# sara-nl/saraGAN

Hardware: AMD Instinct MI355X
Metric: 3D volumes/sec/node (G+D step) at 128x128x32 (higher is better)
Workload: dtype bf16

## Files before the change

include/saragan_hip.h:

```cpp
#ifndef SARAGAN_HIP_H
#define SARAGAN_HIP_H

#include <stddef.h>
#include <stdint.h>

#ifdef __cplusplus
extern "C" {
#endif

typedef void* sg_stream_t;

typedef enum { SG_F32 = 0, SG_BF16 = 1 } sg_dtype;

enum {
  SG_OK = 0,
  SG_EINVAL = -1,
  SG_EWORKSPACE = -2,
  SG_EALIGN = -3,
  SG_EUNSUPPORTED = -4
};

typedef struct {
  int32_t n, d, h, w;
  int32_t cin, cout;
  int32_t kd, kh, kw;
  int32_t upsample_in;
} sg_conv_shape;

typedef struct {
  uint32_t struct_size;
  const float* bias;
  int32_t act;
  float slope;
  int32_t pixel_norm;
  float eps;
  float* pn_scale;
  const void* mask_bits;
  float mask_slope;
  void* sign_out;
  int32_t out_scale;
  int32_t out_off[3];
  int32_t tap_off[3];
  int32_t pool;
  void* workspace;
  size_t workspace_bytes;
  int32_t x_plane_channels;
  const void* pn_bwd_y;
  const float* pn_bwd_scale;
  const void* in_mask_bits;
  float in_mask_slope;
  float in_gain;
  const float* rgb_w;
  const float* rgb_bias;
  void* rgb_out;
  const void* pw_x;
  const float* pw_wmat;
  void* pw_dx;
  float* pw_dw;
  float* pw_dbias;
  float pw_coef;
} sg_conv_epilogue;

size_t sg_sign_words_bytes(int64_t nvox, int32_t c);
int sg_sign_words(const void* t, void* words, int64_t nvox, int32_t c, sg_dtype dt, sg_stream_t st);

const char* sg_version(void);
const char* sg_error_string(int code);

size_t sg_conv3d_packed_bytes(const sg_conv_shape* s, sg_dtype dt);
int sg_conv3d_pack_weights(const float* w_dhwio, float coef, int transpose_flip, void* wp,
                           const sg_conv_shape* s, sg_dtype dt, sg_stream_t st);
int sg_conv3d_pack_weights_batch(int n, const float* const* w_dhwio, const float* coef, const int* transpose_flip,
                                 void* const* wp, const sg_conv_shape* shapes, sg_dtype dt, sg_stream_t st);
size_t sg_conv3d_fwd_workspace(const sg_conv_shape* s, sg_dtype dt);
size_t sg_conv3d_pw_epilogue_workspace(void);
int sg_conv3d_fwd(const void* x, const void* wp, void* y, const sg_conv_shape* s,
                  const sg_conv_epilogue* ep, sg_dtype dt, sg_stream_t st);
int sg_upconv3d_subpixel_supported(const sg_conv_shape* s, sg_dtype dt);
size_t sg_upconv3d_subpixel_packed_bytes(const sg_conv_shape* s, sg_dtype dt);
int sg_upconv3d_subpixel_pack(const float* w_dhwio, float coef, void* wp, const sg_conv_shape* s, sg_dtype dt, sg_stream_t st);
int sg_upconv3d_subpixel_fwd(const void* x, const void* wp, void* y, const sg_conv_shape* s, const sg_conv_epilogue* ep,
                             sg_dtype dt, sg_stream_t st);
int sg_upconv3d_subpixel_wgrad_supported(const sg_conv_shape* s, sg_dtype dt);
size_t sg_upconv3d_subpixel_wgrad_workspace(const sg_conv_shape* s, sg_dtype dt);
int sg_upconv3d_subpixel_wgrad(const void* x, const void* gy, float* dw_dhwio, float* dbias, float coef, void* workspace,
                               size_t workspace_bytes, const sg_conv_shape* s, sg_dtype dt, sg_stream_t st);
int sg_upconv3d_subpixel_dgrad_supported(const sg_conv_shape* s, sg_dtype dt);
size_t sg_upconv3d_subpixel_dgrad_packed_bytes(const sg_conv_shape* s, sg_dtype dt);
int sg_upconv3d_subpixel_dgrad_pack(const float* w_dhwio, float coef, void* wp, const sg_conv_shape* s, sg_dtype dt, sg_stream_t st);
int sg_upconv3d_subpixel_dgrad(const void* gy, const void* wp, void* gx, const sg_conv_shape* s, sg_dtype dt, sg_stream_t st);
size_t sg_conv3d_wgrad_workspace(const sg_conv_shape* s, sg_dtype dt);
int sg_conv3d_wgrad(const void* x, const void* dy, float* dw_dhwio, float coef, void* workspace,
                    size_t workspace_bytes, const sg_conv_shape* s, sg_dtype dt, sg_stream_t st);
int sg_conv3d_wgrad_bias(const void* x, const void* dy, float* dw_dhwio, float* dbias, float coef, void* workspace,
                         size_t workspace_bytes, const sg_conv_shape* s, sg_dtype dt, sg_stream_t st);
int sg_conv3d_wgrad_bias_up_masked(const void* x, const void* dy_half, const void* mask_bits, float mask_slope, float dy_gain,
                                   float* dw, float* dbias, float coef, void* workspace, size_t workspace_bytes,
                                   const sg_conv_shape* s, sg_dtype dt, sg_stream_t st);
#define SG_WGRAD_ACCUMULATE 1u
#define SG_WGRAD_CLEAN_WORKSPACE 2u
int sg_conv3d_wgrad_bias_ex(const void* x, const void* dy, const void* mask_bits, float mask_slope, float dy_gain,
                            float* dw_dhwio, float* dbias, float coef, unsigned flags, void* workspace, size_t workspace_bytes,
                            const sg_conv_shape* s, sg_dtype dt, sg_stream_t st);
size_t sg_conv3d_wgrad_clean_bytes(const sg_conv_shape* s, sg_dtype dt);

int sg_conv3d_pw_bwd(const void* x, const void* dy, const float* w_mat, float* dw_dhwio, float* dbias, void* dx,
                     float coef, void* workspace, size_t workspace_bytes, const sg_conv_shape* s, sg_dtype dt,
                     sg_stream_t st);

int sg_bias_act_fwd(const void* x, const float* bias, void* y, int64_t nvox, int32_t c, int32_t act,
                    float slope, sg_dtype dt, sg_stream_t st);
size_t sg_bias_act_bwd_workspace(int32_t c);
int sg_bias_act_bwd(const void* dy, const void* y, void* dx, float* dbias, void* workspace, int64_t nvox,
                    int32_t c, float slope, sg_dtype dt, sg_stream_t st);
int sg_bias_act_bwd_bits(const void* dy, const void* y_sign_words, void* dx, float* dbias, void* workspace,
                         int64_t nvox, int32_t c, float slope, sg_dtype dt, sg_stream_t st);
int sg_pixel_norm_fwd(const void* x, void* y, float* scale, int64_t nvox, int32_t c, float eps,
                      sg_dtype dt, sg_stream_t st);
int sg_pixel_norm_bwd(const void* dy, const void* y, const float* scale, void* dx, int64_t nvox,
                      int32_t c, sg_dtype dt, sg_stream_t st);
int sg_pixel_norm_act_bwd(const void* dy, const void* y, const float* scale, const void* y_sign_words, float slope,
                          void* dz, float* dbias, void* workspace, int64_t nvox, int32_t c, sg_dtype dt,
                          sg_stream_t st);
int sg_pixel_norm_act_bwd_pw(const void* g_small, int32_t cs, const float* w_small, const void* y, const float* scale,
                             const void* y_sign_words, float slope, void* dz, float* dbias, void* workspace,
                             int64_t nvox, int32_t c, sg_dtype dt, sg_stream_t st);
size_t sg_pixel_norm_act_bwd_pw_wg_workspace(int32_t c, int32_t cs);
int sg_pixel_norm_act_bwd_pw_wg(const void* g_small, int32_t cs, const float* w_small, const void* y, const float* scale,
                                const void* y_sign_words, float slope, void* dz, float* dbias, float* dw_small, float* db_small,
                                float coef_small, void* workspace, size_t workspace_bytes, int64_t nvox, int32_t c, sg_dtype dt,
                                sg_stream_t st);
int sg_upscale2x(const void* x, void* y, int32_t n, int32_t d, int32_t h, int32_t w, int32_t c,
                 float gain, sg_dtype dt, sg_stream_t st);
int sg_upscale2x_masked(const void* x, void* y, const void* mask_bits, float mask_slope, int32_t n, int32_t d,
                        int32_t h, int32_t w, int32_t c, float gain, sg_dtype dt, sg_stream_t st);
int sg_downscale2x(const void* x, void* y, int32_t n, int32_t d, int32_t h, int32_t w, int32_t c,
                   float gain, sg_dtype dt, sg_stream_t st);
int sg_upscale_nn(const void* x, void* y, const void* mask_bits, float mask_slope, int32_t n, int32_t d, int32_t h,
                  int32_t w, int32_t c, int32_t fd, int32_t fh, int32_t fw, float gain, sg_dtype dt, sg_stream_t st);
int sg_upscale_nn_planes(const void* x, void* y, const void* mask_bits, float mask_slope, int32_t n, int32_t d, int32_t h,
                         int32_t w, int32_t c, int32_t fd, int32_t fh, int32_t fw, float gain, int32_t plane_channels,
                         sg_dtype dt, sg_stream_t st);
int sg_downscale_sum(const void* x, void* y, int32_t n, int32_t d, int32_t h, int32_t w, int32_t c, int32_t fd,
                     int32_t fh, int32_t fw, float gain, sg_dtype dt, sg_stream_t st);
int sg_downscale_sum_masked(const void* x, const void* mask_bits, float mask_slope, void* y, int32_t n, int32_t d, int32_t h,
                            int32_t w, int32_t c, int32_t fd, int32_t fh, int32_t fw, float gain, sg_dtype dt, sg_stream_t st);
int sg_trilinear_up2x(const void* x, void* y, int32_t n, int32_t d, int32_t h, int32_t w, int32_t c, int32_t adjoint,
                      sg_dtype dt, sg_stream_t st);
int sg_axpby(const void* a, const void* b, void* out, float wa, float wb, int64_t numel, sg_dtype dt,
             sg_stream_t st);
int sg_axpby_dev(const void* a, const void* b, void* out, const float* w, int64_t numel, sg_dtype dt, sg_stream_t st);
int sg_lerp_rows(const void* a, const void* b, const float* gamma, void* out, int32_t n, int64_t per_sample, sg_dtype dt,
                 sg_stream_t st);
int sg_add_noise(const void* x, void* out, float stddev, uint64_t seed, uint64_t offset, int64_t numel,
                 sg_dtype dt, sg_stream_t st);
int sg_add_noise_dev(const void* x, void* out, float stddev, uint64_t seed, uint64_t* offset_dev, uint64_t bump,
                     int64_t numel, sg_dtype dt, sg_stream_t st);
int sg_sumsq_ndhwc_keep_w(const void* g, float* out, int32_t n, int32_t d, int32_t h, int32_t w, int32_t c,
                          sg_dtype dt, sg_stream_t st);
int sg_minibatch_stddev_fwd(const void* x, void* y, float* workspace, int32_t n, int64_t vox_per_sample,
                            int32_t c, int32_t group_size, sg_dtype dt, sg_stream_t st);
int sg_minibatch_stddev_bwd(const void* dy, const void* x, void* dx, float* workspace, int32_t n,
                            int64_t vox_per_sample, int32_t c, int32_t group_size, sg_dtype dt, sg_stream_t st);
size_t sg_mbstd_stat_workspace(int32_t n, int64_t vox_per_sample, int32_t c, int32_t group_size, int32_t nseg);
int sg_mbstd_stat_fwd(const void* x, float* stat, float* workspace, size_t workspace_bytes, int32_t n, int64_t vox_per_sample,
                      int32_t c, int32_t group_size, int32_t nseg, sg_dtype dt, sg_stream_t st);
int sg_mbstd_stat_bwd(const float* gstat, const void* x, void* dx, int32_t n, int64_t vox_per_sample, int32_t c,
                      int32_t group_size, int32_t nseg, sg_dtype dt, sg_stream_t st);
int sg_mbstd_stat_bwd2(const void* h, const void* x, const float* gstat, void* gx, float* ggstat, float* workspace,
                       size_t workspace_bytes, int32_t n, int64_t vox_per_sample, int32_t c, int32_t group_size, int32_t nseg,
                       sg_dtype dt, sg_stream_t st);
int sg_mbstd_term_fwd(const void* y, const float* s, const float* B, void* out, int32_t n, int64_t plane, sg_dtype dt,
                      sg_stream_t st);
int sg_mbstd_term_dot(const void* g, const float* B, float* r, int32_t n, int64_t plane, sg_dtype dt, sg_stream_t st);
int sg_mbstd_term_outer(const float* s, const void* g, float* Bg, int32_t n, int64_t plane, sg_dtype dt, sg_stream_t st);
int sg_cond_embed(void* z, const float* c, float* W, void* out, int32_t n, int32_t zdim, int32_t l, int32_t adjoint, sg_dtype dt,
                  sg_stream_t st);
int sg_cond_project(const void* o, const float* c, void* out, int32_t n, int32_t l, int32_t adjoint, sg_dtype dt, sg_stream_t st);
int sg_cast(const void* src, sg_dtype dt_src, void* dst, sg_dtype dt_dst, int64_t numel, sg_stream_t st);

int sg_adam_ema(float* p, const float* g, float* m, float* v, float* ema, int64_t numel, float lr_t,
                float b1, float b2, float eps, float gscale, float ema_decay, sg_stream_t st);
enum { SG_OPT_SGD = 0, SG_OPT_MOMENTUM = 1, SG_OPT_ADADELTA = 2 };
int sg_optim_step(int kind, float* p, const float* g, float* s1, float* s2, float* ema, int64_t numel, float lr,
                  float h, float eps, int nesterov, float gscale, float ema_decay, sg_stream_t st);
int sg_adam_ema_dev(float* p, const float* g, float* m, float* v, float* ema, int64_t numel, const float* lr_t,
                    float b1, float b2, float eps, float gscale, float ema_decay, sg_stream_t st);
int sg_optim_step_dev(int kind, float* p, const float* g, float* s1, float* s2, float* ema, int64_t numel, const float* lr,
                      float h, float eps, int nesterov, float gscale, float ema_decay, sg_stream_t st);
int sg_segment_sumsq(const float* flat, const int64_t* offsets, float* out, int32_t nseg, sg_stream_t st);
int sg_nonfinite_flag(const float* x, int64_t numel, int32_t* flag, int32_t accumulate, sg_stream_t st);
int sg_segment_sumsq_flag(const float* flat, const int64_t* offsets, float* out, int32_t nseg, int32_t* flag,
                          int32_t accumulate, sg_stream_t st);
int sg_guard_step(const int32_t* flag, int64_t* t, int64_t* counters, double lr, const double* lr_dev, float* lr_t,
                  int32_t adam, double b1, double b2, sg_stream_t st);
int sg_adam_ema_guarded(float* p, const float* g, float* m, float* v, float* ema, int64_t numel, const float* lr_t,
                        const int32_t* skip, float b1, float b2, float eps, float gscale, float ema_decay, sg_stream_t st);
int sg_optim_step_guarded(int kind, float* p, const float* g, float* s1, float* s2, float* ema, int64_t numel,
                          const float* lr, const int32_t* skip, float h, float eps, int nesterov, float gscale,
                          float ema_decay, sg_stream_t st);
#define SG_SEG_CHUNK 4096
int sg_adamw_ema(float* p, const float* g, float* m, float* v, float* ema, int64_t total, const int64_t* segs,
                 const int32_t* blocks, int32_t nseg, int32_t nblocks, float lr, const float* lr_dev, const int32_t* skip,
                 float b1, float b2, float eps, float decay, float gscale, float ema_decay, sg_stream_t st);
int sg_lamb_moments(const float* p, const float* g, float* m, float* v, int64_t total, const int64_t* segs,
                    const int32_t* blocks, int32_t nseg, int32_t nblocks, float* partials, const int64_t* t, int32_t advance,
                    const int32_t* skip, double b1, double b2, float eps, float decay, float gscale, sg_stream_t st);
int sg_lamb_ratios(const int64_t* segs, int32_t nseg, int32_t nblocks, const float* partials, float* ratios, int64_t* t,
                   int32_t advance, const int32_t* skip, sg_stream_t st);
int sg_lamb_update(float* p, const float* m, const float* v, float* ema, int64_t total, const int64_t* segs,
                   const int32_t* blocks, int32_t nseg, int32_t nblocks, const float* ratios, const int64_t* t, float lr,
                   const float* lr_dev, const int32_t* skip, double b1, double b2, float eps, float decay, float ema_decay,
                   sg_stream_t st);

#define SG_SPECTRAL_SEG_FIELDS 8
int sg_spectral_refresh(const float* p, float* eff, int64_t total, const int64_t* segs, const int32_t* blocks, int32_t nseg,
                        int32_t nblocks, float* u, int64_t ulen, float* v, int64_t vlen, float* sigma, float* nt,
                        float* partials, float* cols, int64_t collen, int32_t iteration, sg_stream_t st);
int sg_spectral_pullback(float* g, const float* eff, int64_t total, const int64_t* segs, const int32_t* blocks, int32_t nseg,
                         int32_t nblocks, const float* u, int64_t ulen, const float* v, int64_t vlen, const float* sigma,
                         float* partials, sg_stream_t st);

enum { SG_AUG_FLIP_W = 1, SG_AUG_FLIP_H = 2, SG_AUG_FLIP_D = 4, SG_AUG_ROT90 = 8, SG_AUG_TRANSLATE = 16, SG_AUG_ALL = 31 };
int sg_augment_draw(int32_t* params, int32_t n, uint32_t ops, int32_t m_d, int32_t m_h, int32_t m_w, float p,
                    const float* p_dev, uint64_t seed, uint64_t offset, uint64_t* offset_dev, uint64_t bump, sg_stream_t st);
int sg_augment_apply(const void* x, void* y, const int32_t* params, int32_t n, int32_t d, int32_t h, int32_t w, int32_t c,
                     uint32_t ops, float fill, int32_t adjoint, sg_dtype dt, sg_stream_t st);
int sg_ada_update(const float* logits, int32_t n, int64_t* state, float* p, int32_t interval, int64_t target_num,
                  int64_t target_den, float delta, float p_max, sg_stream_t st);

enum { SG_AUGF_SCALE = 32, SG_AUGF_ROTATE = 64, SG_AUGF_SHIFT = 128, SG_AUGF_BRIGHTNESS = 256, SG_AUGF_CONTRAST = 512,
       SG_AUGF_ALL = 992 };
int sg_augment_affine_draw(float* params, int32_t n, uint32_t ops, int32_t d, int32_t h, int32_t w, double max_scale,
                           double max_angle, double max_shift_d, double max_shift_h, double max_shift_w, double max_brightness,
                           double max_contrast, float p, const float* p_dev, uint64_t seed, uint64_t offset, uint64_t* offset_dev,
                           uint64_t bump, sg_stream_t st);
int sg_augment_affine_apply(const void* x, void* y, const float* params, int32_t n, int32_t d, int32_t h, int32_t w, int32_t c,
                            float fill, uint32_t flags, sg_dtype dt, sg_stream_t st);

int sg_filter_axis(const void* x, void* y, const void* add, int64_t outer, int32_t n, int64_t inner, const double* taps,
                   int32_t ntaps, int32_t mode, int32_t border, double alpha, int32_t f64, sg_stream_t st);
int sg_swd_gather(const float* x, float* out, const int32_t* d0, const int32_t* h0, const int32_t* w0, int32_t n_img,
                  int32_t c, int32_t d, int32_t h, int32_t w, int32_t per_image, int32_t rd, int32_t rh, int32_t rw,
// ... 44 lines not shown
```

saragan_amd/_lib.py:

```python
import ctypes as C
import os

_HERE = os.path.dirname(os.path.abspath(__file__))
LIB_PATH = os.environ.get('SARAGAN_LIB') or os.path.join(_HERE, 'libsaragan_hip.so')

SG_F32, SG_BF16 = 0, 1
SG_OPT_SGD, SG_OPT_MOMENTUM, SG_OPT_ADADELTA = 0, 1, 2
SG_SEG_CHUNK = 4096
SG_EUNSUPPORTED = -4
SG_WGRAD_ACCUMULATE, SG_WGRAD_CLEAN_WORKSPACE = 1, 2
SG_AUG_FLIP_W, SG_AUG_FLIP_H, SG_AUG_FLIP_D, SG_AUG_ROT90, SG_AUG_TRANSLATE, SG_AUG_ALL = 1, 2, 4, 8, 16, 31
SG_AUGF_SCALE, SG_AUGF_ROTATE, SG_AUGF_SHIFT, SG_AUGF_BRIGHTNESS, SG_AUGF_CONTRAST, SG_AUGF_ALL = 32, 64, 128, 256, 512, 992
SG_AUGF_ADJOINT, SG_AUGF_LINEAR = 1, 2


class ConvShape(C.Structure):
    _fields_ = [('n', C.c_int32), ('d', C.c_int32), ('h', C.c_int32), ('w', C.c_int32),
                ('cin', C.c_int32), ('cout', C.c_int32),
                ('kd', C.c_int32), ('kh', C.c_int32), ('kw', C.c_int32), ('upsample_in', C.c_int32)]


class ConvEpilogue(C.Structure):
    _fields_ = [('struct_size', C.c_uint32),
                ('bias', C.c_void_p), ('act', C.c_int32), ('slope', C.c_float), ('pixel_norm', C.c_int32),
                ('eps', C.c_float), ('pn_scale', C.c_void_p), ('mask_bits', C.c_void_p), ('mask_slope', C.c_float),
                ('sign_out', C.c_void_p), ('out_scale', C.c_int32), ('out_off', C.c_int32 * 3),
                ('tap_off', C.c_int32 * 3), ('pool', C.c_int32), ('workspace', C.c_void_p),
                ('workspace_bytes', C.c_size_t), ('x_plane_channels', C.c_int32), ('pn_bwd_y', C.c_void_p),
                ('pn_bwd_scale', C.c_void_p), ('in_mask_bits', C.c_void_p), ('in_mask_slope', C.c_float),
                ('in_gain', C.c_float), ('rgb_w', C.c_void_p), ('rgb_bias', C.c_void_p), ('rgb_out', C.c_void_p),
                ('pw_x', C.c_void_p), ('pw_wmat', C.c_void_p), ('pw_dx', C.c_void_p), ('pw_dw', C.c_void_p),
                ('pw_dbias', C.c_void_p), ('pw_coef', C.c_float)]

    def __init__(self, *args, **kw):
        super().__init__(C.sizeof(type(self)), *args, **kw)


class ProfEntry(C.Structure):
    _fields_ = [('kind', C.c_int32), ('shape', ConvShape), ('dtype', C.c_int32), ('launches', C.c_int64),
                ('total_ms', C.c_double), ('flops_per_launch', C.c_double), ('kernel', C.c_char * 64)]


_p, _i32, _i64, _f, _u64, _sz = C.c_void_p, C.c_int32, C.c_int64, C.c_float, C.c_uint64, C.c_size_t
_SHP = C.POINTER(ConvShape)

SIGNATURES = {
    'sg_version': (C.c_char_p, []),
    'sg_error_string': (C.c_char_p, [C.c_int]),
    'sg_conv3d_packed_bytes': (_sz, [_SHP, C.c_int]),
    'sg_conv3d_pack_weights': (C.c_int, [_p, _f, C.c_int, _p, _SHP, C.c_int, _p]),
    'sg_conv3d_pack_weights_batch': (C.c_int, [C.c_int, _p, _p, _p, _p, _p, C.c_int, _p]),
    'sg_conv3d_fwd_workspace': (_sz, [_SHP, C.c_int]),
    'sg_conv3d_pw_epilogue_workspace': (_sz, []),
    'sg_conv3d_fwd': (C.c_int, [_p, _p, _p, _SHP, C.POINTER(ConvEpilogue), C.c_int, _p]),
    'sg_upconv3d_subpixel_supported': (C.c_int, [_SHP, C.c_int]),
    'sg_upconv3d_subpixel_packed_bytes': (_sz, [_SHP, C.c_int]),
    'sg_upconv3d_subpixel_pack': (C.c_int, [_p, _f, _p, _SHP, C.c_int, _p]),
    'sg_upconv3d_subpixel_fwd': (C.c_int, [_p, _p, _p, _SHP, C.POINTER(ConvEpilogue), C.c_int, _p]),
    'sg_upconv3d_subpixel_wgrad_supported': (C.c_int, [_SHP, C.c_int]),
    'sg_upconv3d_subpixel_wgrad_workspace': (_sz, [_SHP, C.c_int]),
    'sg_upconv3d_subpixel_wgrad': (C.c_int, [_p, _p, _p, _p, _f, _p, _sz, _SHP, C.c_int, _p]),
    'sg_upconv3d_subpixel_dgrad_supported': (C.c_int, [_SHP, C.c_int]),
    'sg_upconv3d_subpixel_dgrad_packed_bytes': (_sz, [_SHP, C.c_int]),
    'sg_upconv3d_subpixel_dgrad_pack': (C.c_int, [_p, _f, _p, _SHP, C.c_int, _p]),
    'sg_upconv3d_subpixel_dgrad': (C.c_int, [_p, _p, _p, _SHP, C.c_int, _p]),
    'sg_conv3d_wgrad_workspace': (_sz, [_SHP, C.c_int]),
    'sg_conv3d_wgrad': (C.c_int, [_p, _p, _p, _f, _p, _sz, _SHP, C.c_int, _p]),
    'sg_conv3d_pw_bwd': (C.c_int, [_p, _p, _p, _p, _p, _p, _f, _p, _sz, _SHP, C.c_int, _p]),
    'sg_conv3d_wgrad_bias': (C.c_int, [_p, _p, _p, _p, _f, _p, _sz, _SHP, C.c_int, _p]),
    'sg_conv3d_wgrad_bias_up_masked': (C.c_int, [_p, _p, _p, _f, _f, _p, _p, _f, _p, _sz, _SHP, C.c_int, _p]),
    'sg_conv3d_wgrad_bias_ex': (C.c_int, [_p, _p, _p, _f, _f, _p, _p, _f, C.c_uint, _p, _sz, _SHP, C.c_int, _p]),
    'sg_conv3d_wgrad_clean_bytes': (_sz, [_SHP, C.c_int]),
    'sg_bias_act_fwd': (C.c_int, [_p, _p, _p, _i64, _i32, _i32, _f, C.c_int, _p]),
    'sg_bias_act_bwd_workspace': (_sz, [_i32]),
    'sg_bias_act_bwd': (C.c_int, [_p, _p, _p, _p, _p, _i64, _i32, _f, C.c_int, _p]),
    'sg_bias_act_bwd_bits': (C.c_int, [_p, _p, _p, _p, _p, _i64, _i32, _f, C.c_int, _p]),
    'sg_sign_words_bytes': (_sz, [_i64, _i32]),
    'sg_sign_words': (C.c_int, [_p, _p, _i64, _i32, C.c_int, _p]),
    'sg_pixel_norm_fwd': (C.c_int, [_p, _p, _p, _i64, _i32, _f, C.c_int, _p]),
    'sg_pixel_norm_bwd': (C.c_int, [_p, _p, _p, _p, _i64, _i32, C.c_int, _p]),
    'sg_pixel_norm_act_bwd': (C.c_int, [_p, _p, _p, _p, _f, _p, _p, _p, _i64, _i32, C.c_int, _p]),
    'sg_pixel_norm_act_bwd_pw': (C.c_int, [_p, _i32, _p, _p, _p, _p, _f, _p, _p, _p, _i64, _i32, C.c_int, _p]),
    'sg_pixel_norm_act_bwd_pw_wg': (C.c_int, [_p, _i32, _p, _p, _p, _p, _f, _p, _p, _p, _p, _f, _p, _sz, _i64, _i32, C.c_int, _p]),
    'sg_pixel_norm_act_bwd_pw_wg_workspace': (_sz, [_i32, _i32]),
    'sg_upscale2x': (C.c_int, [_p, _p, _i32, _i32, _i32, _i32, _i32, _f, C.c_int, _p]),
    'sg_upscale2x_masked': (C.c_int, [_p, _p, _p, _f, _i32, _i32, _i32, _i32, _i32, _f, C.c_int, _p]),
    'sg_downscale2x': (C.c_int, [_p, _p, _i32, _i32, _i32, _i32, _i32, _f, C.c_int, _p]),
    'sg_upscale_nn': (C.c_int, [_p, _p, _p, _f, _i32, _i32, _i32, _i32, _i32, _i32, _i32, _i32, _f, C.c_int, _p]),
    'sg_upscale_nn_planes': (C.c_int, [_p, _p, _p, _f, _i32, _i32, _i32, _i32, _i32, _i32, _i32, _i32, _f, _i32, C.c_int, _p]),
    'sg_downscale_sum': (C.c_int, [_p, _p, _i32, _i32, _i32, _i32, _i32, _i32, _i32, _i32, _f, C.c_int, _p]),
    'sg_downscale_sum_masked': (C.c_int, [_p, _p, _f, _p, _i32, _i32, _i32, _i32, _i32, _i32, _i32, _i32, _f, C.c_int, _p]),
    'sg_trilinear_up2x': (C.c_int, [_p, _p, _i32, _i32, _i32, _i32, _i32, _i32, C.c_int, _p]),
    'sg_axpby': (C.c_int, [_p, _p, _p, _f, _f, _i64, C.c_int, _p]),
    'sg_axpby_dev': (C.c_int, [_p, _p, _p, _p, _i64, C.c_int, _p]),
    'sg_lerp_rows': (C.c_int, [_p, _p, _p, _p, _i32, _i64, C.c_int, _p]),
    'sg_add_noise': (C.c_int, [_p, _p, _f, _u64, _u64, _i64, C.c_int, _p]),
    'sg_add_noise_dev': (C.c_int, [_p, _p, _f, _u64, _p, _u64, _i64, C.c_int, _p]),
    'sg_sumsq_ndhwc_keep_w': (C.c_int, [_p, _p, _i32, _i32, _i32, _i32, _i32, C.c_int, _p]),
    'sg_minibatch_stddev_fwd': (C.c_int, [_p, _p, _p, _i32, _i64, _i32, _i32, C.c_int, _p]),
    'sg_minibatch_stddev_bwd': (C.c_int, [_p, _p, _p, _p, _i32, _i64, _i32, _i32, C.c_int, _p]),
    'sg_mbstd_stat_workspace': (_sz, [_i32, _i64, _i32, _i32, _i32]),
    'sg_mbstd_stat_fwd': (C.c_int, [_p, _p, _p, _sz, _i32, _i64, _i32, _i32, _i32, C.c_int, _p]),
    'sg_mbstd_stat_bwd': (C.c_int, [_p, _p, _p, _i32, _i64, _i32, _i32, _i32, C.c_int, _p]),
    'sg_mbstd_stat_bwd2': (C.c_int, [_p, _p, _p, _p, _p, _p, _sz, _i32, _i64, _i32, _i32, _i32, C.c_int, _p]),
    'sg_mbstd_term_fwd': (C.c_int, [_p, _p, _p, _p, _i32, _i64, C.c_int, _p]),
    'sg_mbstd_term_dot': (C.c_int, [_p, _p, _p, _i32, _i64, C.c_int, _p]),
    'sg_mbstd_term_outer': (C.c_int, [_p, _p, _p, _i32, _i64, C.c_int, _p]),
    'sg_cond_embed': (C.c_int, [_p, _p, _p, _p, _i32, _i32, _i32, _i32, C.c_int, _p]),
    'sg_cond_project': (C.c_int, [_p, _p, _p, _i32, _i32, _i32, C.c_int, _p]),
    'sg_cast': (C.c_int, [_p, C.c_int, _p, C.c_int, _i64, _p]),
    'sg_adam_ema': (C.c_int, [_p, _p, _p, _p, _p, _i64, _f, _f, _f, _f, _f, _f, _p]),
    'sg_optim_step': (C.c_int, [C.c_int, _p, _p, _p, _p, _p, _i64, _f, _f, _f, C.c_int, _f, _f, _p]),
    'sg_adam_ema_dev': (C.c_int, [_p, _p, _p, _p, _p, _i64, _p, _f, _f, _f, _f, _f, _p]),
    'sg_optim_step_dev': (C.c_int, [C.c_int, _p, _p, _p, _p, _p, _i64, _p, _f, _f, C.c_int, _f, _f, _p]),
    'sg_segment_sumsq': (C.c_int, [_p, _p, _p, _i32, _p]),
    'sg_nonfinite_flag': (C.c_int, [_p, _i64, _p, _i32, _p]),
    'sg_segment_sumsq_flag': (C.c_int, [_p, _p, _p, _i32, _p, _i32, _p]),
    'sg_guard_step': (C.c_int, [_p, _p, _p, C.c_double, _p, _p, _i32, C.c_double, C.c_double, _p]),
    'sg_adam_ema_guarded': (C.c_int, [_p, _p, _p, _p, _p, _i64, _p, _p, _f, _f, _f, _f, _f, _p]),
    'sg_optim_step_guarded': (C.c_int, [C.c_int, _p, _p, _p, _p, _p, _i64, _p, _p, _f, _f, C.c_int, _f, _f, _p]),
    'sg_adamw_ema': (C.c_int, [_p, _p, _p, _p, _p, _i64, _p, _p, _i32, _i32, _f, _p, _p, _f, _f, _f, _f, _f, _f, _p]),
    'sg_lamb_moments': (C.c_int, [_p, _p, _p, _p, _i64, _p, _p, _i32, _i32, _p, _p, _i32, _p, C.c_double, C.c_double, _f, _f,
                                  _f, _p]),
    'sg_lamb_ratios': (C.c_int, [_p, _i32, _i32, _p, _p, _p, _i32, _p, _p]),
    'sg_lamb_update': (C.c_int, [_p, _p, _p, _p, _i64, _p, _p, _i32, _i32, _p, _p, _f, _p, _p, C.c_double, C.c_double, _f, _f,
                                 _f, _p]),
    'sg_spectral_refresh': (C.c_int, [_p, _p, _i64, _p, _p, _i32, _i32, _p, _i64, _p, _i64, _p, _p, _p, _p, _i64, _i32, _p]),
    'sg_spectral_pullback': (C.c_int, [_p, _p, _i64, _p, _p, _i32, _i32, _p, _i64, _p, _i64, _p, _p, _p]),
    'sg_augment_draw': (C.c_int, [_p, _i32, C.c_uint32, _i32, _i32, _i32, _f, _p, _u64, _u64, _p, _u64, _p]),
    'sg_augment_apply': (C.c_int, [_p, _p, _p, _i32, _i32, _i32, _i32, _i32, C.c_uint32, _f, _i32, C.c_int, _p]),
    'sg_ada_update': (C.c_int, [_p, _i32, _p, _p, _i32, _i64, _i64, _f, _f, _p]),
    'sg_augment_affine_draw': (C.c_int, [_p, _i32, C.c_uint32, _i32, _i32, _i32, C.c_double, C.c_double, C.c_double, C.c_double,
                                         C.c_double, C.c_double, C.c_double, _f, _p, _u64, _u64, _p, _u64, _p]),
    'sg_augment_affine_apply': (C.c_int, [_p, _p, _p, _i32, _i32, _i32, _i32, _i32, _f, C.c_uint32, C.c_int, _p]),
    'sg_filter_axis': (C.c_int, [_p, _p, _p, _i64, _i32, _i64, C.POINTER(C.c_double), _i32, _i32, _i32, C.c_double, _i32, _p]),
    'sg_swd_gather': (C.c_int, [_p, _p, _p, _p, _p, _i32, _i32, _i32, _i32, _i32, _i32, _i32, _i32, _i32, _p]),
    'sg_desc_normalize_workspace': (_sz, [_i32]),
    'sg_desc_normalize': (C.c_int, [_p, _i64, _i32, _i64, _p, _sz, _p]),
    'sg_swd_padded_rows': (_i32, [_i32]),
    'sg_swd_project': (C.c_int, [_p, _p, _p, _i32, _i32, _i32, _i32, _p]),
    'sg_sort_rows': (C.c_int, [_p, _i32, _i32, _p]),
    'sg_swd_distance': (C.c_int, [_p, _p, _p, _i32, _i32, _i32, _p]),
    'sg_metric_workspace': (_sz, []),
    'sg_sqdiff_mean': (C.c_int, [_p, _p, _p, _i64, _p, _sz, _p]),
    'sg_minmax': (C.c_int, [_p, _p, _i64, _p, _sz, _p]),
    'sg_ssim_products': (C.c_int, [_p, _p, _p, _p, _p, _i64, _p]),
    'sg_ssim_mean': (C.c_int, [_p, _p, _p, _p, _p, _p, _i32, _i32, _i32, _i32, _i32, _i32, C.c_double, C.c_double, C.c_double, _p, _sz, _p]),
    'sg_pairwise_sqdist_chunk': (_i32, []),
    'sg_pairwise_sqdist_workspace': (_sz, [_i32, _i32, _i64]),
    'sg_pairwise_sqdist': (C.c_int, [_p, _p, _p, _i32, _i32, _i64, _p, _sz, _p]),
    'sg_prof_enable': (C.c_int, [C.c_int]),
    'sg_prof_enabled': (C.c_int, []),
    'sg_prof_collect': (C.c_int, [C.POINTER(ProfEntry), _i32, C.POINTER(_i32)]),
    'sg_prof_set_filter': (C.c_int, [C.c_int, _SHP]),
    'sg_config_reload': (C.c_int, []),
}

_lib = None


def load():
    global _lib
    if _lib is not None:
        return _lib
    if not os.path.exists(LIB_PATH):
        raise ImportError(
            f'{LIB_PATH} not found: build it with `python -m saragan_amd.build` (hipcc, gfx950). '
            'There is no CPU or PyTorch fallback for the HIP path.')
    import torch
    lib = C.CDLL(LIB_PATH)
    for name, (res, args) in SIGNATURES.items():
        fn = getattr(lib, name)
        fn.restype = res
        fn.argtypes = args
    _lib = lib
    return lib


class SgError(RuntimeError):
    pass


def check(rc, what=''):
    if rc != 0:
        msg = load().sg_error_string(int(rc)).decode()
        raise SgError(f'{what}: {msg} (code {rc})')
```

saragan_amd/csrc/conv3d.hip:

```cpp
#include "common.h"
#include "prof.h"
#include "conv_args.h"

struct PackArgs {
  const float* w;
  void* wp;
  float coef;
  int taps, kd, kh, kw, cin, cout, nchunk, ntile, flip;
};

template <typename T>
__global__ void pack_weights_kernel(PackArgs a) {
  constexpr int CH = sg_traits<T>::CH;
  constexpr int EPL = CH / 2;
  const int64_t total = (int64_t)a.nchunk * a.taps * a.ntile * 64 * EPL;
  T* out = reinterpret_cast<T*>(a.wp);
  for (int64_t i = (int64_t)blockIdx.x * blockDim.x + threadIdx.x; i < total; i += (int64_t)gridDim.x * blockDim.x) {
    int e = (int)(i % EPL);
    int64_t q = i / EPL;
    int lane = (int)(q % 64); q /= 64;
    int nt = (int)(q % a.ntile); q /= a.ntile;
    int tap = (int)(q % a.taps);
    int chunk = (int)(q / a.taps);
    int ci = chunk * CH + (lane >> 5) * EPL + e;
// ... 1856 lines not shown
            float ss = 0.f;
#pragma unroll
            for (int nt = 0; nt < NTB; ++nt)
#pragma unroll
              for (int i = 0; i < 16; ++i) ss += acc[mt][nt][i] * acc[mt][nt][i];
            ss += __shfl_xor(ss, 32);
            const float sc = rsqrtf(ss * inv_c + a.eps);
#pragma unroll
            for (int nt = 0; nt < NTB; ++nt)
#pragma unroll
              for (int i = 0; i < 16; ++i) acc[mt][nt][i] *= sc;
            if (a.pn_scale != nullptr && hh == 0 && ok)
              a.pn_scale[ovox(n, d, h, w)] = sc;
          }
          if (a.sign_out != nullptr) {
#pragma unroll
            for (int nt = 0; nt < NTB; ++nt) {
              const uint32_t sw = sg_sign_word(acc[mt][nt], hh);
              if (hh == 0 && ok && nt < ntb)
                a.sign_out[ovox(n, d, h, w) * a.ntile + nt0 + nt] = sw;
            }
          }
          if (use_mask) {
#pragma unroll
            for (int nt = 0; nt < NTB; ++nt) sg_apply_sign_word(acc[mt][nt], mb[mt][nt], hh, a.mask_slope);
          }
          if (sizeof(T) == 2 && wide_store) {
            bf16_t* yrow = reinterpret_cast<bf16_t*>(y) + ovox(n, d, h, w) * (int64_t)a.cout + nt0 * 32;
#pragma unroll
            for (int nt = 0; nt < NTB; ++nt) sg_store_tile_row_bf16(yrow + nt * 32, acc[mt][nt], hh, ok && nt < ntb);
          } else if (ok) {
            T* yrow = y + ovox(n, d, h, w) * (int64_t)a.cout;
#pragma unroll
            for (int nt = 0; nt < NTB; ++nt)
#pragma unroll
              for (int qd = 0; qd < 4; ++qd) {
                const int co = (nt0 + nt) * 32 + 8 * qd + 4 * hh;
                if (a.vec_out && co + 4 <= a.cout) {
                  T tmp[4];
#pragma unroll
                  for (int e = 0; e < 4; ++e) tmp[e] = sg_traits<T>::from_f(acc[mt][nt][qd * 4 + e]);
                  if (sizeof(T) == 2) *reinterpret_cast<u32x2*>(yrow + co) = *reinterpret_cast<u32x2*>(tmp);
                  else { const u32x4 t16 = *reinterpret_cast<u32x4*>(tmp); *reinterpret_cast<u32x4*>(yrow + co) = t16; SG_STORE16_GUARD(t16); }
                } else {
#pragma unroll
                  for (int e = 0; e < 4; ++e)
                    if (co + e < a.cout) yrow[co + e] = sg_traits<T>::from_f(acc[mt][nt][qd * 4 + e]);
                }
              }
          }
        }
      }
    }
    stamp();
    __syncthreads();
  }
}

template <typename T, int MTW, int NTB, int KD, int KH, int KW, int RS = 1>
static int launch_fwd4(ConvFwdArgs& a, const sg_conv_shape* s, hipStream_t st, bool* used) {
  *used = false;
  constexpr int BM = MTW * 128;
  a.g = sg_make_geom(s, BM, true);
  const sg_tile_geom& g = a.g;
  if (g.TW > 255 || g.TH > 255 || g.TD > 255 || g.TN > 127) return SG_OK;
  const int64_t ntiles = (int64_t)g.nTn * g.nTd * g.nTh * g.nTw;
  const int ny = sg_cdiv(a.ntile, NTB);
  int gx = (256 / ny) / 8 * 8;
  if (gx < 8) gx = 8;
  if (sg_cfg().fwd4_gx > 0) gx = sg_cfg().fwd4_gx;
  if (gx < 8 || (gx & 7)) return SG_EINVAL;
  if (ntiles >= (1 << 24) || ntiles < 2 * gx) return SG_OK;
  if (KD == 1 && ntiles < 4 * gx) return SG_OK;
  if ((int64_t)g.TN * s->d * s->h * s->w * (int64_t)s->cin * (int64_t)sizeof(T) >= (1ll << 31)) return SG_OK;
  const int hv = g.TN * g.HD * g.HH * g.HW;
  a.G = 1;
  a.rs = 32;
  a.xbytes = hv * 32;
  a.lean = ((!s->upsample_in || (g.TD % 2 == 0 && g.TH % 2 == 0 && g.TW % 2 == 0 && g.TN == 1)) &&
            !sg_cfg().fwd4_no_lean) ? 1 : 0;
  a.wbytes = a.taps * NTB * 1024;
  if (sg_cdiv(hv * 2, 64) > (MTW > 2 ? 40 : (RS == 2 ? 24 : 32))) return SG_OK;
  if (MTW * NTB >= 4 && !(RS == 1 ? (g.TW == 32 && g.TH % MTW == 0) : (g.TW == 16 && g.TH % (2 * MTW) == 0))) return SG_OK;
  size_t lds = 2ull * a.xbytes + (size_t)a.nchunk * a.wbytes + NTB * 128;
  a.wres = (lds <= 160 * 1024 && !sg_cfg().fwd4_no_wres) ? 1 : 0;
  if (!a.wres) lds = 2ull * a.xbytes + 2ull * a.wbytes + NTB * 128;
  if (lds > 160 * 1024) return SG_OK;
  a.ntiles = (int)ntiles;
  a.vec_in = 1;
  a.vec_out = (s->cout % 4 == 0) ? 1 : 0;
  auto kern = conv_fwd4_kernel<T, MTW, NTB, KD, KH, KW, RS>;
  SG_ALLOW_160K_LDS(kern);
  SG_KNAME("conv_fwd4<%s,%d,%d,%d,%d,%d>", sg_tname<T>(), MTW, NTB, KD, KH, KW);
  hipLaunchKernelGGL(kern, dim3((unsigned)gx, (unsigned)ny), dim3(512), lds, st, a);
  SG_LAUNCH_CHECK();
  *used = true;
  return SG_OK;
}

template <int RING>
struct sg_unrolled_k5 {
  static constexpr int TAPS = 27, PF = RING - 1, RPS = 4, NA = 36;
  template <int ST>
  static __device__ __forceinline__ void load(u32x4 (&wfr)[RING][2], u32x4 (&xfr)[RING][2], const int (&xaddr)[NA], int wl_off) {
    constexpr int SL = ST % RING;
#pragma unroll
    for (int nt = 0; nt < 2; ++nt)
      asm volatile("ds_read_b128 %0, %1 offset:%2" : "=v"(wfr[SL][nt]) : "v"(wl_off), "n"((ST * 2 + nt) << 10));
#pragma unroll
    for (int mt = 0; mt < 2; ++mt)
      asm volatile("ds_read_b128 %0, %1" : "=v"(xfr[SL][mt]) : "v"(xaddr[sg_xa_index<2, 3, 3, true>(ST, mt)]));
  }
  template <int ST>
  static __device__ __forceinline__ void step(f32x16 (&acc)[2][2], u32x4 (&wfr)[RING][2], u32x4 (&xfr)[RING][2],
                                              const int (&xaddr)[NA], int wl_off) {
    if constexpr (ST < TAPS) {
      if constexpr (ST + PF < TAPS) load<ST + PF>(wfr, xfr, xaddr, wl_off);
      constexpr int younger = (TAPS - 1 - ST < PF ? TAPS - 1 - ST : PF) * RPS;
      asm volatile("s_waitcnt lgkmcnt(%0)" ::"n"(younger));
      __builtin_amdgcn_sched_barrier(0);
#pragma unroll
      for (int mt = 0; mt < 2; ++mt)
#pragma unroll
        for (int nt = 0; nt < 2; ++nt) sg_mfma_bf16_acc(acc[mt][nt], wfr[ST % RING][nt], xfr[ST % RING][mt]);
      __builtin_amdgcn_sched_barrier(0);
      step<ST + 1>(acc, wfr, xfr, xaddr, wl_off);
    }
  }
  template <int ST>
  static __device__ __forceinline__ void prologue(u32x4 (&wfr)[RING][2], u32x4 (&xfr)[RING][2], const int (&xaddr)[NA], int wl_off) {
    if constexpr (ST < PF) {
      load<ST>(wfr, xfr, xaddr, wl_off);
      prologue<ST + 1>(wfr, xfr, xaddr, wl_off);
    }
  }
  static __device__ __forceinline__ void run(f32x16 (&acc)[2][2], const int (&xaddr)[NA], int wl_off) {
    u32x4 wfr[RING][2], xfr[RING][2];
    SG_KLOOP_BEGIN();
    prologue<0>(wfr, xfr, xaddr, wl_off);
    step<0>(acc, wfr, xfr, xaddr, wl_off);
    asm volatile("s_nop 7\n\ts_nop 7\n\ts_nop 3" : "+v"(acc[0][0]), "+v"(acc[0][1]), "+v"(acc[1][0]), "+v"(acc[1][1]));
    SG_KLOOP_END();
  }
};

template <int EPI>
__global__ __launch_bounds__(512) void conv_fwd5_kernel(ConvFwdArgs a) {
  extern __shared__ __attribute__((aligned(16))) char smem[];
  typedef bf16_t T;
  constexpr int TAPS = 27, ES = 2, EPP = 8, NFRAG = TAPS * 2, HF = (NFRAG + 1) / 2;
  constexpr uint32_t DEAD = 0x80000000u;
  constexpr bool SIGN = (EPI & SG_EP_SIGN) != 0, MASK = (EPI & SG_EP_MASK) != 0, PN = (EPI & SG_EP_PN) != 0;
  constexpr bool POOL = (EPI & SG_EP_POOL) != 0;
  const sg_tile_geom& g = a.g;
  const int tid = threadIdx.x, lane = tid & 63;
  const int wave8 = __builtin_amdgcn_readfirstlane(tid >> 6);
  const int grp = wave8 >> 2, wave = wave8 & 3;
  const int r = lane & 31, hh = lane >> 5;
  const int xmine = grp * a.xbytes, wbase = 2 * a.xbytes;
  float* bias_lds = reinterpret_cast<float*>(smem + 2 * a.xbytes + 2 * a.wbytes);
  const int nt0 = blockIdx.y * 2;
  const int ncg = a.nchunk, cout = a.cout, ntile = a.ntile, cin = a.cin;
  const int D = g.D, H = g.H, W = g.W;

  const int xg = blockIdx.x & 7, slot = blockIdx.x >> 3;
  const int per_x = gridDim.x >> 3;
  const int cpx = (a.ntiles + 7) >> 3;
  const int t_begin = xg * cpx;
  const int t_end = min(a.ntiles, t_begin + cpx);
  const int first = t_begin + slot;
  const int K = first < t_end ? (t_end - first + per_x - 1) / per_x : 0;
  const int kmine = (K + 1 - grp) >> 1;
  const int items_mine = kmine * ncg;
  const int items_max = ((K + 1) >> 1) * ncg;

  int xaddr[36];
  int tcoord[2];
#pragma unroll
  for (int mt = 0; mt < 2; ++mt) {
    const int m = (wave * 2 + mt) * 32 + r;
    const int tw = m & 31, q = m >> 5;
    const int th = q % g.TH, td = q / g.TH;
    tcoord[mt] = tw | (th << 8) | (td << 16);
    if (mt > 0) continue;
    const int lrow = (td * g.HH + th) * g.HW + tw;
#pragma unroll
    for (int kd = 0; kd < 3; ++kd)
#pragma unroll
      for (int kh = 0; kh < 4; ++kh)
#pragma unroll
        for (int kw = 0; kw < 3; ++kw) {
          const int row = lrow + (kd * g.HH + kh) * g.HW + kw;
          xaddr[(kd * 4 + kh) * 3 + kw] = xmine + row * 32 + ((hh ^ ((row >> 3) & 1)) << 4);
        }
  }
  const int hv = g.HD * g.HH * g.HW;
  constexpr int MAXIT = 8;
  uint32_t relb[MAXIT];
  int crd[MAXIT];
#pragma unroll
  for (int k = 0; k < MAXIT; ++k) {
    const int it = (wave + 4 * k) * 64 + lane;
    const int row = it >> 1;
    const int sl = (it & 1) ^ ((row >> 3) & 1);
    uint32_t q = sg_div((uint32_t)row, g.fHW);
    const int hw = (int)(row - q * g.HW);
    uint32_t q2 = sg_div(q, g.fHH);
    const int hh_ = (int)(q - q2 * g.HH), hd = (int)q2;
    relb[k] = row < hv ? (uint32_t)((((hd * H + hh_) * W + hw) * cin + sl * EPP) * ES) : 0xC0000000u;
    crd[k] = row < hv ? (hw | (hh_ << 8) | (hd << 16)) : 0x7F7F7F7F;
  }
  const int64_t svox = (int64_t)D * H * W;
  const int64_t xsb = svox * cin * ES, ysb = (POOL ? svox >> 2 : svox) * cout * ES, wsb = svox * ntile * 4, psb = svox * 4;
  auto rsrc_of = [&](const void* base, int64_t sample_bytes, int n0) {
    return __builtin_amdgcn_make_buffer_rsrc(const_cast<char*>(reinterpret_cast<const char*>(base)) + n0 * sample_bytes, 0,
                                             (int)sample_bytes, 0x00020000);
  };
  const __amdgpu_buffer_rsrc_t rw = __builtin_amdgcn_make_buffer_rsrc(const_cast<void*>(a.wp), 0, 0x7FFFFFFF, 0x00020000);

  int kS = 0, cgS = 0;
  __amdgpu_buffer_rsrc_t rxS;
  uint32_t vk[MAXIT];
  auto enter_tile_S = [&]() {
    const sg_tile_origin o = sg_tile_of(g, (uint32_t)(first + (2 * kS + grp) * per_x));
    rxS = rsrc_of(a.x, xsb, o.n0);
    const int tile_off = (((o.d0 - 1) * H + (o.h0 - 1)) * W + (o.w0 - 1)) * cin * ES;
    const int lo_w = max(0, 1 - o.w0), hi_w = min(g.HW, W + 1 - o.w0) - 1;
    const int lo_h = max(0, 1 - o.h0), hi_h = min(g.HH, H + 1 - o.h0) - 1;
    const int lo_d = max(0, 1 - o.d0), hi_d = min(g.HD, D + 1 - o.d0) - 1;
    const uint32_t lo = (uint32_t)(lo_w | (lo_h << 8) | (lo_d << 16));
    const uint32_t hi = (uint32_t)(hi_w | (hi_h << 8) | (hi_d << 16)) | 0x808080u;
#pragma unroll
    for (int k = 0; k < MAXIT; ++k) {
      const uint32_t c_ = (uint32_t)crd[k] & 0xFFFFFFu;
      const uint32_t t1 = (c_ | 0x808080u) - lo, t2 = hi - c_;
      vk[k] = (t1 & t2 & 0x808080u) == 0x808080u ? relb[k] + (uint32_t)tile_off : DEAD;
    }
  };
  auto stage_halo = [&]() {
    const uint32_t soff = (uint32_t)(cgS * 32);
#pragma unroll
    for (int k = 0; k < MAXIT; ++k)
      if ((wave + 4 * k) * 64 < hv * 2 && crd[k] != 0x7F7F7F7F)
        __builtin_amdgcn_raw_ptr_buffer_load_lds(rxS, (lds_ptr_t)(smem + xmine + (wave + 4 * k) * 1024), 16, vk[k], soff, 0, 0);
  };
  auto stage_slab = [&](int j, int f0, int f1, int w, int nw) {
    const int cg = j % ncg;
    char* dst = smem + wbase + (j & 1) * a.wbytes;
    const uint32_t cbase = (uint32_t)(cg * TAPS * ntile + nt0) << 10;
    for (int f = f0 + w; f < f1; f += nw) {
      const int tap = f >> 1, nt = f & 1;
      __builtin_amdgcn_raw_ptr_buffer_load_lds(rw, (lds_ptr_t)(dst + (f << 10)), 16, (uint32_t)(lane * 16),
                                               cbase + ((uint32_t)(tap * ntile + nt) << 10), 0, 0);
    }
  };
  int kE = 0;
  __amdgpu_buffer_rsrc_t ryE, rsE, rmE, rpE;
  uint32_t vox[2];
  uint32_t pvox = DEAD;
  auto enter_tile_E = [&]() {
    const sg_tile_origin o = sg_tile_of(g, (uint32_t)(first + (2 * kE + grp) * per_x));
    ryE = rsrc_of(a.y, ysb, o.n0);
    if (SIGN) rsE = rsrc_of(a.sign_out, wsb, o.n0);
    if (MASK) rmE = rsrc_of(a.mask_bits, wsb, o.n0);
    if (PN) rpE = rsrc_of(a.pn_scale, psb, o.n0);
#pragma unroll
    for (int mt = 0; mt < 2; ++mt) {
      const int tc = tcoord[mt];
      const int d = o.d0 + (tc >> 16), h = o.h0 + ((tc >> 8) & 255), w = o.w0 + (tc & 255);
      vox[mt] = (d < D && h < H && w < W) ? (uint32_t)((d * H + h) * W + w) : DEAD;
      if (POOL && mt == 0)
        pvox = (vox[0] != DEAD && !(r & 1)) ? (uint32_t)((d * (H >> 1) + (h >> 1)) * (W >> 1) + (w >> 1)) : DEAD;
    }
  };
  uint32_t mbn[2][2] = {{0u, 0u}, {0u, 0u}};
  auto request_mask = [&]() {
    if constexpr (MASK) {
#pragma unroll
      for (int mt = 0; mt < 2; ++mt)
#pragma unroll
        for (int nt = 0; nt < 2; ++nt)
          mbn[mt][nt] = __builtin_amdgcn_raw_buffer_load_b32(rmE, (kE < kmine && vox[mt] != DEAD) ? (vox[mt] * (uint32_t)ntile + nt0 + nt) * 4u : DEAD, 0, 0);
    }
  };

  if (tid < 64) {
    const int co = nt0 * 32 + tid;
    bias_lds[tid] = (a.bias != nullptr && co < cout) ? a.bias[co] : 0.f;
  }
  if (items_max > 0) stage_slab(0, 0, NFRAG, wave8, 8);
  if (items_mine > 0) {
    enter_tile_S();
    enter_tile_E();
    request_mask();
    if (grp == 0) stage_halo();
  }
  asm volatile("s_waitcnt vmcnt(0)" ::: "memory");
  __syncthreads();

  const int wl0 = wbase + lane * 16;
  const float inv_c = 1.f / (float)cout;
  const float slope = a.act ? a.slope : 1.f;
  f32x16 acc[2][2];
  auto init_acc = [&]() {
#pragma unroll
    for (int mt = 0; mt < 2; ++mt)
#pragma unroll
      for (int nt = 0; nt < 2; ++nt)
#pragma unroll
        for (int i = 0; i < 16; ++i) acc[mt][nt][i] = bias_lds[nt * 32 + (i & 3) + 8 * (i >> 2) + 4 * hh];
    asm volatile("" : "+v"(acc[0][0]), "+v"(acc[0][1]), "+v"(acc[1][0]), "+v"(acc[1][1]));
  };
  int dbgi = 0;
  auto stamp = [&]() {
    if (a.dbg != nullptr && blockIdx.x == 8 && blockIdx.y == 0 && lane == 0 && wave == 0 && dbgi < 120)
      a.dbg[grp * 128 + dbgi] = __builtin_amdgcn_s_memtime();
    ++dbgi;
  };
  auto mfma_phase = [&](int q) { sg_unrolled_k5<3>::run(acc, xaddr, wl0 + (q & 1) * a.wbytes); };

  auto off_phase = [&](bool closes, int qn, int js, int f0, int f1) {
    if (qn < items_mine) stage_halo();
    if (js < items_max) stage_slab(js, f0, f1, wave, 4);
    __builtin_amdgcn_sched_barrier(0);
    stamp();
    if (closes) {
#pragma unroll
      for (int mt = 0; mt < 2; ++mt) {
        const bool ok = vox[mt] != DEAD;
        if (slope != 1.f) {
#pragma unroll
          for (int nt = 0; nt < 2; ++nt)
#pragma unroll
            for (int i = 0; i < 16; ++i) acc[mt][nt][i] = sg_lrelu(acc[mt][nt][i], slope);
        }
        if (PN) {
          float ss = 0.f;
#pragma unroll
          for (int nt = 0; nt < 2; ++nt)
#pragma unroll
            for (int i = 0; i < 16; ++i) ss += acc[mt][nt][i] * acc[mt][nt][i];
          const auto sw2 = __builtin_amdgcn_permlane32_swap(__float_as_uint(ss), __float_as_uint(ss), false, false);
          ss = __uint_as_float(sw2[0]) + __uint_as_float(sw2[1]);
          const float sc = rsqrtf(ss * inv_c + a.eps);
#pragma unroll
          for (int nt = 0; nt < 2; ++nt)
#pragma unroll
            for (int i = 0; i < 16; ++i) acc[mt][nt][i] *= sc;
          if (a.pn_scale != nullptr)
            __builtin_amdgcn_raw_buffer_store_b32(__float_as_uint(sc), rpE, (ok && hh == 0) ? vox[mt] * 4u : DEAD, 0, 0);
        }
#pragma unroll
        for (int nt = 0; nt < 2; ++nt) {
          if (SIGN) {
            uint32_t b = 0u;
#pragma unroll
            for (int i = 0; i < 16; ++i) b |= (__float_as_uint(acc[mt][nt][i]) >> 31) << ((i & 3) + 8 * (i >> 2));
            b <<= 4 * hh;
            const auto sw2 = __builtin_amdgcn_permlane32_swap(b, b, false, false);
            __builtin_amdgcn_raw_buffer_store_b32(sw2[0] | sw2[1], rsE, (ok && hh == 0) ? (vox[mt] * (uint32_t)ntile + nt0 + nt) * 4u : DEAD, 0, 0);
          }
          if (MASK) sg_apply_sign_word(acc[mt][nt], mbn[mt][nt], hh, a.mask_slope);
          if constexpr (!POOL) {
#pragma unroll
            for (int j = 0; j < 2; ++j) {
              const uint32_t a0 = sg_pack_bf16(acc[mt][nt][8 * j + 0], acc[mt][nt][8 * j + 1]), a1 = sg_pack_bf16(acc[mt][nt][8 * j + 2], acc[mt][nt][8 * j + 3]);
              const uint32_t b0 = sg_pack_bf16(acc[mt][nt][8 * j + 4], acc[mt][nt][8 * j + 5]), b1 = sg_pack_bf16(acc[mt][nt][8 * j + 6], acc[mt][nt][8 * j + 7]);
              const auto s0 = __builtin_amdgcn_permlane32_swap(a0, b0, false, false);
              const auto s1 = __builtin_amdgcn_permlane32_swap(a1, b1, false, false);
              u32x4 out;
              out[0] = s0[0]; out[1] = s1[0]; out[2] = s0[1]; out[3] = s1[1];
              __builtin_amdgcn_raw_buffer_store_b128(out, ryE, ok ? (vox[mt] * (uint32_t)cout + (uint32_t)((nt0 + nt) * 32 + 16 * j + 8 * hh)) * 2u : DEAD, 0, 0);
              SG_STORE16_GUARD(out);
            }
          }
        }
      }
      if constexpr (POOL) {
#pragma unroll
        for (int nt = 0; nt < 2; ++nt) {
          float sp[16];
#pragma unroll
          for (int i = 0; i < 16; ++i) {
            const float t = acc[0][nt][i] + acc[1][nt][i];
            const float u = __uint_as_float((uint32_t)__builtin_amdgcn_update_dpp(0, (int)__float_as_uint(t), 0xB1, 0xF, 0xF, true));
            sp[i] = (t + u) * 0.25f;
          }
#pragma unroll
          for (int j = 0; j < 2; ++j) {
            const uint32_t a0 = sg_pack_bf16(sp[8 * j + 0], sp[8 * j + 1]), a1 = sg_pack_bf16(sp[8 * j + 2], sp[8 * j + 3]);
            const uint32_t b0 = sg_pack_bf16(sp[8 * j + 4], sp[8 * j + 5]), b1 = sg_pack_bf16(sp[8 * j + 6], sp[8 * j + 7]);
            const auto s0 = __builtin_amdgcn_permlane32_swap(a0, b0, false, false);
            const auto s1 = __builtin_amdgcn_permlane32_swap(a1, b1, false, false);
            u32x4 out;
            out[0] = s0[0]; out[1] = s1[0]; out[2] = s0[1]; out[3] = s1[1];
            __builtin_amdgcn_raw_buffer_store_b128(out, ryE, pvox != DEAD ? (pvox * (uint32_t)cout + (uint32_t)((nt0 + nt) * 32 + 16 * j + 8 * hh)) * 2u : DEAD, 0, 0);
            SG_STORE16_GUARD(out);
          }
        }
      }
      ++kE;
      if (kE < kmine) enter_tile_E();
      request_mask();
      init_acc();
    }
    if (qn < items_mine) {
      if (++cgS == ncg) {
        cgS = 0;
        ++kS;
        if (kS < kmine) enter_tile_S();
      }
    }
    asm volatile("s_waitcnt vmcnt(0)" ::: "memory");
  };

  if (grp == 0) {
    init_acc();
    if (items_mine > 0 && ++cgS == ncg) { cgS = 0; ++kS; if (kS < kmine) enter_tile_S(); }
    for (int q = 0; q < items_max; ++q) {
      stamp();
      if (q < items_mine) mfma_phase(q);
      stamp();
      __syncthreads();
      stamp();
      off_phase(q < items_mine && (q % ncg) == ncg - 1, q + 1, q + 1, HF, NFRAG);
      stamp();
      __syncthreads();
    }
  } else {
    init_acc();
    for (int q = 0; q < items_max; ++q) {
      stamp();
      off_phase(q > 0 && q - 1 < items_mine && ((q - 1) % ncg) == ncg - 1, q, q + 1, 0, HF);
      stamp();
      __syncthreads();
      stamp();
      if (q < items_mine) mfma_phase(q);
      stamp();
      __syncthreads();
    }
    if (items_mine > 0 && items_mine == items_max) off_phase(true, items_mine, items_max, 0, 0);
    else if (items_mine > 0) {  }
  }
}

template <int EPI>
static int launch_fwd5_inst(const ConvFwdArgs& a, unsigned gx, unsigned gy, size_t lds, hipStream_t st) {
  auto kern = conv_fwd5_kernel<EPI>;
  SG_ALLOW_160K_LDS(kern);
  hipLaunchKernelGGL(kern, dim3(gx, gy), dim3(512), lds, st, a);
  return SG_OK;
}

static int launch_fwd5(ConvFwdArgs& a, const sg_conv_shape* s, hipStream_t st, bool* used) {
  *used = false;
  if (s->upsample_in || s->kd != 3 || s->kh != 3 || s->kw != 3 || a.os == 2 || a.tap_d || a.tap_h || a.tap_w) return SG_OK;
  if ((s->cin % 16) != 0 || (s->cout % 64) != 0 || a.pool == 1) return SG_OK;
  if (a.pool && ((s->h | s->w) & 1 || a.pixel_norm || a.mask_bits)) return SG_OK;
  if (a.pixel_norm && (a.mask_bits || a.ntile != 2)) return SG_OK;
  if (a.mask_bits && a.sign_out) return SG_OK;
  a.g = sg_make_geom(s, 256, true);
  const sg_tile_geom& g = a.g;
  if (g.TN != 1 || g.TW != 32 || (g.TH & 1) || g.TD * g.TH * g.TW != 256 || g.HD > 127 || g.HH > 127 || g.HW > 127) return SG_OK;
  const int64_t ntiles = (int64_t)g.nTn * g.nTd * g.nTh * g.nTw;
  const int ny = a.ntile / 2;
  int gx = (256 / ny) / 8 * 8;
  if (gx < 8) gx = 8;
  if (ntiles >= (1 << 24) || ntiles < 2 * gx) return SG_OK;
  {
    const int64_t svox = (int64_t)s->d * s->h * s->w;
    if (svox * s->cin * 2 >= (1ll << 31) || svox * s->cout * 2 >= (1ll << 31) || svox * a.ntile * 4 >= (1ll << 31)) return SG_OK;
  }
  const int hv = g.HD * g.HH * g.HW;
  if (sg_cdiv(hv * 2, 64) > 32) return SG_OK;
  a.G = 1;
  a.rs = 32;
  a.xbytes = hv * 32;
  a.wbytes = 27 * 2 * 1024;
  a.wres = 0;
  const size_t lds = 2ull * a.xbytes + 2ull * a.wbytes + 256;
  if (lds > 160 * 1024) return SG_OK;
  a.ntiles = (int)ntiles;
  a.vec_in = 1;
  a.vec_out = 1;
  const int epi = (a.sign_out ? SG_EP_SIGN : 0) | (a.mask_bits ? SG_EP_MASK : 0) | (a.pixel_norm ? SG_EP_PN : 0) |
                  (a.pool ? SG_EP_POOL : 0);
  int rc = SG_OK;
  switch (epi) {
    case 0: rc = launch_fwd5_inst<0>(a, (unsigned)gx, (unsigned)ny, lds, st); break;
    case SG_EP_POOL: rc = launch_fwd5_inst<SG_EP_POOL>(a, (unsigned)gx, (unsigned)ny, lds, st); break;
    case SG_EP_SIGN | SG_EP_POOL: rc = launch_fwd5_inst<SG_EP_SIGN | SG_EP_POOL>(a, (unsigned)gx, (unsigned)ny, lds, st); break;
    case SG_EP_SIGN: rc = launch_fwd5_inst<SG_EP_SIGN>(a, (unsigned)gx, (unsigned)ny, lds, st); break;
    case SG_EP_MASK: rc = launch_fwd5_inst<SG_EP_MASK>(a, (unsigned)gx, (unsigned)ny, lds, st); break;
    case SG_EP_PN: rc = launch_fwd5_inst<SG_EP_PN>(a, (unsigned)gx, (unsigned)ny, lds, st); break;
    case SG_EP_PN | SG_EP_SIGN: rc = launch_fwd5_inst<SG_EP_PN | SG_EP_SIGN>(a, (unsigned)gx, (unsigned)ny, lds, st); break;
    default: return SG_OK;
  }
  if (rc != SG_OK) return rc;
  SG_KNAME("conv_fwd5<bf16,2,2,3,3,3>");
  SG_LAUNCH_CHECK();
  *used = true;
  return SG_OK;
}

template <typename T>
__device__ __forceinline__ float sg_packed_w(const char* wp, int ntile, int cin_j, int cout_c) {
  constexpr int CH = sg_traits<T>::CH, ES = (int)sizeof(T);
  const int chunk = cin_j / CH, hh = (cin_j % CH) / (CH / 2), e = cin_j % (CH / 2);
  const char* frag = wp + ((int64_t)(chunk * ntile + (cout_c >> 5)) << 10);
  return sg_traits<T>::to_f(*reinterpret_cast<const T*>(frag + ((cout_c & 31) + 32 * hh) * 16 + e * ES));
}

template <typename T, int CIN>
__global__ __launch_bounds__(256) void pw_fwd_small_cin_kernel(ConvFwdArgs a, int64_t nvox) {
  constexpr int E = 16 / (int)sizeof(T);
  const int P = a.cout / E;
  const int p = threadIdx.x % P;
  const int c0 = p * E;
  const char* wp = reinterpret_cast<const char*>(a.wp);
  float w[CIN][E], b[E];
#pragma unroll
  for (int j = 0; j < CIN; ++j)
#pragma unroll
    for (int e = 0; e < E; ++e) w[j][e] = sg_packed_w<T>(wp, a.ntile, j, c0 + e);
#pragma unroll
  for (int e = 0; e < E; ++e) b[e] = a.bias ? a.bias[c0 + e] : 0.f;
  const T* x = reinterpret_cast<const T*>(a.x);
  T* y = reinterpret_cast<T*>(a.y);
  const int rows = 256 / P;
  const int tpw = P < 32 / E ? P : 32 / E;
  const int64_t nv_pad = (nvox + rows - 1) / rows * rows;
  const int64_t stride = (int64_t)gridDim.x * rows;
  const float slope = a.act ? a.slope : 1.f;
  const bool masked = a.mask_bits != nullptr, signs = a.sign_out != nullptr;
  const int wsel = c0 >> 5, wsh = c0 & 31, psh = (p % tpw) * E;
  auto fetch = [&](int64_t v, float (&xv)[CIN], uint32_t& mw) {
    const int64_t vc = v < nvox ? v : nvox - 1;
#pragma unroll
    for (int j = 0; j < CIN; ++j) xv[j] = sg_traits<T>::to_f(x[vc * CIN + j]);
    mw = masked ? a.mask_bits[vc * a.ntile + wsel] >> wsh : 0u;
  };
  int64_t v = (int64_t)blockIdx.x * rows + threadIdx.x / P;
  float xn[CIN];
  uint32_t mwn = 0u;
  if (v < nv_pad) fetch(v, xn, mwn);
  for (; v < nv_pad; v += stride) {
    float xv[CIN];
#pragma unroll
    for (int j = 0; j < CIN; ++j) xv[j] = xn[j];
    const uint32_t mw = mwn;
    if (v + stride < nv_pad) fetch(v + stride, xn, mwn);
    const bool live = v < nvox;
    float o[E];
    uint32_t neg = 0u;
#pragma unroll
    for (int e = 0; e < E; ++e) {
      float t = b[e];
#pragma unroll
      for (int j = 0; j < CIN; ++j) t = fmaf(xv[j], w[j][e], t);
      t = fmaxf(t, t * slope);
      neg |= (t < 0.f ? 1u : 0u) << e;
      o[e] = t;
    }
    if (signs) {
      uint32_t wbits = neg << psh;
      if (tpw == 4) {
        wbits |= (uint32_t)__builtin_amdgcn_update_dpp(0, (int)wbits, 0xB1, 0xF, 0xF, true);
        wbits |= (uint32_t)__builtin_amdgcn_update_dpp(0, (int)wbits, 0x4E, 0xF, 0xF, true);
      } else {
        for (int sh = 1; sh < tpw; sh <<= 1) wbits |= (uint32_t)__shfl_xor((int)wbits, sh);
      }
      if (live && p % tpw == 0) a.sign_out[v * a.ntile + wsel] = wbits;
    }
    if (!live) continue;
    if (masked) {
#pragma unroll
      for (int e = 0; e < E; ++e) o[e] = ((mw >> e) & 1u) ? o[e] * a.mask_slope : o[e];
    }
    u32x4 raw;
    T* t = reinterpret_cast<T*>(&raw);
#pragma unroll
    for (int e = 0; e < E; ++e) t[e] = sg_traits<T>::from_f(o[e]);
    __builtin_nontemporal_store(raw, reinterpret_cast<u32x4*>(y + v * a.cout + c0));
    SG_STORE16_GUARD(raw);
  }
}

template <typename T>
__global__ __launch_bounds__(256) void pw_fwd_small_cout_kernel(ConvFwdArgs a, int64_t nvox) {
  constexpr int E = 16 / (int)sizeof(T);
  const int P = a.cin / E;
  const int p = threadIdx.x % P;
  const char* wp = reinterpret_cast<const char*>(a.wp);
  float w[E][4];
#pragma unroll
  for (int e = 0; e < E; ++e)
#pragma unroll
    for (int c = 0; c < 4; ++c) w[e][c] = c < a.cout ? sg_packed_w<T>(wp, a.ntile, p * E + e, c) : 0.f;
  const T* x = reinterpret_cast<const T*>(a.x);
  T* y = reinterpret_cast<T*>(a.y);
  const int rows = 256 / P;
  const int64_t nv_pad = (nvox + rows - 1) / rows * rows;
  constexpr int U = 4;
  const int64_t nv_pad4 = (nvox + U * rows - 1) / (U * rows) * (U * rows);
  for (int64_t vb = (int64_t)blockIdx.x * U * rows + threadIdx.x / P; vb < nv_pad4; vb += (int64_t)gridDim.x * U * rows) {
    u32x4 rawu[U];
    uint32_t mwu[U];
#pragma unroll
    for (int u = 0; u < U; ++u) {
      const int64_t v = vb + u * rows;
      rawu[u] = v < nvox ? *reinterpret_cast<const u32x4*>(x + v * a.cin + p * E) : u32x4{0u, 0u, 0u, 0u};
      mwu[u] = (v < nvox && p == 0 && a.mask_bits) ? a.mask_bits[v] : 0u;
    }
#pragma unroll
    for (int u = 0; u < U; ++u) {
    const int64_t v = vb + u * rows;
    if (v >= nv_pad) break;
    const bool live = v < nvox;
    float s[4] = {0.f, 0.f, 0.f, 0.f};
    {
      const u32x4 raw = rawu[u];
      const T* t = reinterpret_cast<const T*>(&raw);
#pragma unroll
      for (int e = 0; e < E; ++e) {
        const float xv = sg_traits<T>::to_f(t[e]);
#pragma unroll
        for (int c = 0; c < 4; ++c) s[c] = fmaf(xv, w[e][c], s[c]);
      }
    }
    for (int sh = 1; sh < P; sh <<= 1)
#pragma unroll
      for (int c = 0; c < 4; ++c) s[c] += __shfl_xor(s[c], sh);
    if (live && p == 0) {
      uint32_t neg = 0u;
      const uint32_t mw = mwu[u];
#pragma unroll
      for (int c = 0; c < 4; ++c) {
        if (c < a.cout) {
          float t = s[c] + (a.bias ? a.bias[c] : 0.f);
          if (a.act) t = fmaxf(t, t * a.slope);
          neg |= (t < 0.f ? 1u : 0u) << c;
          if ((mw >> c) & 1u) t *= a.mask_slope;
          y[v * a.cout + c] = sg_traits<T>::from_f(t);
        }
      }
      if (a.sign_out != nullptr) a.sign_out[v] = neg;
    }
    }
  }
}

template <typename T>
// ... 30 lines not shown
  if (wave == 0) {
#pragma unroll
    for (int i = 0; i < 16; ++i) {
      float t = 0.f;
#pragma unroll
      for (int w = 0; w < 16; ++w) t += red[w][i][lane];
      const int co = nt0 * 32 + (i & 3) + 8 * (i >> 2) + 4 * hh;
      if (a.bias != nullptr && co < a.cout) t += a.bias[co];
      if (a.act) t = fmaxf(t, t * a.slope);
      acc[i] = t;
    }
    if (a.sign_out != nullptr) {
      const uint32_t sw = sg_sign_word(acc, hh);
      if (hh == 0 && vlive) a.sign_out[(int64_t)vrow * a.ntile + nt0] = sw;
    }
    if (a.mask_bits != nullptr && vlive) sg_apply_sign_word(acc, a.mask_bits[(int64_t)vrow * a.ntile + nt0], hh, a.mask_slope);
    if (vlive) {
      T* yrow = reinterpret_cast<T*>(a.y) + (int64_t)vrow * a.cout;
#pragma unroll
      for (int i = 0; i < 16; ++i) {
        const int co = nt0 * 32 + (i & 3) + 8 * (i >> 2) + 4 * hh;
        if (co < a.cout) yrow[co] = sg_traits<T>::from_f(acc[i]);
      }
    }
  }
}

template <typename T>
static int launch_pw_fwd(ConvFwdArgs& a, const sg_conv_shape* s, hipStream_t st, bool* used) {
  *used = false;
  constexpr int E = 16 / (int)sizeof(T);
  if (a.taps != 1 || s->upsample_in || a.pixel_norm) return SG_OK;
  const int64_t nvox = (int64_t)s->n * s->d * s->h * s->w;
  if (nvox <= 128 && s->cin % sg_traits<T>::CH == 0 && a.nchunk >= 64 && !sg_cfg().fwd_no_dense) {
    SG_KNAME("dense_small_m<%s>", sg_tname<T>());
    hipLaunchKernelGGL(dense_small_m_kernel<T>, dim3((unsigned)a.ntile, (unsigned)((nvox + 31) / 32)), dim3(1024), 0, st, a, (int)nvox);
    SG_LAUNCH_CHECK();
    *used = true;
    return SG_OK;
  }
  if (s->cin <= 4 && s->cout % E == 0 && 256 % (s->cout / E) == 0 && s->cout / E <= 256 &&
      ((s->cout / E) & (s->cout / E - 1)) == 0) {
    const int rows = 256 / (s->cout / E);
    const int64_t full = (nvox + rows - 1) / rows;
    int64_t nb = (full + 7) / 8;
    if (nb < 2048) nb = full < 2048 ? full : 2048;
    SG_KNAME("pw_fwd_small_cin<%s>", sg_tname<T>());
    switch (s->cin) {
      case 1: hipLaunchKernelGGL((pw_fwd_small_cin_kernel<T, 1>), dim3((unsigned)nb), dim3(256), 0, st, a, nvox); break;
      case 2: hipLaunchKernelGGL((pw_fwd_small_cin_kernel<T, 2>), dim3((unsigned)nb), dim3(256), 0, st, a, nvox); break;
      case 3: hipLaunchKernelGGL((pw_fwd_small_cin_kernel<T, 3>), dim3((unsigned)nb), dim3(256), 0, st, a, nvox); break;
      default: hipLaunchKernelGGL((pw_fwd_small_cin_kernel<T, 4>), dim3((unsigned)nb), dim3(256), 0, st, a, nvox); break;
    }
    SG_LAUNCH_CHECK();
    *used = true;
  } else if (s->cout <= 4 && s->cin % E == 0 && (s->cin / E) <= 64 && ((s->cin / E) & (s->cin / E - 1)) == 0) {
    const int rows = 256 / (s->cin / E);
    int64_t nb = (nvox + rows - 1) / rows;
    if (nb > 8192) nb = 8192;
    SG_KNAME("pw_fwd_small_cout<%s>", sg_tname<T>());
    hipLaunchKernelGGL(pw_fwd_small_cout_kernel<T>, dim3((unsigned)nb), dim3(256), 0, st, a, nvox);
    SG_LAUNCH_CHECK();
    *used = true;
  }
  return SG_OK;
}

unsigned long long* g_dbg_ts = nullptr;
extern "C" __attribute__((visibility("default"))) void sg_debug_set_ts_buffer(void* p) { g_dbg_ts = (unsigned long long*)p; }

extern "C" size_t sg_conv3d_pw_epilogue_workspace(void) { return (size_t)SG_PW_PART_ROWS * 64 * sizeof(float); }

extern "C" size_t sg_conv3d_fwd_workspace(const sg_conv_shape* s, sg_dtype dt) {
  if (!conv_shape_ok(s) || dt != SG_BF16) return 0;
  if (!sg_cfg().no_gemm && sg_gemm_conv_eligible(s, dt)) return sg_gemm_conv_workspace(s, dt);
  if (s->kd == 3 && s->kh == 3 && s->kw == 3 && s->cin == 64 && s->cout == 32 && s->w % 32 == 0 && s->d >= 4 &&
      (!s->upsample_in || ((s->d | s->h | s->w) & 1) == 0))
    return (size_t)s->n * s->d * s->h * s->w * (size_t)s->cout * 4;
  return 0;
}

extern "C" int sg_conv3d_fwd(const void* x, const void* wp, void* y, const sg_conv_shape* s,
                             const sg_conv_epilogue* ep, sg_dtype dt, sg_stream_t st) {
  if (!conv_shape_ok(s) || !x || !wp || (!y && !(ep && ep->pw_x))) return SG_EINVAL;
  if (ep && ep->struct_size != (uint32_t)sizeof(sg_conv_epilogue)) return SG_EINVAL;
  if (!sg_aligned16(x) || !sg_aligned16(wp) || !sg_aligned16(y)) return SG_EALIGN;
  ConvFwdArgs a;
  a.x = x; a.wp = wp; a.y = y;
  a.bias = ep ? ep->bias : nullptr;
  a.pn_scale = ep ? ep->pn_scale : nullptr;
  a.mask_bits = ep ? reinterpret_cast<const uint32_t*>(ep->mask_bits) : nullptr;
  a.sign_out = ep ? reinterpret_cast<uint32_t*>(ep->sign_out) : nullptr;
  a.mask_slope = ep ? ep->mask_slope : 0.f;
  a.act = ep ? ep->act : 0;
  a.slope = ep ? ep->slope : 0.f;
  a.pixel_norm = ep ? ep->pixel_norm : 0;
  a.eps = ep ? ep->eps : 0.f;
  a.tap_d = ep ? ep->tap_off[0] : 0; a.tap_h = ep ? ep->tap_off[1] : 0; a.tap_w = ep ? ep->tap_off[2] : 0;
  a.pool = ep ? ep->pool : 0;
  if (a.pool < 0 || a.pool > 3) return SG_EINVAL;
  a.pnb_y = ep ? ep->pn_bwd_y : nullptr;
  a.pnb_scale = ep ? ep->pn_bwd_scale : nullptr;
  if ((a.pnb_y != nullptr) != (a.pnb_scale != nullptr) || (a.pnb_y && !sg_aligned16(a.pnb_y))) return SG_EINVAL;
  a.xcs = s->cin; a.xco = 0; a.addend = nullptr;
  a.in_mask = ep ? reinterpret_cast<const uint32_t*>(ep->in_mask_bits) : nullptr;
  a.in_mask_slope = ep ? ep->in_mask_slope : 0.f;
  a.in_gain = ep ? ep->in_gain : 1.f;
  a.in_mask_nw = (s->cin + 31) >> 5;
  if (a.in_mask && (dt != SG_BF16 || !s->upsample_in || s->kd != 3 || s->kh != 3 || s->kw != 3 || s->cin != 64 || s->cout != 32 ||
                    !sg_aligned16(a.in_mask) || !sg_is_pow2f(a.in_gain)))
    return a.in_mask && !sg_aligned16(a.in_mask) ? SG_EALIGN : SG_EUNSUPPORTED;
  a.rgb_w = ep ? ep->rgb_w : nullptr; a.rgb_bias = ep ? ep->rgb_bias : nullptr; a.rgb_out = ep ? ep->rgb_out : nullptr;
  a.pw_x = ep ? ep->pw_x : nullptr; a.pw_wmat = ep ? ep->pw_wmat : nullptr; a.pw_dx = ep ? ep->pw_dx : nullptr;
  a.pw_part = (ep && ep->pw_x) ? reinterpret_cast<float*>(ep->workspace) : nullptr;
  if (a.rgb_out && (!a.rgb_w || !sg_aligned16(a.rgb_out))) return SG_EINVAL;
  if (a.pw_x && (!a.pw_wmat || !ep->workspace || ep->workspace_bytes < sg_conv3d_pw_epilogue_workspace() || !sg_aligned16(ep->workspace)))
    return SG_EINVAL;
  if ((a.rgb_out || a.pw_x) && (dt != SG_BF16 || s->kd != 3 || s->kh != 3 || s->kw != 3 || s->cin != 32 || s->cout != 32 || s->upsample_in ||
                                !sg_cfg().fwd3s_16 || sg_cfg().fwd_no_v3 || sg_cfg().fwd_no_v3s || sg_cfg().fwd_v1 || ep->x_plane_channels))
    return SG_EUNSUPPORTED;
  a.os = (ep && ep->out_scale == 2) ? 2 : 1;
  a.oa = ep ? ep->out_off[0] : 0; a.ob = ep ? ep->out_off[1] : 0; a.oc = ep ? ep->out_off[2] : 0;
  const bool subpixel = a.os == 2 || a.tap_d || a.tap_h || a.tap_w || s->kd == 2;
  if (subpixel && ((a.tap_d | a.tap_h | a.tap_w | a.oa | a.ob | a.oc) & ~1)) return SG_EINVAL;
  a.dbg = g_dbg_ts;
  a.dbg_flags = sg_cfg().dbg_flags;
  a.cin = s->cin; a.cout = s->cout;
  a.taps = s->kd * s->kh * s->kw; a.kh = s->kh; a.kw = s->kw;
  a.nchunk = conv_nchunk(s, dt);
  a.ntile = conv_ntile(s);
  if (a.pixel_norm && a.ntile > 4) return SG_EINVAL;
  sg_prof_scope prof(0, s, dt, sg_st(st));
  int rc;
  hipStream_t hs = sg_st(st);
  const int es = dt == SG_BF16 ? 2 : 4;
  if (subpixel) {
    const int es_ = dt == SG_BF16 ? 2 : 4;
    bool used = false;
    rc = SG_OK;
    if (s->kd == 2 && s->kh == 2 && s->kw == 2 && (s->cin * es_) % 16 == 0 && (!a.pixel_norm || a.ntile <= 2)) {
      const bool n1 = a.ntile == 1;
      if (dt == SG_BF16) rc = n1 ? launch_fwd4<bf16_t, 2, 1, 2, 2, 2>(a, s, hs, &used) : launch_fwd4<bf16_t, 2, 2, 2, 2, 2>(a, s, hs, &used);
      else rc = n1 ? launch_fwd4<float, 2, 1, 2, 2, 2>(a, s, hs, &used) : launch_fwd4<float, 2, 2, 2, 2, 2>(a, s, hs, &used);
    }
    if (rc == SG_OK && !used) rc = SG_EUNSUPPORTED;
    prof.done(rc);
    return rc;
  }
  if (a.pool && (subpixel || dt != SG_BF16 || sg_cfg().fwd_v1 || (s->cin * 2) % 16 != 0 || a.pixel_norm ||
                 (a.pool == 1 && (sg_cfg().fwd_no_v3 || sg_cfg().fwd_no_v3s)) || (a.pool == 2 && sg_cfg().fwd_no_v5) ||
                 (a.pool == 3 && (s->cin != 32 || s->kd != 3 || s->kh != 3 || s->kw != 3 || s->upsample_in || !sg_cfg().fwd3s_16 ||
                                  sg_cfg().fwd_no_v3 || sg_cfg().fwd_no_v3s || (ep && ep->x_plane_channels)))))
    return SG_EUNSUPPORTED;
  if (a.pnb_y && (subpixel || dt != SG_BF16 || sg_cfg().fwd_v1 || sg_cfg().fwd_no_v3 || sg_cfg().fwd_no_v3s || a.pool ||
                  a.pixel_norm || (s->cin * 2) % 16 != 0 || s->kd != 3 || s->kh != 3 || s->kw != 3 || s->upsample_in ||
                  (ep && ep->x_plane_channels)))
    return SG_EUNSUPPORTED;
  if (sg_small_eligible(s) && !sg_cfg().no_small && !a.pool && !a.pnb_y && !(ep && ep->x_plane_channels)) {
    rc = sg_small_fwd(x, reinterpret_cast<const char*>(wp) + (size_t)a.nchunk * a.taps * a.ntile * 1024, y, s, a.bias, a.act, a.slope,
                      a.pixel_norm, a.eps, a.pn_scale, a.mask_bits, a.mask_slope, a.sign_out, dt, hs);
    prof.done(rc);
    return rc;
  }
  if (dt == SG_BF16 && !sg_cfg().no_gemm && !a.pool && !a.pnb_y && !a.pixel_norm && !(ep && ep->x_plane_channels) &&
      sg_gemm_conv_eligible(s, dt)) {
    bool used = false;
    rc = sg_gemm_conv_fwd(x, wp, y, s, a.bias, a.act, a.slope, a.mask_bits, a.mask_slope, a.sign_out, ep ? ep->workspace : nullptr,
                          ep ? ep->workspace_bytes : 0, hs, &used);
    if (rc != SG_OK || used) { prof.done(rc); return rc; }
  }
  if (a.pool == 2) {
    bool used = false;
    rc = launch_fwd5(a, s, hs, &used);
    if (rc == SG_OK && !used) rc = SG_EUNSUPPORTED;
    prof.done(rc);
    return rc;
  }
  if (!sg_cfg().fwd_no_pw && !a.pool && !a.pnb_y) {
    bool used = false;
    rc = dt == SG_BF16 ? launch_pw_fwd<bf16_t>(a, s, hs, &used) : launch_pw_fwd<float>(a, s, hs, &used);
    if (rc != SG_OK || used) { prof.done(rc); return rc; }
  }
  const bool v2 = ((s->cin * es) % 16 == 0) && !sg_cfg().fwd_v1;
  const int xpl = ep ? ep->x_plane_channels : 0;
  if (xpl != 0 && (xpl != 32 || s->upsample_in || a.pool || !(v2 && !sg_cfg().fwd_no_v3 && (!a.pixel_norm || a.ntile == 1)))) {
    prof.done(xpl != 32 ? SG_EINVAL : SG_EUNSUPPORTED);
    return xpl != 32 ? SG_EINVAL : SG_EUNSUPPORTED;
  }
  if (v2 && !sg_cfg().fwd_no_v3 && (!a.pixel_norm || a.ntile == 1)) {
    bool used = false;
    rc = SG_OK;
    const bool k333 = s->kd == 3 && s->kh == 3 && s->kw == 3, k133 = s->kd == 1 && s->kh == 3 && s->kw == 3;
    if (dt == SG_BF16 && k333 && !sg_cfg().fwd_no_v3s && !sg_cfg().fwd_no_ksplit && a.nchunk == 4 && a.ntile == 1 && s->cin == 64 &&
        !a.pool && !a.pnb_y && !(a.mask_bits && a.sign_out) && !(a.pixel_norm && a.mask_bits) &&
        !(s->upsample_in && a.mask_bits && !a.in_mask) &&
        !(a.in_mask && (!s->upsample_in || a.sign_out || a.pixel_norm || xpl)) &&
        ep && ep->workspace &&
        ep->workspace_bytes >= (size_t)s->n * s->d * s->h * s->w * (size_t)s->cout * 4 && sg_aligned16(ep->workspace)) {
      if (!sg_cfg().fwd_no_3p && !xpl) {
        bool u3 = false;
        rc = sg_launch_fwd3p(a, s, hs, &u3);
        if (rc != SG_OK || u3) { prof.done(rc); return rc; }
      }
      ConvFwdArgs p1 = a, p2 = a;
      sg_conv_shape sh = *s;
      sh.cin = 32;
      p1.cin = p2.cin = 32; p1.nchunk = p2.nchunk = 2; p1.xcs = p2.xcs = 64;
      p1.xco = 0; p1.y = ep->workspace; p1.bias = nullptr; p1.act = 0; p1.mask_bits = nullptr; p1.sign_out = nullptr;
      p1.pixel_norm = 0; p1.pn_scale = nullptr;
      p2.xco = 32; p2.addend = reinterpret_cast<const float*>(ep->workspace);
      if (xpl) {
        p1.xcs = p2.xcs = 32;
        p2.xco = 0;
        p2.x = reinterpret_cast<const char*>(a.x) + (size_t)s->n * s->d * s->h * s->w * 64;
      }
      p2.wp = reinterpret_cast<const char*>(a.wp) + (size_t)2 * a.taps * a.ntile * 1024;
      bool u1 = false, u2 = false;
      rc = launch_fwd3s<2, 1>(p1, &sh, hs, &u1);
      if (rc == SG_OK && u1) {
        rc = launch_fwd3s<2, 2>(p2, &sh, hs, &u2);
        if (rc == SG_OK && !u2) rc = SG_EINVAL;
        SG_KNAME("conv_fwd3s<bf16,2> x2 (K split)");
        prof.done(rc);
        return rc;
      }
      if (rc != SG_OK) { prof.done(rc); return rc; }
    }
    if (xpl || a.in_mask) { prof.done(SG_EUNSUPPORTED); return SG_EUNSUPPORTED; }
    if (dt == SG_BF16 && k333 && !sg_cfg().fwd_no_v3s) {
      if (a.nchunk == 2 && sg_cfg().fwd3s_16) {
        int pw_rows = 0;
        rc = sg_launch_fwd3w(a, s, hs, &used, &pw_rows);
        if (rc == SG_OK && used && a.pw_x)
          rc = sg_pw_wgrad_finalize(a.pw_part, pw_rows, ep->pw_dw, ep->pw_dbias, ep->pw_coef, hs);
        if (rc != SG_OK || used) { prof.done(rc); return rc; }
      }
      if (a.rgb_out || a.pw_x || a.pool == 3) { prof.done(SG_EUNSUPPORTED); return SG_EUNSUPPORTED; }
      if (a.nchunk == 2) rc = launch_fwd3s<2>(a, s, hs, &used);
      else if (a.nchunk == 1) rc = launch_fwd3s<1>(a, s, hs, &used);
      if (rc != SG_OK || used) { prof.done(rc); return rc; }
    }
    if (a.pool || a.pnb_y) { prof.done(SG_EUNSUPPORTED); return SG_EUNSUPPORTED; }
    if (dt == SG_BF16) {
      if (k333 && a.nchunk == 2) rc = launch_fwd3r<bf16_t, 2, 2, 3, 3, 3>(a, s, hs, &used);
      else if (k333 && a.nchunk == 1) rc = launch_fwd3r<bf16_t, 2, 1, 3, 3, 3>(a, s, hs, &used);
      else if (k133 && a.nchunk == 2) rc = launch_fwd3r<bf16_t, 2, 2, 1, 3, 3>(a, s, hs, &used);
      else if (k133 && a.nchunk == 1) rc = launch_fwd3r<bf16_t, 2, 1, 1, 3, 3>(a, s, hs, &used);
    } else {
      if (k333 && a.nchunk == 2) rc = launch_fwd3r<float, 2, 2, 3, 3, 3>(a, s, hs, &used);
      else if (k333 && a.nchunk == 1) rc = launch_fwd3r<float, 2, 1, 3, 3, 3>(a, s, hs, &used);
      else if (k133 && a.nchunk == 2) rc = launch_fwd3r<float, 2, 2, 1, 3, 3>(a, s, hs, &used);
      else if (k133 && a.nchunk == 1) rc = launch_fwd3r<float, 2, 1, 1, 3, 3>(a, s, hs, &used);
    }
    if (rc != SG_OK || used) { prof.done(rc); return rc; }
  }
  if (a.in_mask) { prof.done(SG_EUNSUPPORTED); return SG_EUNSUPPORTED; }
  if (v2 && dt == SG_BF16 && !sg_cfg().fwd_no_v5) {
    bool used = false;
    rc = launch_fwd5(a, s, hs, &used);
    if (rc != SG_OK || used) { prof.done(rc); return rc; }
  }
  if (v2 && !sg_cfg().fwd_no_v4 && (!a.pixel_norm || a.ntile <= 2)) {
    bool used = false;
    rc = SG_OK;
    const bool k333 = s->kd == 3 && s->kh == 3 && s->kw == 3, k133 = s->kd == 1 && s->kh == 3 && s->kw == 3;
    const sg_tile_geom g4 = sg_make_geom(s, 256, true);
    const bool n1 = a.ntile == 1 || (!(g4.TW == 32 && (g4.TH & 1) == 0) && !a.pixel_norm);
    if (dt == SG_BF16 && k333 && a.ntile >= 2 && g4.TW == 16 && (g4.TH & 3) == 0 && !a.pixel_norm && !sg_cfg().fwd4_no_lean) {
      rc = launch_fwd4<bf16_t, 2, 2, 3, 3, 3, 2>(a, s, hs, &used);
      if (rc != SG_OK || used) { prof.done(rc); return rc; }
    }
    if (dt == SG_BF16) {
      if (k333) rc = n1 ? launch_fwd4<bf16_t, 2, 1, 3, 3, 3>(a, s, hs, &used) : launch_fwd4<bf16_t, 2, 2, 3, 3, 3>(a, s, hs, &used);
      else if (k133) rc = n1 ? launch_fwd4<bf16_t, 2, 1, 1, 3, 3>(a, s, hs, &used) : launch_fwd4<bf16_t, 2, 2, 1, 3, 3>(a, s, hs, &used);
    } else {
      if (k333) rc = n1 ? launch_fwd4<float, 2, 1, 3, 3, 3>(a, s, hs, &used) : launch_fwd4<float, 2, 2, 3, 3, 3>(a, s, hs, &used);
      else if (k133) rc = n1 ? launch_fwd4<float, 2, 1, 1, 3, 3>(a, s, hs, &used) : launch_fwd4<float, 2, 2, 1, 3, 3>(a, s, hs, &used);
    }
    if (rc != SG_OK || used) { prof.done(rc); return rc; }
  }
  {
    const int cand[5][2] = {{2, 4}, {2, 2}, {2, 1}, {1, 2}, {1, 1}};
    int best = -1;
    int64_t best_blocks = -1;
    for (int i = 0; i < 5; ++i) {
      const int mtw = cand[i][0], ntb = cand[i][1];
      if (ntb > 1 && ntb / 2 >= a.ntile) continue;
      if (a.pixel_norm && ntb < a.ntile) continue;
      if (!v2 && mtw == 1) continue;
      sg_tile_geom gg = sg_make_geom(s, mtw * 128, v2);
      const int64_t blocks = (int64_t)gg.nTn * gg.nTd * gg.nTh * gg.nTw * sg_cdiv(a.ntile, ntb);
      if (blocks >= 384) { best = i; break; }
      if (blocks > best_blocks) { best_blocks = blocks; best = i; }
    }
    if (best < 0) best = 0;
    const int mtw = cand[best][0], ntb = cand[best][1];
    const int gc = !v2 ? 0 : (a.nchunk >= 4 && a.taps <= 9 && !(mtw == 2 && ntb == 4) ? 4 : (a.nchunk >= 2 ? 2 : 1));
#define SG_FWD2(T, M, N)                                                                                   \
  (gc == 4 ? launch_fwd2<T, M, (M == 2 && N == 4 ? 2 : N), 4>(a, s, hs)                                     \
           : gc == 2 ? launch_fwd2<T, M, N, 2>(a, s, hs) : launch_fwd2<T, M, N, 1>(a, s, hs))
#define SG_FWD_PICK(T)                                                                                     \
  do {                                                                                                     \
    if (!v2) {                                                                                             \
      rc = ntb == 4 ? launch_fwd<T, 2, 4>(a, s, hs) : ntb == 2 ? launch_fwd<T, 2, 2>(a, s, hs)              \
                                                              : launch_fwd<T, 2, 1>(a, s, hs);              \
    } else if (mtw == 2) {                                                                                 \
      rc = ntb == 4 ? SG_FWD2(T, 2, 4) : ntb == 2 ? SG_FWD2(T, 2, 2) : SG_FWD2(T, 2, 1);                    \
    } else {                                                                                               \
      rc = ntb == 2 ? SG_FWD2(T, 1, 2) : SG_FWD2(T, 1, 1);                                                  \
    }                                                                                                      \
  } while (0)
    if (dt == SG_BF16) SG_FWD_PICK(bf16_t);
    else if (dt == SG_F32) SG_FWD_PICK(float);
    else rc = SG_EINVAL;
#undef SG_FWD_PICK
#undef SG_FWD2
  }
  prof.done(rc);
  return rc;
}
```

saragan_amd/csrc/subpix.hip:

```cpp
#include "common.h"
#include "prof.h"
#include <type_traits>

struct SubpixArgs {
  const bf16_t* x;
  const char* wp;
  bf16_t* y;
  const float* bias;
  float* pn_scale;
  uint32_t* sign_out;
  float slope, eps;
  int act, pixel_norm;
  int N, d, h, w, cin, cout, nchunk, ntile;
  int TD, TH, TW;
  int nTd, nTh, nTw;
  int HH, HW, hv;
  int64_t class_stride;
};

namespace {
constexpr int kWHalf = 4 * 8 * 1024;
constexpr int kXMax = 4 * 6 * 34 * 32;

template <int A, int AO>
// ... 450 lines not shown
          if (hh == 0) a.sign_out[ov * 2 + t2] = sw_;
        }
        sg_store_tile_row_bf16(a.y + ov * 64 + t2 * 32, acc[t2 * 4 + cl], hh, true);
      }
    }
  };
  parity(std::integral_constant<int, 0>{});
  parity(std::integral_constant<int, 1>{});
}

struct SubpixPackArgs {
  const float* w;
  char* wp;
  float coef;
  int cin, cout, nchunk, ntile;
  int64_t class_stride;
};

__global__ void upconv_subpixel_pack_kernel(SubpixPackArgs a) {
  const int64_t per_class = (int64_t)a.nchunk * 8 * a.ntile * 64 * 8;
  const int64_t total = per_class * 8;
  for (int64_t i = (int64_t)blockIdx.x * blockDim.x + threadIdx.x; i < total; i += (int64_t)gridDim.x * blockDim.x) {
    const int cls = (int)(i / per_class);
    int64_t q = i % per_class;
    const int e = (int)(q % 8); q /= 8;
    const int lane = (int)(q % 64); q /= 64;
    const int nt = (int)(q % a.ntile); q /= a.ntile;
    const int tap = (int)(q % 8);
    const int chunk = (int)(q / 8);
    const int ci = chunk * 16 + (lane >> 5) * 8 + e, co = nt * 32 + (lane & 31);
    float v = 0.f;
    if (ci < a.cin && co < a.cout) {
      const int par[3] = {cls >> 2, (cls >> 1) & 1, cls & 1};
      const int tp[3] = {tap >> 2, (tap >> 1) & 1, tap & 1};
      int lo[3], hi[3];
#pragma unroll
      for (int k = 0; k < 3; ++k) {
        if (par[k] == 0) { lo[k] = tp[k] == 0 ? 0 : 1; hi[k] = tp[k] == 0 ? 0 : 2; }
        else { lo[k] = tp[k] == 0 ? 0 : 2; hi[k] = tp[k] == 0 ? 1 : 2; }
      }
      for (int kd = lo[0]; kd <= hi[0]; ++kd)
        for (int kh = lo[1]; kh <= hi[1]; ++kh)
          for (int kw = lo[2]; kw <= hi[2]; ++kw)
            v += a.w[((((int64_t)kd * 3 + kh) * 3 + kw) * a.cin + ci) * a.cout + co];
      v *= a.coef;
    }
    reinterpret_cast<bf16_t*>(a.wp + (int64_t)cls * a.class_stride)[i % per_class] = (bf16_t)v;
    const int grp = (cls >> 2) * 2 + (tap >> 2), f = (cls & 3) * 4 + (tap & 3);
    const int64_t gi = ((((int64_t)nt * a.nchunk + chunk) * 4 + grp) * 16 + f) * 512 + lane * 8 + e;
    reinterpret_cast<bf16_t*>(a.wp + 8 * a.class_stride)[gi] = (bf16_t)v;
  }
}

static bool subpix_tile(const sg_conv_shape* s, int* td, int* th, int* tw) {
  int w_ = s->w < 32 ? s->w : 32;
  if (w_ != 32 && w_ != 16 && w_ != 8) return false;
  int h_ = 256 / w_;
  if (h_ > s->h) h_ = s->h;
  if (h_ > 8) h_ = 8;
  if (w_ == 32 && h_ > 4) h_ = 4;
  int d_ = 256 / (w_ * h_);
  if (d_ > s->d || d_ < 1 || d_ * h_ * w_ != 256) return false;
  if (s->w % w_ || s->h % h_ || s->d % d_) return false;
  if ((d_ + 2) * (h_ + 2) * (w_ + 2) * 32 > kXMax) return false;
  *td = d_; *th = h_; *tw = w_;
  return true;
}

extern "C" size_t sg_upconv3d_subpixel_packed_bytes(const sg_conv_shape* s, sg_dtype dt) {
  if (!s || dt != SG_BF16 || s->cin < 1 || s->cout < 1) return 0;
  return (size_t)2 * 8 * sg_cdiv(s->cin, 16) * 8 * sg_cdiv(s->cout, 32) * 1024;
}

extern "C" int sg_upconv3d_subpixel_supported(const sg_conv_shape* s, sg_dtype dt) {
  int td, th, tw;
  return (s && dt == SG_BF16 && s->cin > 0 && s->cout > 0 && s->cin % 16 == 0 && s->cout % 32 == 0 && subpix_tile(s, &td, &th, &tw) &&
          (int64_t)s->d * s->h * s->w * s->cin < (1ll << 31)) ? 1 : 0;
}

extern "C" int sg_upconv3d_subpixel_pack(const float* w_dhwio, float coef, void* wp, const sg_conv_shape* s, sg_dtype dt,
                                         sg_stream_t st) {
  if (!s || !w_dhwio || !wp || dt != SG_BF16) return SG_EINVAL;
  SubpixPackArgs a;
  a.w = w_dhwio; a.wp = reinterpret_cast<char*>(wp); a.coef = coef; a.cin = s->cin; a.cout = s->cout;
  a.nchunk = sg_cdiv(s->cin, 16); a.ntile = sg_cdiv(s->cout, 32);
  a.class_stride = (int64_t)a.nchunk * 8 * a.ntile * 1024;
  const int64_t total = a.class_stride * 8 / 2;
  int blocks = (int)((total + 255) / 256);
  if (blocks > 4096) blocks = 4096;
  hipLaunchKernelGGL(upconv_subpixel_pack_kernel, dim3(blocks), dim3(256), 0, sg_st(st), a);
  SG_LAUNCH_CHECK();
  return SG_OK;
}

extern "C" int sg_upconv3d_subpixel_fwd(const void* x, const void* wp, void* y, const sg_conv_shape* s, const sg_conv_epilogue* ep,
                                        sg_dtype dt, sg_stream_t st) {
  if (!s || !x || !wp || !y) return SG_EINVAL;
  if (ep && ep->struct_size != (uint32_t)sizeof(sg_conv_epilogue)) return SG_EINVAL;
  if (!sg_aligned16(x) || !sg_aligned16(wp) || !sg_aligned16(y)) return SG_EALIGN;
  if (dt != SG_BF16 || s->cin % 16 || s->cout % 32) return SG_EUNSUPPORTED;
  if (ep && (ep->mask_bits || ep->pool || ep->pn_bwd_y || ep->x_plane_channels || ep->out_scale)) return SG_EUNSUPPORTED;
  if (ep && ep->pixel_norm && s->cout != 32 && s->cout != 64) return SG_EUNSUPPORTED;
  const bool two_tiles = ep && ep->pixel_norm && s->cout == 64;
  SubpixArgs a;
  if (!subpix_tile(s, &a.TD, &a.TH, &a.TW)) return SG_EUNSUPPORTED;
  if ((int64_t)s->d * s->h * s->w * s->cin >= (1ll << 31)) return SG_EUNSUPPORTED;
  a.x = reinterpret_cast<const bf16_t*>(x); a.wp = reinterpret_cast<const char*>(wp); a.y = reinterpret_cast<bf16_t*>(y);
  a.bias = ep ? ep->bias : nullptr;
  a.pn_scale = ep ? ep->pn_scale : nullptr;
  a.sign_out = ep ? reinterpret_cast<uint32_t*>(ep->sign_out) : nullptr;
  a.slope = ep ? ep->slope : 0.f; a.eps = ep ? ep->eps : 0.f;
  a.act = ep ? ep->act : 0; a.pixel_norm = ep ? ep->pixel_norm : 0;
  a.N = s->n; a.d = s->d; a.h = s->h; a.w = s->w; a.cin = s->cin; a.cout = s->cout;
  a.nchunk = s->cin / 16; a.ntile = s->cout / 32;
  a.nTd = s->d / a.TD; a.nTh = s->h / a.TH; a.nTw = s->w / a.TW;
  a.HH = a.TH + 2; a.HW = a.TW + 2; a.hv = (a.TD + 2) * a.HH * a.HW;
  a.class_stride = (int64_t)a.nchunk * 8 * a.ntile * 1024;
  const int64_t tiles = (int64_t)s->n * a.nTd * a.nTh * a.nTw;
  if (tiles >= (1ll << 31)) return SG_EUNSUPPORTED;
  sg_conv_shape full = *s;
  full.d *= 2; full.h *= 2; full.w *= 2; full.kd = full.kh = full.kw = 3; full.upsample_in = 1;
  sg_prof_scope prof(0, &full, dt, sg_st(st));
  const size_t lds = 2 * (size_t)kWHalf + 2 * (size_t)kXMax;
  if (two_tiles) {
    auto kern = upconv_subpixel_fwd2_kernel;
    SG_ALLOW_160K_LDS(kern);
    SG_KNAME("upconv_subpixel_fwd<2 N tiles>");
    hipLaunchKernelGGL(kern, dim3((unsigned)tiles), dim3(512), lds, sg_st(st), a);
  } else if ((sg_cfg().dbg_flags & 64) || (int64_t)s->d * s->h * s->w * s->cin * 2 >= (1ll << 31)) {
    auto kern = upconv_subpixel_fwd_kernel;
    SG_ALLOW_160K_LDS(kern);
    SG_KNAME("upconv_subpixel_fwd<one tile per block>");
    hipLaunchKernelGGL(kern, dim3((unsigned)tiles, (unsigned)a.ntile), dim3(512), lds, sg_st(st), a);
  } else {
    auto kern = upconv_subpixel_fwd3_kernel;
    SG_ALLOW_160K_LDS(kern);
    SG_KNAME("upconv_subpixel_fwd");
    int64_t gx = 256 / a.ntile > 8 ? (256 / a.ntile) / 8 * 8 : 8;
    while (gx > 8 && gx > tiles) gx -= 8;
    hipLaunchKernelGGL(kern, dim3((unsigned)gx, (unsigned)a.ntile), dim3(512), 2 * (size_t)(16 * 1024) + 2 * (size_t)kXMax, sg_st(st), a);
  }
  hipError_t e = hipGetLastError();
  prof.done((int)e);
  return (int)e;
}

struct SubpixDgradArgs {
  const bf16_t* gy;
  const char* wp;
  bf16_t* gx;
  int N, d, h, w, ci, co, nchunk;
  int nTd, nTh, nTw;
  int64_t ntiles;
};

namespace {
constexpr int kDgW = 16 * 1024;
constexpr int kDgY = 6 * 10 * 2 * 33 * 32;
}

template <int NT, int TD, int TH, int TW>
__global__ __launch_bounds__(512) void upconv_subpixel_dgrad_kernel(SubpixDgradArgs a) {
  extern __shared__ __attribute__((aligned(16))) char smem[];
  static_assert(TD * TH * TW == 256, "256 low-resolution voxels per tile");
  constexpr int NG = 64 * NT / 16;
  constexpr int TPG = 16 / NT;
  constexpr int FD = 2 * TD + 2, FH = 2 * TH + 2, PW = TW + 1;
  constexpr int NPIECES = FD * FH * 2 * PW * 2, NK = (NPIECES + 511) / 512;
  static_assert(NK <= 16 && NPIECES * 16 <= kDgY, "halo image");
  constexpr uint32_t DEAD = 0x80000000u;
  char* const wbuf = smem;
  char* const ybuf = smem + 2 * kDgW;
  const int tid = threadIdx.x, lane = tid & 63, wave = tid >> 6;
  const int r = lane & 31, hh = lane >> 5;
  const int cpart = blockIdx.y;
  const int q = wave * 32 + r;
  const int vw = q % TW, vh = (q / TW) % TH, vd = q / (TW * TH);
  int xb[2][2];
#pragma unroll
  for (int i = 0; i < 2; ++i)
#pragma unroll
    for (int j = 0; j < 2; ++j)
      xb[i][j] = (((2 * vd + 2 * i) * FH + 2 * vh) * 2 * PW + vw + j) * 32 + ((hh ^ (((vw + j) >> 3) & 1)) << 4);
  const int D2 = 2 * a.d, H2 = 2 * a.h, W2 = 2 * a.w;
  const int64_t ysb = (int64_t)D2 * H2 * W2 * a.co * 2;

  __amdgpu_buffer_rsrc_t ry;
  uint32_t yv[NK];
  int d0 = 0, h0 = 0, w0 = 0, n0 = 0;
  auto enter_tile = [&](int64_t t) __attribute__((always_inline)) {
    w0 = (int)(t % a.nTw) * TW; t /= a.nTw;
    h0 = (int)(t % a.nTh) * TH; t /= a.nTh;
    d0 = (int)(t % a.nTd) * TD;
    n0 = (int)(t / a.nTd);
  };
  auto plan_tile = [&]() __attribute__((always_inline)) {
    ry = __builtin_amdgcn_make_buffer_rsrc(const_cast<char*>(reinterpret_cast<const char*>(a.gy)) + n0 * ysb, 0, (int)ysb, 0x00020000);
    const int gd0 = 2 * d0 - 1, gh0 = 2 * h0 - 1, gw0 = 2 * w0 - 1;
    int tid_ = tid;
    asm volatile("" : "+v"(tid_));
#pragma unroll
    for (int k = 0; k < NK; ++k) {
      const int p = tid_ + k * 512;
      const int row = p >> 1, half = p & 1;
      const int pos = row % PW, t1 = row / PW;
      const int par = t1 & 1, line = t1 >> 1;
      const int fh = line % FH, fd = line / FH;
      const int gd = gd0 + fd, gh = gh0 + fh, gw = gw0 + 2 * pos + par;
      const bool in = p < NPIECES && (unsigned)gd < (unsigned)D2 && (unsigned)gh < (unsigned)H2 && (unsigned)gw < (unsigned)W2;
      yv[k] = in ? (uint32_t)((((gd * H2 + gh) * W2 + gw) * a.co + half * 8) * 2) : DEAD;
    }
  };
  u32x4 gr[NK];
  auto load_y = [&](int chunk) __attribute__((always_inline)) {
#pragma unroll
    for (int k = 0; k < NK; ++k) gr[k] = __builtin_amdgcn_raw_buffer_load_b128(ry, yv[k], (uint32_t)chunk * 32u, 0);
  };
  constexpr int YPG = (NK + (NG > 2 ? NG - 2 : 1) - 1) / (NG > 2 ? NG - 2 : 1);
  auto load_y_part = [&](int chunk, bool ok, auto GG) __attribute__((always_inline)) {
    constexpr int g = decltype(GG)::value;
#pragma unroll
    for (int k = g * YPG; k < (g + 1) * YPG && k < NK; ++k)
      gr[k] = __builtin_amdgcn_raw_buffer_load_b128(ry, ok ? yv[k] : DEAD, (uint32_t)chunk * 32u, 0);
  };
  auto store_y = [&]() __attribute__((always_inline)) {
#pragma unroll
    for (int k = 0; k < NK; ++k) {
      const int p = tid + k * 512;
      const int row = p >> 1, half = p & 1;
      const int pos = row % PW;
      if (p < NPIECES) *reinterpret_cast<u32x4*>(ybuf + row * 32 + ((half ^ ((pos >> 3) & 1)) << 4)) = gr[k];
    }
  };
  u32x4 wr[4][2];
  auto load_w = [&](u32x4 (&dst)[2], int chunk, int g) __attribute__((always_inline)) {
    const char* src = a.wp + ((((int64_t)cpart * a.nchunk + chunk) * NG + g) << 14) + tid * 16;
    dst[0] = *reinterpret_cast<const u32x4*>(src);
    dst[1] = *reinterpret_cast<const u32x4*>(src + 8192);
  };
  auto store_w = [&](const u32x4 (&srcr)[2], char* dst) __attribute__((always_inline)) {
    *reinterpret_cast<u32x4*>(dst + tid * 16) = srcr[0];
    *reinterpret_cast<u32x4*>(dst + 8192 + tid * 16) = srcr[1];
  };

  const int64_t per_x = gridDim.x >> 3;
  const int64_t cpx = (a.ntiles + 7) >> 3;
  const int64_t c_begin = (blockIdx.x & 7) * cpx, c_end = c_begin + cpx < a.ntiles ? c_begin + cpx : a.ntiles;
  const int64_t t_first = c_begin + (blockIdx.x >> 3);
  const int64_t ntl = t_first < c_end ? (c_end - t_first + per_x - 1) / per_x : 0;
  if (ntl == 0) return;
  const int nchunk = a.nchunk;
  f32x16 acc[NT];

  enter_tile(t_first);
  plan_tile();
  load_y(0);
  load_w(wr[0], 0, 0);
  load_w(wr[1], 0, 1 % NG);
  load_w(wr[2], 0, 2 % NG);
  load_w(wr[3], 0, 3 % NG);
  store_y();
  store_w(wr[0], wbuf);
  __syncthreads();

  int64_t ti = 0;
  int chunk = 0;
  for (;;) {
    int nchunk_i = chunk + 1;
    int64_t nti = ti;
    if (nchunk_i == nchunk) { nchunk_i = 0; ++nti; }
    const bool more = nti < ntl;
    const int od0 = d0, oh0 = h0, ow0 = w0, on0 = n0;
    if (more && nchunk_i == 0) { enter_tile(t_first + nti * per_x); plan_tile(); }
    if (chunk == 0) {
#pragma unroll
      for (int nt = 0; nt < NT; ++nt)
#pragma unroll
        for (int i = 0; i < 16; ++i) acc[nt][i] = 0.f;
    }
    sg_static_for<NG>::run([&](auto GG) __attribute__((always_inline)) {
      constexpr int g = decltype(GG)::value;
      {
        const int g4 = g + 4;
        const int c4 = g4 < NG ? chunk : nchunk_i;
        load_w(wr[g & 3], c4, g4 % NG);
      }
      load_y_part(nchunk_i, more, GG);
      const char* ws = wbuf + (g & 1) * kDgW;
      constexpr int FD_ = 3;
      u32x4 xf[FD_], wf[FD_][NT];
      auto read_tap = [&](int slot, int tt) __attribute__((always_inline)) {
        const int tap = g * TPG + tt;
        const int td = tap >> 4, th = (tap >> 2) & 3, tw = tap & 3;
        const int off = (((td & 1) * FH + th) * 2 * PW + (tw & 1) * PW) * 32;
        xf[slot] = *reinterpret_cast<const u32x4*>(ybuf + xb[td >> 1][tw >> 1] + off);
#pragma unroll
        for (int nt = 0; nt < NT; ++nt) wf[slot][nt] = *reinterpret_cast<const u32x4*>(ws + ((tt * NT + nt) << 10) + lane * 16);
      };
#pragma unroll
      for (int tt = 0; tt < FD_ - 1 && tt < TPG; ++tt) read_tap(tt, tt);
#pragma unroll
      for (int tt = 0; tt < TPG; ++tt) {
        if (tt + FD_ - 1 < TPG) read_tap((tt + FD_ - 1) % FD_, tt + FD_ - 1);
        __builtin_amdgcn_sched_barrier(0);
#pragma unroll
        for (int nt = 0; nt < NT; ++nt) acc[nt] = sg_mfma_chunk<bf16_t>(wf[tt % FD_][nt], xf[tt % FD_], acc[nt]);
        __builtin_amdgcn_sched_barrier(0);
      }
      store_w(wr[(g + 1) & 3], wbuf + ((g + 1) & 1) * kDgW);
      __syncthreads();
    });
    if (chunk + 1 == nchunk) {
      const int64_t ov = (((int64_t)on0 * a.d + od0 + vd) * a.h + oh0 + vh) * a.w + ow0 + vw;
#pragma unroll
      for (int nt = 0; nt < NT; ++nt) sg_store_tile_row_bf16(a.gx + ov * a.ci + (cpart * NT + nt) * 32, acc[nt], hh, true);
    }
    store_y();
    __syncthreads();
    if (!more) break;
    ti = nti;
    chunk = nchunk_i;
  }
}

struct SubpixDgradPackArgs {
  const float* w;
  char* wp;
  float coef;
  int ci, co, nchunk, ntile;
};

__global__ void upconv_subpixel_dgrad_pack_kernel(SubpixDgradPackArgs a) {
  const int64_t total = (int64_t)a.nchunk * 64 * a.ntile * 64 * 8;
  for (int64_t i = (int64_t)blockIdx.x * blockDim.x + threadIdx.x; i < total; i += (int64_t)gridDim.x * blockDim.x) {
    int64_t qq = i;
    const int e = (int)(qq % 8); qq /= 8;
    const int lane = (int)(qq % 64); qq /= 64;
    const int ntl = (int)(qq % 2); qq /= 2;
    const int tap = (int)(qq % 64); qq /= 64;
    const int chunk = (int)(qq % a.nchunk);
    const int nt = (int)(qq / a.nchunk) * 2 + ntl;
    const int ci = nt * 32 + (lane & 31), co = chunk * 16 + (lane >> 5) * 8 + e;
    float v = 0.f;
    if (ci < a.ci && co < a.co) {
      const int tj[3] = {tap >> 4, (tap >> 2) & 3, tap & 3};
      int lo[3], hi[3];
#pragma unroll
      for (int k = 0; k < 3; ++k) {
        lo[k] = tj[k] == 0 ? 2 : (tj[k] == 1 ? 1 : 0);
        hi[k] = tj[k] <= 1 ? 2 : (tj[k] == 2 ? 1 : 0);
      }
      for (int kd = lo[0]; kd <= hi[0]; ++kd)
        for (int kh = lo[1]; kh <= hi[1]; ++kh)
          for (int kw = lo[2]; kw <= hi[2]; ++kw)
            v += a.w[((((int64_t)kd * 3 + kh) * 3 + kw) * a.ci + ci) * a.co + co];
      v *= a.coef;
    }
    reinterpret_cast<bf16_t*>(a.wp)[i] = (bf16_t)v;
  }
}

extern "C" int sg_upconv3d_subpixel_dgrad_supported(const sg_conv_shape* s, sg_dtype dt) {
  int td, th, tw;
  if (!s || dt != SG_BF16 || s->cin < 32 || s->cout < 16 || s->cin % 32 || s->cout % 16 || !subpix_tile(s, &td, &th, &tw)) return 0;
  const int nt = s->cin / 32;
  if (nt % 2 || !((tw == 32 && td == 2 && th == 4) || (tw == 16 && td == 2 && th == 8))) return 0;
  if ((int64_t)s->d * s->h * s->w * 8 * s->cout * 2 >= (1ll << 31)) return 0;
  return 1;
}

extern "C" size_t sg_upconv3d_subpixel_dgrad_packed_bytes(const sg_conv_shape* s, sg_dtype dt) {
  if (!s || dt != SG_BF16 || s->cin < 1 || s->cout < 1) return 0;
  return (size_t)sg_cdiv(s->cout, 16) * 64 * sg_cdiv(s->cin, 32) * 1024;
}

extern "C" int sg_upconv3d_subpixel_dgrad_pack(const float* w_dhwio, float coef, void* wp, const sg_conv_shape* s, sg_dtype dt,
                                               sg_stream_t st) {
  if (!s || !w_dhwio || !wp || dt != SG_BF16) return SG_EINVAL;
  SubpixDgradPackArgs a;
  a.w = w_dhwio; a.wp = reinterpret_cast<char*>(wp); a.coef = coef; a.ci = s->cin; a.co = s->cout;
  a.nchunk = sg_cdiv(s->cout, 16); a.ntile = sg_cdiv(s->cin, 32);
  const int64_t total = (int64_t)a.nchunk * 64 * a.ntile * 512;
  int blocks = (int)((total + 255) / 256);
  if (blocks > 4096) blocks = 4096;
  hipLaunchKernelGGL(upconv_subpixel_dgrad_pack_kernel, dim3(blocks), dim3(256), 0, sg_st(st), a);
  SG_LAUNCH_CHECK();
  return SG_OK;
}

extern "C" int sg_upconv3d_subpixel_dgrad(const void* gy, const void* wp, void* gx, const sg_conv_shape* s, sg_dtype dt, sg_stream_t st) {
  if (!s || !gy || !wp || !gx) return SG_EINVAL;
  if (!sg_aligned16(gy) || !sg_aligned16(wp) || !sg_aligned16(gx)) return SG_EALIGN;
  if (!sg_upconv3d_subpixel_dgrad_supported(s, dt)) return SG_EUNSUPPORTED;
  SubpixDgradArgs a;
  int TD, TH, TW;
  subpix_tile(s, &TD, &TH, &TW);
  a.gy = reinterpret_cast<const bf16_t*>(gy); a.wp = reinterpret_cast<const char*>(wp); a.gx = reinterpret_cast<bf16_t*>(gx);
  a.N = s->n; a.d = s->d; a.h = s->h; a.w = s->w; a.ci = s->cin; a.co = s->cout; a.nchunk = s->cout / 16;
  a.nTd = s->d / TD; a.nTh = s->h / TH; a.nTw = s->w / TW;
  a.ntiles = (int64_t)s->n * a.nTd * a.nTh * a.nTw;
  sg_conv_shape full = *s;
  full.d *= 2; full.h *= 2; full.w *= 2; full.kd = full.kh = full.kw = 3; full.upsample_in = 0;
  full.cin = s->cout; full.cout = s->cin;
  sg_prof_scope prof(0, &full, dt, sg_st(st));
  int64_t per_part = 256 / (s->cin / 64) > 8 ? 256 / (s->cin / 64) : 8;
  while (per_part > 8 && per_part > a.ntiles) per_part -= 8;
  const unsigned gx_ = (unsigned)per_part;
  const size_t lds = 2 * (size_t)kDgW + (size_t)kDgY;
  const int nt = s->cin / 32;
  SG_KNAME("upconv_subpixel_dgrad");
#define SG_DG(NT_, TD_, TH_, TW_)                                                    \
  do {                                                                               \
    auto kern = upconv_subpixel_dgrad_kernel<NT_, TD_, TH_, TW_>;                    \
    SG_ALLOW_160K_LDS(kern);                                                         \
    hipLaunchKernelGGL(kern, dim3(gx_, (unsigned)(nt / 2)), dim3(512), lds, sg_st(st), a); \
  } while (0)
  if (TW == 32) SG_DG(2, 2, 4, 32);
  else if (TW == 16) SG_DG(2, 2, 8, 16);
  else { prof.done(SG_EUNSUPPORTED); return SG_EUNSUPPORTED; }
#undef SG_DG
  hipError_t e = hipGetLastError();
  prof.done((int)e);
  return (int)e;
}

struct SubpixWgradArgs {
  const bf16_t* x;
  const bf16_t* gy;
  float* dwt;
  float* dbias;
  int N, d, h, w, cin, cout, ciT, coT;
  int nTh, nTw;
  int64_t ntiles;
  int64_t slab, bslab;
};

namespace {
constexpr int kWX = 3 * 4 * 34 * 64;
constexpr int kWY = 8 * 2 * 32 * 64;
typedef short s16x4_t __attribute__((ext_vector_type(4)));
typedef __attribute__((address_space(3))) s16x4_t* lds_s16x4;

__device__ __forceinline__ bf16x8 sg_tr_frag(const char* p) {
  const s16x4_t lo = __builtin_amdgcn_ds_read_tr16_b64_v4i16((lds_s16x4)p);
  const s16x4_t hi = __builtin_amdgcn_ds_read_tr16_b64_v4i16((lds_s16x4)(p + 256));
  typedef short s16x8_t __attribute__((ext_vector_type(8)));
  const s16x8_t v = {lo[0], lo[1], lo[2], lo[3], hi[0], hi[1], hi[2], hi[3]};
  return __builtin_bit_cast(bf16x8, v);
}
}

__global__ __launch_bounds__(512) void upconv_subpixel_wgrad_kernel(SubpixWgradArgs a) {
  extern __shared__ __attribute__((aligned(16))) char smem[];
  const int tid = threadIdx.x, lane = tid & 63;
  const int cls = __builtin_amdgcn_readfirstlane(tid >> 6);
  const int ca = cls >> 2, cb = (cls >> 1) & 1, cc = cls & 1;
  const int ci_t = blockIdx.y / a.coT, co_t = blockIdx.y % a.coT;
  const bool ones = a.dbias != nullptr && ci_t == 0;
  const int i16 = lane & 15, q16 = lane >> 4;
  const int colb = (16 * (q16 & 1) + 4 * (i16 & 3)) * 2;
  const int kb = 8 * (q16 >> 1) + (i16 >> 2);
  const int D2 = 2 * a.d, H2 = 2 * a.h, W2 = 2 * a.w;
  auto tile_of = [&](int64_t t, int& n, int& dd, int& h0, int& w0) {
    w0 = (int)(t % a.nTw) * 32; t /= a.nTw;
    h0 = (int)(t % a.nTh) * 2; t /= a.nTh;
    dd = (int)(t % a.d);
    n = (int)(t / a.d);
  };
  u32x4 sx[4], sy[4];
  auto load_tile = [&](int64_t t) {
    int n, dd, h0, w0;
    tile_of(t, n, dd, h0, w0);
#pragma unroll
    for (int k = 0; k < 4; ++k) {
      const int p = tid + k * 512;
      const int hv = p >> 2, sub = p & 3;
      const int hw_ = hv % 34, hh_ = (hv / 34) & 3, hd_ = hv / 136;
      const int zd = dd + hd_ - 1, zy = h0 + hh_ - 1, zx = w0 + hw_ - 1;
      const bool ok = p < 1632 && zd >= 0 && zd < a.d && zy >= 0 && zy < a.h && zx >= 0 && zx < a.w;
      const int64_t off = ((((int64_t)n * a.d + (ok ? zd : 0)) * a.h + (ok ? zy : 0)) * a.w + (ok ? zx : 0)) * a.cin + ci_t * 32 + sub * 8;
      const u32x4 v = *reinterpret_cast<const u32x4*>(a.x + off);
      sx[k] = ok ? v : u32x4{0u, 0u, 0u, 0u};
    }
#pragma unroll
    for (int k = 0; k < 4; ++k) {
      const int p = tid + k * 512;
      const int fv = p >> 2, sub = p & 3;
      const int fw = fv & 63, fh = (fv >> 6) & 3, fd = fv >> 8;
      const int64_t off = ((((int64_t)n * D2 + 2 * dd + fd) * H2 + 2 * h0 + fh) * W2 + 2 * w0 + fw) * a.cout + co_t * 32 + sub * 8;
      sy[k] = *reinterpret_cast<const u32x4*>(a.gy + off);
    }
  };
  auto store_tile = [&](char* xb, char* yb) {
#pragma unroll
    for (int k = 0; k < 4; ++k) {
      const int p = tid + k * 512;
      if (p < 1632) *reinterpret_cast<u32x4*>(xb + p * 16) = sx[k];
    }
#pragma unroll
    for (int k = 0; k < 4; ++k) {
      const int p = tid + k * 512;
      const int fv = p >> 2, sub = p & 3;
      const int fw = fv & 63, fh = (fv >> 6) & 3, fd = fv >> 8;
      const int pc = fd * 4 + (fh & 1) * 2 + (fw & 1);
      *reinterpret_cast<u32x4*>(yb + (((pc * 2 + (fh >> 1)) * 32 + (fw >> 1)) << 6) + sub * 16) = sy[k];
    }
  };

  f32x16 acc[9];
#pragma unroll
  for (int j = 0; j < 9; ++j)
#pragma unroll
    for (int i = 0; i < 16; ++i) acc[j][i] = 0.f;
  const bf16x8 one8 = __builtin_bit_cast(bf16x8, u32x4{0x3F803F80u, 0x3F803F80u, 0x3F803F80u, 0x3F803F80u});

  int buf = 0;
  int64_t t = blockIdx.x;
  if (t < a.ntiles) {
    load_tile(t);
    store_tile(smem, smem + kWX);
  }
  __syncthreads();
  for (; t < a.ntiles; t += gridDim.x) {
    const int64_t tn = t + gridDim.x;
    if (tn < a.ntiles) load_tile(tn);
    const char* xb = smem + buf * (kWX + kWY);
    const char* yb = xb + kWX;
#pragma unroll
    for (int th = 0; th < 2; ++th)
#pragma unroll
      for (int wh = 0; wh < 2; ++wh) {
        const bf16x8 bf = sg_tr_frag(yb + (((cls * 2 + th) * 32 + 16 * wh + kb) << 6) + colb);
#pragma unroll
        for (int tap = 0; tap < 8; ++tap) {
          const int tz = tap >> 2, ty = (tap >> 1) & 1, tx = tap & 1;
          const bf16x8 af = sg_tr_frag(xb + ((((ca + tz) * 4 + th + cb + ty) * 34 + 16 * wh + kb + cc + tx) << 6) + colb);
          acc[tap] = __builtin_amdgcn_mfma_f32_32x32x16_bf16(af, bf, acc[tap], 0, 0, 0);
        }
        if (ones) acc[8] = __builtin_amdgcn_mfma_f32_32x32x16_bf16(one8, bf, acc[8], 0, 0, 0);
      }
    if (tn < a.ntiles) store_tile(smem + (buf ^ 1) * (kWX + kWY), smem + (buf ^ 1) * (kWX + kWY) + kWX);
    __syncthreads();
    buf ^= 1;
  }
  const int r = lane & 31, hh = lane >> 5;
  const bool slab = a.slab != 0;
  __syncthreads();
  float* red = reinterpret_cast<float*>(smem);
  if (ones && hh == 0) red[cls * 32 + r] = acc[8][0];
  __syncthreads();
  if (ones && tid < 32) {
    float s = 0.f;
#pragma unroll
    for (int w8 = 0; w8 < 8; ++w8) s += red[w8 * 32 + tid];
    float* dst = a.dbias + (int64_t)blockIdx.x * a.bslab + co_t * 32 + tid;
    if (slab) *dst = s;
    else unsafeAtomicAdd(dst, s);
  }
#pragma unroll
  for (int tap = 0; tap < 8; ++tap) {
    float* dst = a.dwt + (int64_t)blockIdx.x * a.slab + (((((int64_t)cls * 8 + tap) * a.ciT + ci_t) * a.coT + co_t) << 10);
#pragma unroll
    for (int i = 0; i < 16; ++i) {
      const int row = (i & 3) + 8 * (i >> 2) + 4 * hh;
      if (slab) dst[row * 32 + r] = acc[tap][i];
      else unsafeAtomicAdd(dst + row * 32 + r, acc[tap][i]);
    }
  }
}

__global__ void upconv_subpixel_wgrad_finalize_kernel(const float* __restrict__ dwt, float* __restrict__ dw, const float* __restrict__ bsl,
// ... 96 lines not shown
```

saragan_amd/functional.py:

```python
import collections
import contextlib
import ctypes as C
import math
import os

import torch

from . import _lib
from ._lib import ConvEpilogue, ConvShape, check

_DT = {torch.float32: _lib.SG_F32, torch.bfloat16: _lib.SG_BF16}


def _stream():
    return C.c_void_p(torch.cuda.current_stream().cuda_stream)


def _dt(t):
    try:
        return _DT[t.dtype]
    except KeyError:
        raise TypeError(f'saragan_amd supports float32 and bfloat16 activations, got {t.dtype}')


def _req_cuda(*ts):
    for t in ts:
        if t is not None and not t.is_cuda:
            raise RuntimeError('saragan_amd ops run on the GPU only (no CPU fallback); got a CPU tensor')


def ndhwc(x):
    if x.dim() == 5:
        return x.contiguous(memory_format=torch.channels_last_3d)
    if x.dim() == 2:
        return x.contiguous()
    raise ValueError(f'expected a [N,C,D,H,W] or [N,F] tensor, got shape {tuple(x.shape)}')


def _dims(x):
    if x.dim() == 5:
        n, c, d, h, w = x.shape
        return n, c, d, h, w
    n, c = x.shape
    return n, c, 1, 1, 1


def _empty_like_shape(x, c_out, spatial=None, dtype=None):
    n, _, d, h, w = _dims(x)
    if spatial is not None:
        d, h, w = spatial
    dtype = dtype or x.dtype
    if x.dim() == 5:
        return torch.empty((n, c_out, d, h, w), device=x.device, dtype=dtype, memory_format=torch.channels_last_3d)
    return torch.empty((n, c_out), device=x.device, dtype=dtype)


def _ptr(t):
    return C.c_void_p(t.data_ptr()) if t is not None else None


def _switch(name):
    return bool(int(os.environ.get('SARAGAN_' + name, '0')))


_NO_PACK_BATCH = _switch('NO_PACK_BATCH')
_NO_SUBPIXEL = _switch('NO_SUBPIXEL')
_NO_CLEAN_WS = _switch('NO_CLEAN_WS')
_NO_SIGN_WORDS = _switch('NO_SIGN_WORDS')
_NO_GRAD_DEST = _switch('NO_GRAD_DEST')
_NO_PN_EPILOGUE = _switch('NO_PN_EPILOGUE')
_NO_PW_EPILOGUE = _switch('NO_PW_EPILOGUE')
_NO_BACK_PREMASK = _switch('NO_BACK_PREMASK')
_NO_RGB_FWD_EPILOGUE = _switch('NO_RGB_FWD_EPILOGUE')
_NO_RGB_FUSION = _switch('NO_RGB_FUSION')
_NO_RGB_WG_FUSION = _switch('NO_RGB_WG_FUSION')
_NO_POOL3 = _switch('NO_POOL3')
_NO_POOL_FUSION = _switch('NO_POOL_FUSION')
_NO_PLANES = _switch('NO_PLANES')
_NO_GATHER_BWD = _switch('NO_GATHER_BWD')


def _shape(n, d, h, w, cin, cout, k, ups=False):
    return ConvShape(n, d, h, w, cin, cout, k[0], k[1], k[2], 1 if ups else 0)


_PACK_CACHE = {}
_PACK_STATE = {'stale': False}
PACK_STATS = {'single': 0, 'batches': 0, 'batched': 0}


def clear_pack_cache():
    _PACK_CACHE.clear()
    _SUBPIX_CACHE.clear()
    _PACK_STATE['stale'] = False


def mark_packs_stale():
    if _NO_PACK_BATCH:
        return clear_pack_cache()
    for k in [k for k in _PACK_CACHE if k[0] == 'rgbmat']:
        del _PACK_CACHE[k]
    _SUBPIX_CACHE.clear()
    _PACK_STATE['stale'] = bool(_PACK_CACHE)


def live_packs():
    return [v[0] for v in _PACK_CACHE.values()] + list(_CLEAN_WS.values())


def _refresh_packs(lib, st):
    _PACK_STATE['stale'] = False
    by_dt = {}
    for key in list(_PACK_CACHE):
        if key[0] == 'rgbmat':
            continue
        wp, w, shp, w32 = _PACK_CACHE[key]
        if w._version != key[1] or w.data_ptr() != key[0]:
            del _PACK_CACHE[key]
            continue
        by_dt.setdefault(key[4], []).append((w32, key[2], 1 if key[3] else 0, wp, shp))
    for dt, items in by_dt.items():
        n = len(items)
        ws = (C.c_void_p * n)(*[it[0].data_ptr() for it in items])
        coefs = (C.c_float * n)(*[it[1] for it in items])
        flips = (C.c_int * n)(*[it[2] for it in items])
        wps = (C.c_void_p * n)(*[it[3].data_ptr() for it in items])
        shapes = (ConvShape * n)(*[it[4] for it in items])
        check(lib.sg_conv3d_pack_weights_batch(n, ws, coefs, flips, wps, shapes, dt, st), 'sg_conv3d_pack_weights_batch')
        PACK_STATS['batches'] += 1
        PACK_STATS['batched'] += n


def _packed(w, coef, flip, shp, dt, lib, st):
    if _PACK_STATE['stale']:
        _refresh_packs(lib, st)
    key = (w.data_ptr(), w._version, float(coef), bool(flip), dt, shp.cin, shp.cout, shp.kd, shp.kh, shp.kw)
    hit = _PACK_CACHE.get(key)
    if hit is not None:
        return hit[0]
    w32 = w.detach()
    if w32.dtype != torch.float32 or not w32.is_contiguous():
        w32 = w32.contiguous().float()
    wp = torch.empty(lib.sg_conv3d_packed_bytes(C.byref(shp), dt), device=w.device, dtype=torch.uint8)
    check(lib.sg_conv3d_pack_weights(_ptr(w32), float(coef), 1 if flip else 0, _ptr(wp), C.byref(shp), dt, st),
          'sg_conv3d_pack_weights')
    PACK_STATS['single'] += 1
    base = w._base if w._is_view() else None
    long_lived = w.is_leaf or not w.requires_grad or (base is not None and base.is_leaf)
    if long_lived and w32.data_ptr() == w.data_ptr():
        keep = ConvShape(shp.n, shp.d, shp.h, shp.w, shp.cin, shp.cout, shp.kd, shp.kh, shp.kw, shp.upsample_in)
        _PACK_CACHE[key] = (wp, w if (w.is_leaf or not w.requires_grad) else w32, keep, w32)
    return wp


def _empty_signs(device, n, d, h, w, c):
    return torch.empty((n, d, h, w, (c + 31) // 32), device=device, dtype=torch.int32)


def _check_signs(bits, nvox, c):
    if bits is None:
        return
    if bits.dtype != torch.int32 or not bits.is_contiguous() or bits.numel() != nvox * ((c + 31) // 32):
        raise ValueError('sign words must be a contiguous int32 tensor [n,d,h,w,ceil(c/32)] of the masked tensor')


def sign_words(t):
    lib = _lib.load()
    _req_cuda(t)
    t = ndhwc(t)
    n, c, d, h, w = _dims(t)
    out = _empty_signs(t.device, n, d, h, w, c)
    check(lib.sg_sign_words(_ptr(t), _ptr(out), n * d * h * w, c, _dt(t), _stream()), 'sg_sign_words')
    return out


_SUBPIX_CACHE = {}


def _subpixel_packed(w, coef, shp, dt, lib, st):
    key = (w.data_ptr(), w._version, float(coef), dt)
    hit = _SUBPIX_CACHE.get(key)
    if hit is not None:
        return hit[0]
    w32 = w.detach()
    if w32.dtype != torch.float32 or not w32.is_contiguous():
        w32 = w32.contiguous().float()
    wp = torch.empty(lib.sg_upconv3d_subpixel_packed_bytes(C.byref(shp), dt), device=w.device, dtype=torch.uint8)
    check(lib.sg_upconv3d_subpixel_pack(_ptr(w32), float(coef), _ptr(wp), C.byref(shp), dt, st), 'sg_upconv3d_subpixel_pack')
    if w.is_leaf or not w.requires_grad:
        _SUBPIX_CACHE[key] = (wp, w)
    return wp


def _raw_upconv_subpixel(x, w, coef, bias, act, slope, pixel_norm, eps, want_scale, want_signs):
    lib = _lib.load()
    n, cin, d, h, wd = _dims(x)
    cout = w.shape[-1]
    dt = _dt(x)
    if dt != _lib.SG_BF16 or x.dim() != 5:
        return None
    st = _stream()
    shp = _shape(n, d, h, wd, cin, cout, (3, 3, 3), False)
    if not lib.sg_upconv3d_subpixel_packed_bytes(C.byref(shp), dt):
        return None
    y = _empty_like_shape(x, cout, (2 * d, 2 * h, 2 * wd))
    signs = _empty_signs(x.device, n, 2 * d, 2 * h, 2 * wd, cout) if want_signs else None
    scale = torch.empty(n * 8 * d * h * wd, device=x.device, dtype=torch.float32) if (pixel_norm and want_scale) else None
    b32 = bias.detach().contiguous().float() if bias is not None else None
    ep = ConvEpilogue(_ptr(b32), 1 if act else 0, float(slope), 1 if pixel_norm else 0, float(eps), _ptr(scale), None, 0.0,
                      _ptr(signs))
    wp = _subpixel_packed(w, coef, shp, dt, lib, st)
    rc = lib.sg_upconv3d_subpixel_fwd(_ptr(x), _ptr(wp), _ptr(y), C.byref(shp), C.byref(ep), dt, st)
    if rc == _lib.SG_EUNSUPPORTED:
        return None
    check(rc, 'sg_upconv3d_subpixel_fwd')
    return y, scale, signs


PwBwd = collections.namedtuple('PwBwd', 'x wmat want_dx dw db coef')


def raw_conv(x, w, coef, flip, ups=False, bias=None, act=False, slope=0.2, pixel_norm=False, eps=1e-8,
             want_scale=False, mask_bits=None, mask_slope=0.0, want_signs=False, pool=False, pn_bwd=None, rgb=None, pw_bwd=None,
# ... 150 lines not shown
    dy = ndhwc(dy)
    n, c, d, h, w = _dims(dy)
    nvox = n * d * h * w
    bits = y is not None and y.dtype == torch.int32
    if bits:
        _check_signs(y, nvox, c)
    elif y is not None:
        y = ndhwc(y)
    dx = torch.empty_like(dy) if want_dx else None
    db = ws = None
    if want_db:
        db = _f32_out(b_ptr, (c,), dy.device)
        ws = torch.empty(lib.sg_bias_act_bwd_workspace(c), device=dy.device, dtype=torch.uint8)
    fn = lib.sg_bias_act_bwd_bits if bits else lib.sg_bias_act_bwd
    check(fn(_ptr(dy), _ptr(y), _ptr(dx), _ptr(db), _ptr(ws), nvox, c, float(slope), _dt(dy), _stream()),
          'sg_bias_act_bwd')
    return dx, db


_ZERO = {}


def _zero_scalar(like):
    z = _ZERO.get(like.device)
    if z is None:
        z = _ZERO[like.device] = torch.zeros((), device=like.device, dtype=torch.float32)
    return z.detach()


_SKIP = {'ptrs': frozenset()}
_GRAD_DEST = {}
ACCUMULATED_IN_PLACE = set()
GRAD_DEST_STATS = {'claimed': 0, 'accumulated': 0, 'adopted': 0, 'copied': 0, 'unreached': 0}


@contextlib.contextmanager
def grads_into(dest):
    prev = dict(_GRAD_DEST)
    _GRAD_DEST.clear()
    ACCUMULATED_IN_PLACE.clear()
    if not _NO_GRAD_DEST:
        _GRAD_DEST.update({k: [v, False] for k, v in dest.items()})
    try:
        yield
    finally:
        _GRAD_DEST.clear()
        _GRAD_DEST.update(prev)


def _grad_out(ptr, shape):
    if not ptr or not _GRAD_DEST or torch.is_grad_enabled():
        return None
    ent = _GRAD_DEST.get(ptr)
    if ent is None or ent[1] or ent[0].numel() != math.prod(shape):
        return None
    ent[1] = True
    GRAD_DEST_STATS['claimed'] += 1
    return ent[0].view(shape)


def _grad_acc(ptr, shape):
    if not ptr or not _GRAD_DEST or torch.is_grad_enabled():
        return None
    ent = _GRAD_DEST.get(ptr)
    if ent is None or not ent[1] or ent[0].numel() != math.prod(shape):
        return None
    return ent[0].view(shape)


def _note_accumulated(ptr):
    ACCUMULATED_IN_PLACE.add(ptr)
    GRAD_DEST_STATS['accumulated'] += 1


def _unclaim(ptr, t):
    ent = _GRAD_DEST.get(ptr) if (ptr and t is not None) else None
    if ent is not None and ent[1] and t.data_ptr() == ent[0].data_ptr():
        ent[1] = False
        GRAD_DEST_STATS['claimed'] -= 1


def _f32_out(ptr, shape, device):
    out = _grad_out(ptr, shape)
    return out if out is not None else torch.empty(shape, device=device, dtype=torch.float32)


class _GradOuts:

    def __init__(self, device):
        self.device, self.claimed = device, []

    def take(self, ptr, shape, want=True):
        if not want:
            return None
        out = _grad_out(ptr, shape)
        if out is None:
            return torch.empty(shape, device=self.device, dtype=torch.float32)
        self.claimed.append((ptr, out))
        return out

    def release(self):
        for ptr, out in self.claimed:
            _unclaim(ptr, out)
        self.claimed = []

    def declined(self, rc):
        if rc != _lib.SG_EUNSUPPORTED:
            return False
        self.release()
        return True


@contextlib.contextmanager
def skip_param_grads(params):
    prev = _SKIP['ptrs']
    _SKIP['ptrs'] = prev | frozenset(p.data_ptr() for p in params)
    try:
        yield
    finally:
        _SKIP['ptrs'] = prev


def _wants(ctx, i, ptr):
    return ctx.needs_input_grad[i] and ptr not in _SKIP['ptrs']


class ActInfo:

    def __init__(self, slope):
        self.slope = float(slope)
        self.bits = None
        self.pn = None
        self.pw = None
        self.pw_result = None
        self.n_consumers = 0
        self.n_premask = 0

    def consume(self, premask):
        self.n_consumers += 1
        if premask:
            self.n_premask += 1

    def all_premask(self):
        return self.bits is not None and self.n_consumers > 0 and self.n_consumers == self.n_premask


PwStage = collections.namedtuple('PwStage', 'x w coef b_ptr has_b x_req')


def _masked_in(ctx_info):
    return ctx_info is not None and ctx_info.all_premask()


def pn_bwd_epilogue_available(prod_shape, kernel, fmaps, dtype):
    if _NO_PN_EPILOGUE or dtype != torch.bfloat16 or len(prod_shape) != 5 or tuple(kernel) != (3, 3, 3):
        return False
    n, c, d, h, w = prod_shape
    return c == 32 and fmaps == 32 and w % 32 == 0 and d >= 2 and h >= 8


def _dgrad_into(info, g, w, coef, flip):
    if info.pn is None:
        if info.pw is not None and not torch.is_grad_enabled() and not _NO_PW_EPILOGUE and g.dtype == torch.bfloat16:
            res = _pw_fused_backward(info, g, w, coef, flip)
            if res is not None:
                return res
        return _Conv.apply(g, w, coef, flip, False, None, info.bits, info.slope)
    if torch.is_grad_enabled():
        raise NotImplementedError('second-order gradient through pixel_norm is not part of the pgan step')
    res = raw_conv(g, w, coef, flip, mask_bits=info.bits, mask_slope=info.slope, pn_bwd=info.pn)
    if res is not None:
        return res[0]
    gy = raw_conv(g, w, coef, flip)[0]
    return _PnActBwd.apply(gy, info.pn[0], info.pn[1], info.bits, info.slope, False)[0]


def _pw_fused_backward(info, g, w, coef, flip):
    pw = info.pw
    wr = pw.w
    want_w = wr.data_ptr() not in _SKIP['ptrs']
    want_b = pw.has_b and pw.b_ptr not in _SKIP['ptrs']
    want_dx = bool(pw.x_req)
    if not (want_w or want_b or want_dx):
        return None
    x_img = ndhwc(pw.x)
    if x_img.dtype != g.dtype or x_img.shape[1] != 1:
        return None
    outs = _GradOuts(g.device)
    dw = outs.take(wr.data_ptr(), tuple(wr.shape), want_w)
    db = outs.take(pw.b_ptr, (wr.shape[-1],), want_b)
    res = raw_conv(g, w, coef, flip, mask_bits=info.bits, mask_slope=info.slope,
                   pw_bwd=PwBwd(x_img, _rgb_matrix(wr, pw.coef, g.dtype, small_is_cin=True), want_dx, dw, db, pw.coef))
    if res is None:
        outs.release()
        return None
    info.pw_result = (res if want_dx else None, dw, db)
    n, c, d, h, wd = _dims(ndhwc(g))
    return torch.zeros((), device=g.device, dtype=g.dtype).expand(n, w.shape[3] if flip else w.shape[4], d, h, wd)


class BackInfo:

    def __init__(self, bits, slope):
        self.bits, self.slope = bits, float(slope)
        self.n_consumers = 0
        self.n_premask = 0
        self._decision = None

    def all_premask(self):
        if self._decision is None:
            self._decision = self.n_consumers > 0 and self.n_consumers == self.n_premask
        return self._decision


def _note_consumer(t, premask=False):
    info = getattr(t, '_sg_back', None) if t is not None else None
    if info is not None and info._decision is None:
        info.n_consumers += 1
        if premask and not _NO_BACK_PREMASK:
            info.n_premask += 1
    return info


def _note_all(*args):
    for a in args:
        if isinstance(a, torch.Tensor):
            _note_consumer(a)


def _conv_dgrad(g, w, coef, flip, ups=False, in_info=None, x_back=None):
    if ups:
        return _upconv_dgrad(g, w, coef, flip)
    if x_back is not None and x_back.all_premask():
        return _Conv.apply(g, w, coef, flip, False, None, x_back.bits, x_back.slope)
    if _masked_in(in_info):
        return _dgrad_into(in_info, g, w, coef, flip)
    return _Conv.apply(g, w, coef, flip, False)


def _conv_param_grads(x, g, w, coef, ups, want_w, want_db, b_ptr=0, gb=None):
    db_here = want_db and gb is None
    gw = None
    if want_w:
        k = tuple(w.shape[:3]) if w.dim() == 5 else (1, 1, 1)
        gw, gb2 = _Wgrad.apply(x, g, k, coef, ups, db_here, w.data_ptr(), b_ptr)
        gw = gw.reshape(w.shape) if gw is not None else None
        if db_here:
            gb = gb2
    elif db_here:
        _, gb = raw_bias_act_bwd(g, None, 0.0, want_dx=False, want_db=True, b_ptr=b_ptr)
    return gw, (gb if want_db else None)


class _Conv(torch.autograd.Function):

    @staticmethod
    def forward(ctx, x, w, coef, flip, ups, in_info=None, mask_bits=None, mask_slope=0.0):
        ctx.save_for_backward(x, w, mask_bits)
        ctx.coef, ctx.flip, ctx.ups, ctx.in_info, ctx.mask_slope = coef, flip, ups, in_info, mask_slope
        ctx.x_back = _note_consumer(x, premask=not ups)
        y, _, _ = raw_conv(x, w, coef, flip, ups, mask_bits=mask_bits, mask_slope=mask_slope)
        ctx.out_back = None
        if mask_bits is not None:
            ctx.out_back = y._sg_back = BackInfo(mask_bits, mask_slope)
        return y

    @staticmethod
    def backward(ctx, gy):
        x, w, mask_bits = ctx.saved_tensors
        if mask_bits is not None and not (ctx.out_back is not None and ctx.out_back.all_premask()):
            gy, _ = _BiasActBwd.apply(gy, mask_bits, ctx.mask_slope, False)
        gx = gw = None
        if ctx.needs_input_grad[0]:
            gx = _conv_dgrad(gy, w, ctx.coef, not ctx.flip, ctx.ups, ctx.in_info, ctx.x_back)
        if _wants(ctx, 1, w.data_ptr()):
            if ctx.flip and ctx.ups:
                raise NotImplementedError
            xs, gs = (gy, x) if ctx.flip else (x, gy)
            gw, _ = _conv_param_grads(xs, gs, w, ctx.coef, ctx.ups, True, False)
        return gx, gw, None, None, None, None, None, None


class _Wgrad(torch.autograd.Function):
    @staticmethod
    def forward(ctx, x, dy, k, coef, ups, want_db, w_ptr=0, b_ptr=0):
        _note_all(x, dy, k, coef, ups, want_db)
        ctx.save_for_backward(x, dy)
        ctx.k, ctx.coef, ctx.ups = k, coef, ups
        dw, db = raw_wgrad(x, dy, k, coef, ups, want_db, w_ptr, b_ptr)
        if db is None:
            db = _zero_scalar(x)
        ctx.mark_non_differentiable(db)
        return dw, db

    @staticmethod
    def backward(ctx, gw, _gdb):
        x, dy = ctx.saved_tensors
        if ctx.ups:
            raise NotImplementedError('third-order gradient through a fused-upsample conv')
        gx = gdy = None
        if ctx.needs_input_grad[0]:
            gx = _Conv.apply(dy, gw, ctx.coef, True, False)
        if ctx.needs_input_grad[1]:
            gdy = _Conv.apply(x, gw, ctx.coef, False, False)
        return gx, gdy, None, None, None, None, None, None


class _ConvBiasAct(torch.autograd.Function):

    @staticmethod
    def forward(ctx, x, w, b, coef, ups, act, slope, pixel_norm, eps, out_info=None, in_info=None):
        _note_all(x, w, b, coef, ups, act, slope, pixel_norm, eps, out_info, in_info)
        y, scale, signs = raw_conv(x, w, coef, False, ups, bias=b, act=act, slope=slope, pixel_norm=pixel_norm,
                                   eps=eps, want_scale=True, want_signs=act and not _NO_SIGN_WORDS)
        if out_info is not None:
            out_info.bits = signs
            out_info.pn = (y.detach(), scale) if pixel_norm else None
            if (act and not pixel_norm and not ups and signs is not None and w.dim() == 5 and tuple(w.shape[:4]) == (1, 1, 1, 1) and
                    x.dim() == 5 and not _NO_RGB_FUSION):
                out_info.pw = PwStage(x.detach(), w, coef, b.data_ptr() if b is not None else 0, b is not None, x.requires_grad)
        ctx.save_for_backward(x, w, y if (pixel_norm or (act and signs is None)) else None, scale, signs)
        ctx.cfg = (coef, ups, act, slope, pixel_norm)
        ctx.has_b = b is not None
        ctx.b_ptr = b.data_ptr() if b is not None else 0
        ctx.out_info, ctx.in_info = out_info, in_info
        return y

    @staticmethod
    def backward(ctx, gy):
        x, w, y, scale, signs = ctx.saved_tensors
        coef, ups, act, slope, pixel_norm = ctx.cfg
        if ctx.out_info is not None and ctx.out_info.pw_result is not None:
            gx, gw, gb = ctx.out_info.pw_result
            ctx.out_info.pw_result = None
            return (gx if ctx.needs_input_grad[0] else None), gw, gb, None, None, None, None, None, None, None, None
        g = gy
        want_db = ctx.has_b and _wants(ctx, 2, ctx.b_ptr)
        gb = None
        fused_pn_act = pixel_norm and act and signs is not None
        if fused_pn_act and _masked_in(ctx.out_info):
            pass
        elif fused_pn_act:
            g, gb = _PnActBwd.apply(g, y.detach(), scale, signs, slope, want_db, ctx.b_ptr)
            if not want_db:
                gb = None
        elif pixel_norm:
            g = _PixelNormBwd.apply(g, y, scale)
        premasked = act and not pixel_norm and _masked_in(ctx.out_info)
        if act and not premasked and not fused_pn_act:
            g, gb = _BiasActBwd.apply(g, signs if signs is not None else y.detach(), slope, want_db, ctx.b_ptr)
        gx = None
        db_from_wgrad = want_db and gb is None
        if (ctx.needs_input_grad[0] and _wants(ctx, 1, w.data_ptr()) and not torch.is_grad_enabled() and not ups and
                not _masked_in(ctx.in_info) and w.dim() == 5 and x.dim() == 5 and tuple(w.shape[:3]) == (1, 1, 1) and w.shape[3] <= 4 and
                not _NO_RGB_FUSION):
            res = _pw_backward(x, g, w, coef, db_from_wgrad, ctx.b_ptr)
            if res is not None:
                gx, gw, gb2 = res
                return gx, gw, ((gb2 if db_from_wgrad else gb) if want_db else None), None, None, None, None, None, None, None, None
        if ctx.needs_input_grad[0]:
            gx = _conv_dgrad(g, w, coef, True, ups, ctx.in_info)
        gw, gb = _conv_param_grads(x, g, w, coef, ups, _wants(ctx, 1, w.data_ptr()), want_db, ctx.b_ptr, gb)
        return gx, gw, gb, None, None, None, None, None, None, None, None


def _rgb_matrix(w_rgb, coef, dtype, small_is_cin=False):
    key = ('rgbmat', w_rgb.data_ptr(), w_rgb._version, float(coef), dtype, small_is_cin)
    hit = _PACK_CACHE.get(key)
    if hit is not None:
        return hit[0]
    m = (w_rgb.detach().reshape(w_rgb.shape[-2], w_rgb.shape[-1]).float() * float(coef)).to(dtype).float()
    m = (m if small_is_cin else m.t()).contiguous()
    _PACK_CACHE[key] = (m, w_rgb)
    return m


def _pw_backward(x, dy, w, coef, want_db, b_ptr=0):
    lib = _lib.load()
    x, dy = ndhwc(x), ndhwc(dy)
    n, cin, d, h, wd = _dims(x)
    cout = dy.shape[1]
    if x.dtype != dy.dtype or cin > 4 or cin > cout:
        return None
    shp = _shape(n, d, h, wd, cin, cout, (1, 1, 1), False)
# ... 166 lines not shown


class _PooledDgradGather(torch.autograd.Function):

    @staticmethod
    def forward(ctx, gy, w, signs, slope, coef, mask_bits, mask_slope):
        _note_all(gy)
        gx = _gather_dgrad(gy, w, signs, slope, coef, mask_bits, mask_slope)
        if gx is None:
            raise _GatherDeclined()
        ctx.save_for_backward(gy, w, signs, mask_bits)
        ctx.cfg = (float(slope), float(coef), float(mask_slope))
        ctx.out_back = None
        if mask_bits is not None:
            ctx.out_back = gx._sg_back = BackInfo(mask_bits, mask_slope)
        return gx

    @staticmethod
    def backward(ctx, ggx):
        gy, w, signs, mask_bits = ctx.saved_tensors
        slope, coef, mask_slope = ctx.cfg
        if mask_bits is not None and not (ctx.out_back is not None and ctx.out_back.all_premask()):
            ggx, _ = _BiasActBwd.apply(ggx, mask_bits, mask_slope, False)
        g_gy = g_w = None
        if ctx.needs_input_grad[0]:
            res = res3 = None
            mode = _pool_mode(ggx, (3, 3, 3), 32, 64) if not torch.is_grad_enabled() else 0
            if mode in (1, 3):
                if mode == 3:
                    res3 = raw_conv(ggx, w, coef, False, False, mask_bits=signs, mask_slope=slope, pool=3)
                if res3 is None:
                    res = raw_conv(ggx, w, coef, False, False, mask_bits=signs, mask_slope=slope, pool=1)
            if res3 is not None:
                g_gy = res3[0]
            elif res is not None:
                g_gy = _Down.apply(res[0], 0.5, None, _POOL_REST[1])
            else:
                g_gy = _Down.apply(_Conv.apply(ggx, w, coef, False, False), 0.125, None, (2, 2, 2), signs, slope)
        if _wants(ctx, 1, w.data_ptr()):
            lib = _lib.load()
            ggx_, gy_ = ndhwc(ggx), ndhwc(gy)
            n, _, d, h, wd = _dims(ggx_)
            dt = _dt(ggx_)
            shp = _shape(n, d, h, wd, 32, 64, (3, 3, 3), False)
            acc = _grad_acc(w.data_ptr(), (3, 3, 3, 32, 64))
            rc = _lib.SG_EUNSUPPORTED
            if acc is not None:
                rc = _wgrad_launch(lib, ggx_, gy_, signs, slope, 0.125, acc, None, coef, True, shp, dt)
            if rc != _lib.SG_EUNSUPPORTED:
                check(rc, 'sg_conv3d_wgrad_bias_ex (gathered dy, accumulate)')
                _note_accumulated(w.data_ptr())
                return g_gy, None, None, None, None, None, None
            outs = _GradOuts(ggx.device)
            dw = outs.take(w.data_ptr(), (3, 3, 3, 32, 64))
            rc = _wgrad_launch(lib, ggx_, gy_, signs, slope, 0.125, dw, None, coef, False, shp, dt)
            if outs.declined(rc):
                g_full = _Up.apply(gy_, 0.125, signs, slope, (2, 2, 2))
                dw, _ = raw_wgrad(ggx_, g_full, (3, 3, 3), coef, False, False, w.data_ptr())
            else:
                check(rc, 'sg_conv3d_wgrad_bias_ex (gathered dy)')
            g_w = dw.reshape(w.shape) if dw is not None else None
        return g_gy, g_w, None, None, None, None, None


def _pooled_backward_gather(gy, x, w, signs, coef, slope, in_info, want_gx, want_gw, want_db, b_ptr=0):
    if gy.dtype != torch.bfloat16 or w.dim() != 5 or tuple(w.shape) != (3, 3, 3, 32, 64) or signs is None:
        return None
    lib = _lib.load()
    gy, x = ndhwc(gy), ndhwc(x)
    n, cout, dc, hc, wc = _dims(gy)
    d, h, wd = 2 * dc, 2 * hc, 2 * wc
    _check_signs(signs, n * d * h * wd, 64)
    gx = gw = gb = None
    if want_gx:
        masked = _masked_in(in_info)
        gx = _gather_dgrad(gy, w, signs, slope, coef, in_info.bits if masked else None, in_info.slope if masked else 0.0)
        if gx is None:
            return None
    if want_gw or want_db:
        shp = _shape(n, d, h, wd, 32, 64, (3, 3, 3), False)
        outs = _GradOuts(gy.device)
        acc = _grad_acc(w.data_ptr(), (3, 3, 3, 32, 64)) if want_gw else None
        dw = acc if acc is not None else outs.take(w.data_ptr() if want_gw else 0, (3, 3, 3, 32, 64))
        gb = outs.take(b_ptr, (64,), want_db)
        rc = _wgrad_launch(lib, x, gy, signs, slope, 0.125, dw, gb, coef, acc is not None, shp, _dt(gy))
        if outs.declined(rc):
            return None
        check(rc, 'sg_conv3d_wgrad_bias_ex (gathered dy)')
        if acc is not None:
            _note_accumulated(w.data_ptr())
        gw = dw.reshape(w.shape) if (want_gw and acc is None) else None
    return gx, gw, gb


def _pooled_backward_planes(gy, x, w, signs, coef, slope, in_info, want_gx, want_gw, want_db):
    if gy.dtype != torch.bfloat16 or w.dim() != 5 or tuple(w.shape[:3]) != (3, 3, 3) or w.shape[4] != 64 or w.shape[3] != 32:
        return None
    lib = _lib.load()
    gy = ndhwc(gy)
    n, cout, dc, hc, wc = _dims(gy)
    d, h, wd = 2 * dc, 2 * hc, 2 * wc
    dt, st = _dt(gy), _stream()
    k = (3, 3, 3)
    shp = _shape(n, d, h, wd, 64, 32, k, False)
    ws_bytes = lib.sg_conv3d_fwd_workspace(C.byref(shp), dt)
    if not ws_bytes or signs is None:
        return None
    _check_signs(signs, n * d * h * wd, 64)
    planes = torch.empty((2, n, d, h, wd, 32), device=gy.device, dtype=gy.dtype)
    rc = lib.sg_upscale_nn_planes(_ptr(gy), _ptr(planes), _ptr(signs), float(slope), n, dc, hc, wc, 64, 2, 2, 2, 0.125, 32,
                                  dt, st)
    if rc == _lib.SG_EUNSUPPORTED:
        return None
    check(rc, 'sg_upscale_nn_planes')
    gx = gw = gb = None
    if want_gx:
        masked = _masked_in(in_info)
        res = raw_conv(planes, w, coef, True, False, slope=0.0, mask_bits=in_info.bits if masked else None,
                       mask_slope=in_info.slope if masked else 0.0, x_plane_channels=32)
        if res is None:
            return None
        gx = res[0]
    if want_gw or want_db:
        halves = [planes[i].permute(0, 4, 1, 2, 3) for i in range(2)]
        if want_gw:
            parts = [raw_wgrad(x, g, k, coef, False, want_db) for g in halves]
            gw = torch.cat([p[0] for p in parts], dim=4).reshape(w.shape)
            if want_db:
                gb = torch.cat([p[1] for p in parts])
        else:
            gb = torch.cat([raw_bias_act_bwd(g, None, 0.0, want_dx=False, want_db=True)[1] for g in halves])
    return gx, gw, gb


def _pool_mode(x, k, cin, cout):
    if _NO_POOL_FUSION or x.dim() != 5 or x.dtype != torch.bfloat16 or tuple(k) != (3, 3, 3):
        return 0
    n, _, d, h, wd = x.shape
    if (d | h | wd) & 1 or wd % 32:
        return 0
    nvox = n * d * h * wd
    if cin <= 32 and cin % 8 == 0 and cout % 32 == 0 and d >= 4 and nvox >= (1 << 20):
        if cin == 32 and h >= 8 and not _NO_POOL3:
            return 3
        return 1
    if cin % 16 == 0 and cout % 64 == 0 and nvox >= (1 << 18):
        return 2
    return 0


_POOL_REST = {1: (1, 2, 1), 2: (2, 1, 1)}


def _upconv_dgrad_subpixel(g, w, coef):
    lib = _lib.load()
    g = ndhwc(g)
    n, co, d2, h2, w2 = _dims(g)
    ci = w.shape[3]
    if (d2 | h2 | w2) & 1 or w.shape[4] != co:
        return None
    dt, st = _dt(g), _stream()
    low = _shape(n, d2 // 2, h2 // 2, w2 // 2, ci, co, (3, 3, 3), False)
    if not lib.sg_upconv3d_subpixel_dgrad_supported(C.byref(low), dt):
        return None
    key = ('subpix_dgrad', w.data_ptr(), w._version, float(coef), dt)
    hit = _SUBPIX_CACHE.get(key)
    if hit is None:
        w32 = w.detach()
        if w32.dtype != torch.float32 or not w32.is_contiguous():
            w32 = w32.contiguous().float()
        wp = torch.empty(lib.sg_upconv3d_subpixel_dgrad_packed_bytes(C.byref(low), dt), device=w.device, dtype=torch.uint8)
        check(lib.sg_upconv3d_subpixel_dgrad_pack(_ptr(w32), float(coef), _ptr(wp), C.byref(low), dt, st), 'sg_upconv3d_subpixel_dgrad_pack')
        if w.is_leaf or not w.requires_grad:
            _SUBPIX_CACHE[key] = (wp, w)
    else:
        wp = hit[0]
    gx = _empty_like_shape(g, ci, (d2 // 2, h2 // 2, w2 // 2))
    rc = lib.sg_upconv3d_subpixel_dgrad(_ptr(g), _ptr(wp), _ptr(gx), C.byref(low), dt, st)
    if rc == _lib.SG_EUNSUPPORTED:
        return None
    check(rc, 'sg_upconv3d_subpixel_dgrad')
    return gx


def _upconv_dgrad(g, w, coef, flip):
    if not torch.is_grad_enabled() and w.dim() == 5:
        if flip and not _NO_SUBPIXEL and tuple(w.shape[:3]) == (3, 3, 3) and g.dtype == torch.bfloat16:
            gx = _upconv_dgrad_subpixel(g, w, coef)
            if gx is not None:
                return gx
        cin, cout = (w.shape[4], w.shape[3]) if flip else (w.shape[3], w.shape[4])
        mode = min(_pool_mode(g, w.shape[:3], cin, cout), 2)
        if mode:
            res = raw_conv(g, w, coef, flip, False, pool=mode)
            if res is not None:
                return _Down.apply(res[0], 4.0, None, _POOL_REST[mode])
    return _Down.apply(_Conv.apply(g, w, coef, flip, False), 1.0)


def pool_fusion_available(x, w, bias, slope):
    return w.dim() == 5 and _pool_mode(x, w.shape[:3], x.shape[1] if x.dim() == 5 else 0, w.shape[-1]) != 0


class _BiasActBwd(torch.autograd.Function):

    @staticmethod
    def forward(ctx, dy, y, slope, want_db, b_ptr=0):
        _note_all(dy, y, slope, want_db)
        dx, db = raw_bias_act_bwd(dy, y, slope, True, want_db, b_ptr)
        ctx.save_for_backward(y)
        ctx.slope = slope
        if db is None:
            db = _zero_scalar(dy)
        ctx.mark_non_differentiable(db)
        return dx, db

    @staticmethod
    def backward(ctx, gdx, _gdb):
        (y,) = ctx.saved_tensors
        g, _ = _BiasActBwd.apply(gdx, y, ctx.slope, False)
        return g, None, None, None, None


class _BiasAct(torch.autograd.Function):
    @staticmethod
    def forward(ctx, x, b, act, slope):
        _note_all(x, b, act, slope)
        lib = _lib.load()
        _req_cuda(x, b)
        x = ndhwc(x)
        n, c, d, h, w = _dims(x)
        y = torch.empty_like(x)
        b32 = b.detach().contiguous().float() if b is not None else None
        check(lib.sg_bias_act_fwd(_ptr(x), _ptr(b32), _ptr(y), n * d * h * w, c, 1 if act else 0, float(slope),
                                  _dt(x), _stream()), 'sg_bias_act_fwd')
        ctx.save_for_backward(y)
        ctx.act, ctx.slope, ctx.has_b = act, slope, b is not None
        ctx.b_ptr = b.data_ptr() if b is not None else 0
        return y

    @staticmethod
    def backward(ctx, gy):
        (y,) = ctx.saved_tensors
        want_db = ctx.has_b and _wants(ctx, 1, ctx.b_ptr)
        g, gb = _BiasActBwd.apply(gy, y.detach() if ctx.act else None, ctx.slope, want_db, ctx.b_ptr)
        return g, (gb if want_db else None), None, None


class _PixelNorm(torch.autograd.Function):
    @staticmethod
    def forward(ctx, x, eps):
        _note_all(x, eps)
        lib = _lib.load()
        _req_cuda(x)
        x = ndhwc(x)
        n, c, d, h, w = _dims(x)
        y = torch.empty_like(x)
        scale = torch.empty(n * d * h * w, device=x.device, dtype=torch.float32)
        check(lib.sg_pixel_norm_fwd(_ptr(x), _ptr(y), _ptr(scale), n * d * h * w, c, float(eps), _dt(x), _stream()),
              'sg_pixel_norm_fwd')
        ctx.save_for_backward(y, scale)
        return y

    @staticmethod
    def backward(ctx, gy):
        y, scale = ctx.saved_tensors
        return _PixelNormBwd.apply(gy, y, scale), None


class _PixelNormBwd(torch.autograd.Function):

    @staticmethod
    def forward(ctx, gy, y, scale):
        _note_all(gy, y, scale)
        lib = _lib.load()
        gy, y = ndhwc(gy), ndhwc(y)
        n, c, d, h, w = _dims(gy)
        dx = torch.empty_like(gy)
        check(lib.sg_pixel_norm_bwd(_ptr(gy), _ptr(y), _ptr(scale), _ptr(dx), n * d * h * w, c, _dt(gy), _stream()),
              'sg_pixel_norm_bwd')
        return dx

    @staticmethod
    def backward(ctx, g):
        raise NotImplementedError('second-order gradient through pixel_norm is not part of the pgan step')


class _PnActBwd(torch.autograd.Function):

    @staticmethod
    def forward(ctx, gy, y, scale, signs, slope, want_db, b_ptr=0):
        _note_all(gy, y, scale, signs, slope, want_db)
        lib = _lib.load()
        gy, y = ndhwc(gy), ndhwc(y)
        n, c, d, h, w = _dims(gy)
        nvox = n * d * h * w
        _check_signs(signs, nvox, c)
        dz = torch.empty_like(gy)
        db = ws = None
        if want_db:
            db = _f32_out(b_ptr, (c,), gy.device)
            ws = torch.empty(lib.sg_bias_act_bwd_workspace(c), device=gy.device, dtype=torch.uint8)
        check(lib.sg_pixel_norm_act_bwd(_ptr(gy), _ptr(y), _ptr(scale), _ptr(signs), float(slope), _ptr(dz), _ptr(db),
                                        _ptr(ws), nvox, c, _dt(gy), _stream()), 'sg_pixel_norm_act_bwd')
        if db is None:
            db = _zero_scalar(gy)
        ctx.mark_non_differentiable(db)
        return dz, db

    @staticmethod
    def backward(ctx, g, _gdb):
        raise NotImplementedError('second-order gradient through pixel_norm is not part of the pgan step')


class _Up(torch.autograd.Function):

    @staticmethod
    def forward(ctx, x, gain, mask_bits=None, mask_slope=0.0, factors=(2, 2, 2)):
        _note_all(x)
        lib = _lib.load()
        _req_cuda(x, mask_bits)
        x = ndhwc(x)
        n, c, d, h, w = _dims(x)
        fd, fh, fw = factors
        y = _empty_like_shape(x, c, (fd * d, fh * h, fw * w))
        _check_signs(mask_bits, fd * fh * fw * n * d * h * w, c)
        check(lib.sg_upscale_nn(_ptr(x), _ptr(y), _ptr(mask_bits), float(mask_slope), n, d, h, w, c, fd, fh, fw,
                                float(gain), _dt(x), _stream()), 'sg_upscale_nn')
        ctx.gain, ctx.mask_slope, ctx.factors = gain, mask_slope, tuple(factors)
        ctx.save_for_backward(mask_bits)
        return y

    @staticmethod
    def backward(ctx, gy):
        (mask_bits,) = ctx.saved_tensors
# ... 918 lines not shown
```

saragan_amd/networks/ops.py:

```python
import os
import numpy as np
import torch

from .. import functional as F
from ..varstore import compute_dtype, get_variable, variable_scope


class _LazyUp:

    def __init__(self, x):
        self._src = x
        self._v = None

    @property
    def x(self):
        if not isinstance(self._src, torch.Tensor):
            self._src = _val(self._src)
        return self._src

    @property
    def shape(self):
        n, c, d, h, w = self._src.shape
        return torch.Size((n, c, 2 * d, 2 * h, 2 * w))

    def value(self):
        if self._v is None:
            self._v = F.upscale2x(self.x, 1.0)
        return self._v


class _LazyConv:

    def __init__(self, x, w, coef, ups):
        self.x, self.w, self.coef, self.ups = x, w, coef, ups
        self.bias = None
        self.act = False
        self.slope = 0.2
        self.pn = False
        self.eps = 1e-8
        self.stage = 0
        self.in_info = None
        self.act_info = None
        self._v = None

    @property
    def shape(self):
        n = self.x.shape[0]
        sp = [2 * s for s in self.x.shape[2:]] if self.ups else list(self.x.shape[2:])
        return torch.Size((n, self.w.shape[-1], *sp))

    def value(self):
        if self._v is None:
            out_info = self.act_info if self.act else None
            self._v = F.conv3d(self.x, self.w, self.coef, bias=self.bias, act=self.act, slope=self.slope,
                               pixel_norm=self.pn, eps=self.eps, upsample_in=self.ups, out_info=out_info,
                               in_info=self.in_info)
        return self._v


class _LazyRgbTail(_LazyConv):

    def __init__(self, prod, w, coef):
        super().__init__(None, w, coef, False)
        self.prod = prod

    @property
    def shape(self):
        return torch.Size((self.prod.shape[0], self.w.shape[-1], *self.prod.shape[2:]))

    def value(self):
        if self._v is None:
            p = self.prod
            if p._v is None and not self.act and not self.pn:
                p.act_info = None
                self._v, p._v = F.conv3d_pn_to_rgb(p.x, p.w, p.coef, p.bias, p.ups, p.slope, p.eps, p.in_info,
                                                   self.w, self.coef, self.bias)
            else:
                self._v = F.conv3d(_consume(p, False)[0], self.w, self.coef, bias=self.bias, act=self.act, slope=self.slope,
                                   pixel_norm=self.pn, eps=self.eps)
        return self._v


def _consume(x, premask=False, pn_ok=False):
    if isinstance(x, _LazyConv):
        info = x.act_info if x.act else None
        if x.pn:
            premask = premask and pn_ok
        if info is not None:
            info.consume(premask)
        return x.value(), (info if premask else None)
    if isinstance(x, _LazyUp):
        return x.value(), None
    return x, None


def _val(x):
    return _consume(x, False)[0]


class ScalarVariable:

    def __init__(self, value, name='', dtype=np.float32):
        self.name = name
        self.dtype = dtype
        self.value = dtype(value)

    def assign(self, v):
        self.value = self.dtype(v)
        return self.value

    def eval(self):
        return self.value

    def __float__(self):
        return float(self.value)


class Op:

    def __init__(self, fn, name=''):
        self.fn, self.name = fn, name

    def run(self):
        return self.fn()


def alpha_update(alpha, mixing_nimg, starting_alpha, batch_size, global_size):
    if mixing_nimg == 0:
        return Op(lambda: alpha.assign(0), 'alpha_update')
    num_steps = mixing_nimg // (batch_size * global_size)
    upd = np.float32(starting_alpha / num_steps)
    return Op(lambda: alpha.assign(max(np.float32(alpha.value) - upd, np.float32(0))), 'alpha_update')


def k(x):
    return 1 if x < 3 else 3


def get_kernel(x_shape, desired_k_shape):
    if len(x_shape) != len(desired_k_shape):
        print(f"x_shape: {x_shape}. desired_k_shape: {desired_k_shape}")
    assert len(x_shape) == len(desired_k_shape)
    kernel = []
    for x_i, k_i in zip(x_shape, desired_k_shape):
        if x_i < k_i:
            kernel.append(x_i - 1 if (x_i % 2) == 0 else x_i)
        else:
            kernel.append(k_i)
    return kernel


def calculate_gain(activation, param=None):
    linear_fns = ['linear', 'conv1d', 'conv2d', 'conv3d', 'conv_transpose1d', 'conv_transpose2d', 'conv_transpose3d']
    if activation in linear_fns or activation == 'sigmoid':
        return 1
    elif activation == 'tanh':
        return 5.0 / 3
    elif activation == 'relu':
        return np.sqrt(2.0)
    elif activation == 'leaky_relu':
        assert param is not None
        if not isinstance(param, bool) and isinstance(param, int) or isinstance(param, float):
            negative_slope = param
        else:
            raise ValueError("negative_slope {} not a valid number".format(param))
        return np.sqrt(2.0 / (1 + negative_slope ** 2))
    else:
        raise ValueError("Unsupported nonlinearity {}".format(activation))


class ScaledWeight:

    def __init__(self, var, coef):
        self.var, self.coef = var, float(coef)

    @property
    def shape(self):
        return self.var.shape


_SPECTRAL = {'prefixes': (), 'iterations': 1}


def set_spectral_norm(prefixes=(), iterations=1):
    prefixes = (prefixes,) if isinstance(prefixes, str) else tuple(prefixes or ())
    if int(iterations) < 1:
        raise ValueError('set_spectral_norm: iterations >= 1')
    for p in prefixes:
        if not p.startswith('discriminator/'):
            raise ValueError(f'spectral normalisation is offered for the discriminator only, got the scope prefix {p!r}')
    prev = (_SPECTRAL['prefixes'], _SPECTRAL['iterations'])
    _SPECTRAL['prefixes'], _SPECTRAL['iterations'] = prefixes, int(iterations)
    return prev


def spectral_norm_settings():
    return _SPECTRAL['prefixes'], _SPECTRAL['iterations']


def spectral_norm_applies(name):
    return name.endswith('/weight') and any(name.startswith(p) for p in _SPECTRAL['prefixes'])


def get_weight(shape, activation, lrmul=1, use_eq_lr=True, use_spectral_norm=False, param=None):
    fan_in = np.prod(shape[:-1])
    gain = calculate_gain(activation, param)
    he_std = gain / np.sqrt(fan_in)
    runtime_coef = he_std * lrmul
    from ..varstore import current_store, scope_name
    full = (scope_name() + '/weight') if scope_name() else 'weight'
    fresh = full not in current_store().vars
    w = get_variable('weight', shape, 'normal')
    if fresh and lrmul != 1:
        with torch.no_grad():
            w.mul_(1.0 / lrmul)
    if use_spectral_norm or spectral_norm_applies(full) or full in current_store().effective:
        current_store().normalise(full)
        return ScaledWeight(current_store().effective_weight(full), 1.0)
    return ScaledWeight(w, runtime_coef if use_eq_lr else 1.0)


def apply_bias(x, lrmul=1):
    b = get_variable('bias', [x.shape[1]], 'zeros')
    if lrmul != 1:
        b = b * float(lrmul)
    if isinstance(x, _LazyConv) and x.stage == 0 and x._v is None:
        x.bias, x.stage = b, 1
        return x
    return F.bias_act(_val(x), b, False, 0.0)


def dense(x, fmaps, activation, lrmul=1, param=None, logits=False):
    x = _val(x)
    if len(x.shape) > 2:
        x = x.reshape(x.shape[0], int(np.prod(x.shape[1:])))
    w = get_weight([x.shape[1], fmaps], activation, lrmul=lrmul, param=param)
    dt = torch.float32 if (fmaps == 1 or logits) else compute_dtype()
    return _LazyConv(x.to(dt), w.var, w.coef, False)


def label_rows(conditioning, architecture='pgan'):
    if conditioning is None:
        return None
    if architecture != 'pgan':
        raise NotImplementedError(f'conditioning is offered for the 3-D pgan architecture only, not for {architecture}')
    if not (torch.is_tensor(conditioning) and conditioning.dim() == 2 and conditioning.is_floating_point()):
        raise NotImplementedError('pgan conditioning takes a floating [N, L] tensor of label rows, got '
                                  f'{type(conditioning).__name__}'
                                  + (f' {conditioning.dtype} {tuple(conditioning.shape)}' if torch.is_tensor(conditioning) else ''))
    return conditioning


def label_embedding(z, conditioning):
    if conditioning.shape[0] != z.shape[0]:
        raise ValueError(f'conditioning holds {conditioning.shape[0]} label rows for {z.shape[0]} latents')
    with variable_scope('conditioning'):
        w = get_variable('weight', [conditioning.shape[1], z.shape[1]], 'normal')
    return F.cond_embed(z.to(compute_dtype()), conditioning, w)


def label_projection(x, conditioning):
    x = _val(x)
    if conditioning.shape[0] != x.shape[0]:
        raise ValueError(f'conditioning holds {conditioning.shape[0]} label rows for a batch of {x.shape[0]}')
    return F.cond_project(x, conditioning)


def conv3d(x, fmaps, kernel, activation, param=None, lrmul=1):
    ups = isinstance(x, _LazyUp) and x._v is None
    cin = x.shape[1]
    if (tuple(kernel) == (1, 1, 1) and fmaps <= 4 and type(x) is _LazyConv and x._v is None and x.stage == 3 and x.act and
            x.pn and x.x.dtype == compute_dtype() and not F._NO_RGB_FUSION):
        w = get_weight([*kernel, cin, fmaps], activation, param=param, lrmul=lrmul)
        return _LazyRgbTail(x, w.var, w.coef)
    if ups:
        xin, in_info = x.x, None
    else:
        pn_ok = isinstance(x, _LazyConv) and x.pn and F.pn_bwd_epilogue_available(tuple(x.shape), kernel, fmaps, compute_dtype())
        xin, in_info = _consume(x, premask=True, pn_ok=pn_ok)
    w = get_weight([*kernel, cin, fmaps], activation, param=param, lrmul=lrmul)
    if xin.dtype != compute_dtype():
        xin, in_info = xin.to(compute_dtype()), None
    lz = _LazyConv(xin, w.var, w.coef, ups)
    lz.in_info = in_info
    return lz


def leaky_relu(x, alpha_lr=0.2):
    if isinstance(x, _LazyConv) and x.stage <= 1 and x._v is None:
        x.act, x.slope, x.stage = True, float(alpha_lr), 2
        x.act_info = F.ActInfo(alpha_lr)
        return x
    return F.bias_act(_val(x), None, True, float(alpha_lr))


def act(x, activation, param=None):
    if activation == 'leaky_relu':
        assert param is not None
        return leaky_relu(x, alpha_lr=param)
    elif activation == 'linear':
        return x
    else:
        raise ValueError(f"Unknown activation {activation}")


def num_filters(phase, num_phases, base_shape, base_dim=None, size=None):
    lists = {
        'xxs': [256, 256, 64, 32, 16, 8, 4, 2], 'xs': [256, 256, 64, 64, 32, 16, 8, 4],
        's': [512, 512, 128, 128, 64, 32, 16, 8], 'm': [1024, 1024, 256, 256, 128, 64, 32, 16],
        'l': [2048, 2048, 512, 512, 256, 128, 64, 32], 'xl': [4096, 4096, 1024, 1024, 512, 256, 128, 64],
        'xxl': [8192, 8192, 2048, 1024, 1024, 512, 256, 128]}
    if size not in lists:
        raise ValueError(f"Unknown size: {size}")
    filter_list = lists[size]
    assert len(filter_list) == 8, "Filter lists are built for LIDC-IDRI dataset."
    current_dim = [2 ** (phase - 1) * dim for dim in base_shape[1:]]
    log_product = np.log2(np.prod(current_dim))
    reference_log = [4 + n * 3 for n in range(0, 7)]
    index = np.argmin(np.abs(np.array(reference_log) - log_product))
    return filter_list[index]


def to_rgb(x, channels=1):
    return apply_bias(conv3d(x, channels, (1, 1, 1), activation='linear'))


def from_rgb(x, filters_out, activation, param=None):
    x = conv3d(x, filters_out, (1, 1, 1), activation, param)
    x = apply_bias(x)
    x = act(x, activation, param=param)
    return x


def avg_unpool3d(x, factor=2, gain=1):
    x = _val(x)
    if factor == 1:
        return x if gain == 1 else F.lerp(x, None, float(gain), 0.0)
    if factor != 2:
        raise NotImplementedError('only factor 2 is used by the pgan path')
    return F.upscale2x(x, float(gain))


def avg_pool3d(x, factor=2, gain=1):
    if factor == 1:
        x = _val(x)
        return x if gain == 1 else F.lerp(x, None, float(gain), 0.0)
    if factor != 2:
        raise NotImplementedError('only factor 2 is used by the pgan path')
    if (gain == 1 and isinstance(x, _LazyConv) and x._v is None and x.act and not x.pn and not x.ups and
            F.pool_fusion_available(x.x, x.w, x.bias, x.slope)):
        try:
            return F.conv3d_act_pool(x.x, x.w, x.coef, x.bias, x.slope, x.in_info)
        except F._lib.SgError:
            pass
    x, in_info = _consume(x, premask=True)
    return F.downscale2x(x, float(gain) / 8.0, in_info)


def upscale3d(x, factor=2):
    if factor == 1:
        return x
    if factor != 2:
        raise NotImplementedError('only factor 2 is used by the pgan path')
    return _LazyUp(x)


def upscale3d_trilinear(x, factor=2):
    if factor == 1:
        return x
    if factor != 2:
        raise NotImplementedError('only factor 2')
    return F.upscale_trilinear2x(_val(x))


def downscale3d_trilinear(x, factor=2):
    return avg_pool3d(x, factor)


def downscale3d(x, factor=2):
    return avg_pool3d(x, factor)


def pixel_norm(x, epsilon=1e-8):
    if isinstance(x, _LazyConv) and x._v is None and x.shape[1] <= F.PN_FUSE_MAX_CHANNELS:
        x.pn, x.eps, x.stage = True, float(epsilon), 3
        return x
    return F.pixel_norm(_val(x), float(epsilon))


def minibatch_stddev_layer(x, group_size=4):
    return F.minibatch_stddev(_val(x), group_size)


_MBSTD = {'group': 0, 'segments': 1}


def set_minibatch_stddev(group=0):
    if int(group) < 0:
        raise ValueError('set_minibatch_stddev: group >= 0 (0 turns the layer off)')
    prev = _MBSTD['group']
    _MBSTD['group'] = int(group)
    return prev


def minibatch_stddev_settings():
    return _MBSTD['group']


class mbstd_segments:

    def __init__(self, k):
        self.k = int(k)

    def __enter__(self):
        self.prev = _MBSTD['segments']
        _MBSTD['segments'] = self.k

    def __exit__(self, *a):
        _MBSTD['segments'] = self.prev


def conv3d_minibatch_stddev(x, fmaps, kernel, activation, param=None):
    from ..varstore import current_store, scope_name
    group, nseg = _MBSTD['group'], _MBSTD['segments']
    if len(x.shape) != 5:
        raise NotImplementedError('minibatch stddev is offered for the 3-D pgan discriminator only')
    xt = _consume(x, False)[0]
    cin = x.shape[1]
    coef_full = calculate_gain(activation, param) / np.sqrt(np.prod(kernel) * (cin + 1))
# ... 55 lines not shown
```

Baseline: 617.6.

## Fuse pixel-norm and leaky-ReLU backward into subpixel upconv and 64-channel conv dgrad

Adds a pixel-norm backward epilogue to the subpixel upsampling-conv data-gradient kernel and extends the conv_fwd5 kernel's PNB epilogue to 64-channel layers. Inside the epilogue it applies the leaky-ReLU mask and pixel-norm gradient (a dot product with y, then scaling) before storing. The Python lazy-upsample path now consumes the producer's activation info so the fused path can be chosen. The goal is to drop the separate elementwise backward kernels and the extra global read/write of the gradient tensor, at the cost of more register pressure and extra loads of y and scale in the kernel epilogues.

Result: no change. 618.9 (median of 6 runs) (+0.2%).

```diff
diff --git a/include/saragan_hip.h b/include/saragan_hip.h
--- a/include/saragan_hip.h
+++ b/include/saragan_hip.h
@@ -89,6 +89,8 @@
 size_t sg_upconv3d_subpixel_dgrad_packed_bytes(const sg_conv_shape* s, sg_dtype dt);
 int sg_upconv3d_subpixel_dgrad_pack(const float* w_dhwio, float coef, void* wp, const sg_conv_shape* s, sg_dtype dt, sg_stream_t st);
 int sg_upconv3d_subpixel_dgrad(const void* gy, const void* wp, void* gx, const sg_conv_shape* s, sg_dtype dt, sg_stream_t st);
+int sg_upconv3d_subpixel_dgrad_ep(const void* gy, const void* wp, void* gx, const sg_conv_shape* s, const sg_conv_epilogue* ep,
+                                  sg_dtype dt, sg_stream_t st);
 size_t sg_conv3d_wgrad_workspace(const sg_conv_shape* s, sg_dtype dt);
 int sg_conv3d_wgrad(const void* x, const void* dy, float* dw_dhwio, float coef, void* workspace,
                     size_t workspace_bytes, const sg_conv_shape* s, sg_dtype dt, sg_stream_t st);
diff --git a/saragan_amd/_lib.py b/saragan_amd/_lib.py
--- a/saragan_amd/_lib.py
+++ b/saragan_amd/_lib.py
@@ -64,6 +64,7 @@
     'sg_upconv3d_subpixel_dgrad_packed_bytes': (_sz, [_SHP, C.c_int]),
     'sg_upconv3d_subpixel_dgrad_pack': (C.c_int, [_p, _f, _p, _SHP, C.c_int, _p]),
     'sg_upconv3d_subpixel_dgrad': (C.c_int, [_p, _p, _p, _SHP, C.c_int, _p]),
+    'sg_upconv3d_subpixel_dgrad_ep': (C.c_int, [_p, _p, _p, _SHP, C.POINTER(ConvEpilogue), C.c_int, _p]),
     'sg_conv3d_wgrad_workspace': (_sz, [_SHP, C.c_int]),
     'sg_conv3d_wgrad': (C.c_int, [_p, _p, _p, _f, _p, _sz, _SHP, C.c_int, _p]),
     'sg_conv3d_pw_bwd': (C.c_int, [_p, _p, _p, _p, _p, _p, _f, _p, _sz, _SHP, C.c_int, _p]),
diff --git a/saragan_amd/csrc/conv3d.hip b/saragan_amd/csrc/conv3d.hip
--- a/saragan_amd/csrc/conv3d.hip
+++ b/saragan_amd/csrc/conv3d.hip
@@ -2032,6 +2032,8 @@
   constexpr uint32_t DEAD = 0x80000000u;
   constexpr bool SIGN = (EPI & SG_EP_SIGN) != 0, MASK = (EPI & SG_EP_MASK) != 0, PN = (EPI & SG_EP_PN) != 0;
   constexpr bool POOL = (EPI & SG_EP_POOL) != 0;
+  constexpr bool PNB = (EPI & SG_EP_PNB) != 0;
+  static_assert(!PNB || (MASK && !SIGN && !PN && !POOL), "pixel-norm backward epilogue: masked data gradient only");
   const sg_tile_geom& g = a.g;
   const int tid = threadIdx.x, lane = tid & 63;
   const int wave8 = __builtin_amdgcn_readfirstlane(tid >> 6);
@@ -2136,6 +2138,7 @@
   };
   int kE = 0;
   __amdgpu_buffer_rsrc_t ryE, rsE, rmE, rpE;
+  int n0E = 0;
   uint32_t vox[2];
   uint32_t pvox = DEAD;
   auto enter_tile_E = [&]() {
@@ -2144,6 +2147,7 @@
     if (SIGN) rsE = rsrc_of(a.sign_out, wsb, o.n0);
     if (MASK) rmE = rsrc_of(a.mask_bits, wsb, o.n0);
     if (PN) rpE = rsrc_of(a.pn_scale, psb, o.n0);
+    if (PNB) n0E = o.n0;
 #pragma unroll
     for (int mt = 0; mt < 2; ++mt) {
       const int tc = tcoord[mt];
@@ -2199,7 +2203,23 @@
   };
   auto mfma_phase = [&](int q) { sg_unrolled_k5<3>::run(acc, xaddr, wl0 + (q & 1) * a.wbytes); };
 
-  auto off_phase = [&](bool closes, int qn, int js, int f0, int f1) {
+  auto off_phase = [&](bool closes, bool pre, int qn, int js, int f0, int f1) {
+    u32x4 yraw[PNB ? 2 : 1][PNB ? 2 : 1][PNB ? 2 : 1];
+    float pscale[2] = {0.f, 0.f};
+    if constexpr (PNB) {
+      const __amdgpu_buffer_rsrc_t rbE = rsrc_of(a.pnb_y, ysb, n0E), rqE = rsrc_of(a.pnb_scale, psb, n0E);
+#pragma unroll
+      for (int mt = 0; mt < 2; ++mt) {
+        const bool live = closes && vox[mt] != DEAD;
+#pragma unroll
+        for (int nt = 0; nt < 2; ++nt)
+#pragma unroll
+          for (int j = 0; j < 2; ++j)
+            yraw[mt][nt][j] = __builtin_amdgcn_raw_buffer_load_b128(
+                rbE, live ? (vox[mt] * (uint32_t)cout + (uint32_t)((nt0 + nt) * 32 + 16 * j + 8 * hh)) * 2u : DEAD, 0, 0);
+        pscale[mt] = __uint_as_float(__builtin_amdgcn_raw_buffer_load_b32(rqE, live ? vox[mt] * 4u : DEAD, 0, 0));
+      }
+    }
     if (qn < items_mine) stage_halo();
     if (js < items_max) stage_slab(js, f0, f1, wave, 4);
     __builtin_amdgcn_sched_barrier(0);
@@ -2229,6 +2249,38 @@
             for (int i = 0; i < 16; ++i) acc[mt][nt][i] *= sc;
           if (a.pn_scale != nullptr)
             __builtin_amdgcn_raw_buffer_store_b32(__float_as_uint(sc), rpE, (ok && hh == 0) ? vox[mt] * 4u : DEAD, 0, 0);
+        }
+        if constexpr (PNB) {
+          float yv[2][16];
+          float dot = 0.f;
+#pragma unroll
+          for (int nt = 0; nt < 2; ++nt) {
+#pragma unroll
+            for (int i = 0; i < 16; i += 2) {
+              const uint32_t pk = sg_pack_bf16(acc[mt][nt][i], acc[mt][nt][i + 1]);
+              acc[mt][nt][i] = __uint_as_float(pk << 16);
+              acc[mt][nt][i + 1] = __uint_as_float(pk & 0xFFFF0000u);
+            }
+#pragma unroll
+            for (int j = 0; j < 2; ++j) {
+              const auto t0 = __builtin_amdgcn_permlane32_swap(yraw[mt][nt][j][0], yraw[mt][nt][j][2], false, false);
+              const auto t1 = __builtin_amdgcn_permlane32_swap(yraw[mt][nt][j][1], yraw[mt][nt][j][3], false, false);
+              const uint32_t pk[4] = {t0[0], t1[0], t0[1], t1[1]};
+#pragma unroll
+              for (int k = 0; k < 4; ++k) {
+                yv[nt][8 * j + 2 * k] = __uint_as_float(pk[k] << 16);
+                yv[nt][8 * j + 2 * k + 1] = __uint_as_float(pk[k] & 0xFFFF0000u);
+              }
+            }
+#pragma unroll
+            for (int i = 0; i < 16; ++i) dot = fmaf(acc[mt][nt][i], yv[nt][i], dot);
+          }
+          const auto sw2 = __builtin_amdgcn_permlane32_swap(__float_as_uint(dot), __float_as_uint(dot), false, false);
+          const float mean = (__uint_as_float(sw2[0]) + __uint_as_float(sw2[1])) * inv_c;
+#pragma unroll
+          for (int nt = 0; nt < 2; ++nt)
+#pragma unroll
+            for (int i = 0; i < 16; ++i) acc[mt][nt][i] = pscale[mt] * fmaf(-yv[nt][i], mean, acc[mt][nt][i]);
         }
 #pragma unroll
         for (int nt = 0; nt < 2; ++nt) {
@@ -2284,6 +2336,13 @@
       request_mask();
       init_acc();
     }
+    uint32_t pft[2] = {0u, 0u};
+    if constexpr (PNB) {
+      const uint32_t vt = hh ? vox[1] : vox[0];
+      const bool live = pre && kE < kmine && vt != DEAD;
+      pft[0] = __builtin_amdgcn_raw_buffer_load_b32(rsrc_of(a.pnb_y, ysb, n0E), live ? vt * (uint32_t)(cout * ES) : DEAD, 0, 0);
+      pft[1] = __builtin_amdgcn_raw_buffer_load_b32(rsrc_of(a.pnb_scale, psb, n0E), live ? vt * 4u : DEAD, 0, 0);
+    }
     if (qn < items_mine) {
       if (++cgS == ncg) {
         cgS = 0;
@@ -2292,6 +2351,7 @@
       }
     }
     asm volatile("s_waitcnt vmcnt(0)" ::: "memory");
+    if constexpr (PNB) asm volatile("" ::"v"(pft[0]), "v"(pft[1]));
   };
 
   if (grp == 0) {
@@ -2303,7 +2363,7 @@
       stamp();
       __syncthreads();
       stamp();
-      off_phase(q < items_mine && (q % ncg) == ncg - 1, q + 1, q + 1, HF, NFRAG);
+      off_phase(q < items_mine && (q % ncg) == ncg - 1, PNB && q + 1 < items_mine && ((q + 1) % ncg) == ncg - 1, q + 1, q + 1, HF, NFRAG);
       stamp();
       __syncthreads();
     }
@@ -2311,7 +2371,7 @@
     init_acc();
     for (int q = 0; q < items_max; ++q) {
       stamp();
-      off_phase(q > 0 && q - 1 < items_mine && ((q - 1) % ncg) == ncg - 1, q, q + 1, 0, HF);
+      off_phase(q > 0 && q - 1 < items_mine && ((q - 1) % ncg) == ncg - 1, PNB && q < items_mine && (q % ncg) == ncg - 1, q, q + 1, 0, HF);
       stamp();
       __syncthreads();
       stamp();
@@ -2319,7 +2379,7 @@
       stamp();
       __syncthreads();
     }
-    if (items_mine > 0 && items_mine == items_max) off_phase(true, items_mine, items_max, 0, 0);
+    if (items_mine > 0 && items_mine == items_max) off_phase(true, false, items_mine, items_max, 0, 0);
     else if (items_mine > 0) {  }
   }
 }
@@ -2339,6 +2399,7 @@
   if (a.pool && ((s->h | s->w) & 1 || a.pixel_norm || a.mask_bits)) return SG_OK;
   if (a.pixel_norm && (a.mask_bits || a.ntile != 2)) return SG_OK;
   if (a.mask_bits && a.sign_out) return SG_OK;
+  if (a.pnb_y && (a.ntile != 2 || s->cout != 64 || !a.mask_bits || a.bias || a.act || a.sign_out || a.pool || a.pixel_norm)) return SG_OK;
   a.g = sg_make_geom(s, 256, true);
   const sg_tile_geom& g = a.g;
   if (g.TN != 1 || g.TW != 32 || (g.TH & 1) || g.TD * g.TH * g.TW != 256 || g.HD > 127 || g.HH > 127 || g.HW > 127) return SG_OK;
@@ -2364,7 +2425,7 @@
   a.vec_in = 1;
   a.vec_out = 1;
   const int epi = (a.sign_out ? SG_EP_SIGN : 0) | (a.mask_bits ? SG_EP_MASK : 0) | (a.pixel_norm ? SG_EP_PN : 0) |
-                  (a.pool ? SG_EP_POOL : 0);
+                  (a.pool ? SG_EP_POOL : 0) | (a.pnb_y ? SG_EP_PNB : 0);
   int rc = SG_OK;
   switch (epi) {
     case 0: rc = launch_fwd5_inst<0>(a, (unsigned)gx, (unsigned)ny, lds, st); break;
@@ -2372,12 +2433,14 @@
     case SG_EP_SIGN | SG_EP_POOL: rc = launch_fwd5_inst<SG_EP_SIGN | SG_EP_POOL>(a, (unsigned)gx, (unsigned)ny, lds, st); break;
     case SG_EP_SIGN: rc = launch_fwd5_inst<SG_EP_SIGN>(a, (unsigned)gx, (unsigned)ny, lds, st); break;
     case SG_EP_MASK: rc = launch_fwd5_inst<SG_EP_MASK>(a, (unsigned)gx, (unsigned)ny, lds, st); break;
+    case SG_EP_MASK | SG_EP_PNB: rc = launch_fwd5_inst<SG_EP_MASK | SG_EP_PNB>(a, (unsigned)gx, (unsigned)ny, lds, st); break;
     case SG_EP_PN: rc = launch_fwd5_inst<SG_EP_PN>(a, (unsigned)gx, (unsigned)ny, lds, st); break;
     case SG_EP_PN | SG_EP_SIGN: rc = launch_fwd5_inst<SG_EP_PN | SG_EP_SIGN>(a, (unsigned)gx, (unsigned)ny, lds, st); break;
     default: return SG_OK;
   }
   if (rc != SG_OK) return rc;
-  SG_KNAME("conv_fwd5<bf16,2,2,3,3,3>");
+  if (a.pnb_y) SG_KNAME("conv_fwd5<bf16,2,2,3,3,3,pnb>");
+  else SG_KNAME("conv_fwd5<bf16,2,2,3,3,3>");
   SG_LAUNCH_CHECK();
   *used = true;
   return SG_OK;
@@ -2714,9 +2777,10 @@
                  (a.pool == 3 && (s->cin != 32 || s->kd != 3 || s->kh != 3 || s->kw != 3 || s->upsample_in || !sg_cfg().fwd3s_16 ||
                                   sg_cfg().fwd_no_v3 || sg_cfg().fwd_no_v3s || (ep && ep->x_plane_channels)))))
     return SG_EUNSUPPORTED;
-  if (a.pnb_y && (subpixel || dt != SG_BF16 || sg_cfg().fwd_v1 || sg_cfg().fwd_no_v3 || sg_cfg().fwd_no_v3s || a.pool ||
-                  a.pixel_norm || (s->cin * 2) % 16 != 0 || s->kd != 3 || s->kh != 3 || s->kw != 3 || s->upsample_in ||
-                  (ep && ep->x_plane_channels)))
+  const bool pnb5 = a.pnb_y && s->cout == 64 && s->cin == 64;
+  if (a.pnb_y && (subpixel || dt != SG_BF16 || sg_cfg().fwd_v1 || a.pool || a.pixel_norm || (s->cin * 2) % 16 != 0 || s->kd != 3 ||
+                  s->kh != 3 || s->kw != 3 || s->upsample_in || (ep && ep->x_plane_channels) ||
+                  (pnb5 ? sg_cfg().fwd_no_v5 : (sg_cfg().fwd_no_v3 || sg_cfg().fwd_no_v3s))))
     return SG_EUNSUPPORTED;
   if (sg_small_eligible(s) && !sg_cfg().no_small && !a.pool && !a.pnb_y && !(ep && ep->x_plane_channels)) {
     rc = sg_small_fwd(x, reinterpret_cast<const char*>(wp) + (size_t)a.nchunk * a.taps * a.ntile * 1024, y, s, a.bias, a.act, a.slope,
@@ -2802,7 +2866,7 @@
       else if (a.nchunk == 1) rc = launch_fwd3s<1>(a, s, hs, &used);
       if (rc != SG_OK || used) { prof.done(rc); return rc; }
     }
-    if (a.pool || a.pnb_y) { prof.done(SG_EUNSUPPORTED); return SG_EUNSUPPORTED; }
+    if (a.pool || (a.pnb_y && !pnb5)) { prof.done(SG_EUNSUPPORTED); return SG_EUNSUPPORTED; }
     if (dt == SG_BF16) {
       if (k333 && a.nchunk == 2) rc = launch_fwd3r<bf16_t, 2, 2, 3, 3, 3>(a, s, hs, &used);
       else if (k333 && a.nchunk == 1) rc = launch_fwd3r<bf16_t, 2, 1, 3, 3, 3>(a, s, hs, &used);
@@ -2822,6 +2886,7 @@
     rc = launch_fwd5(a, s, hs, &used);
     if (rc != SG_OK || used) { prof.done(rc); return rc; }
   }
+  if (a.pnb_y) { prof.done(SG_EUNSUPPORTED); return SG_EUNSUPPORTED; }
   if (v2 && !sg_cfg().fwd_no_v4 && (!a.pixel_norm || a.ntile <= 2)) {
     bool used = false;
     rc = SG_OK;
diff --git a/saragan_amd/csrc/subpix.hip b/saragan_amd/csrc/subpix.hip
--- a/saragan_amd/csrc/subpix.hip
+++ b/saragan_amd/csrc/subpix.hip
@@ -626,6 +626,10 @@
   int N, d, h, w, ci, co, nchunk;
   int nTd, nTh, nTw;
   int64_t ntiles;
+  const bf16_t* pnb_y;
+  const float* pnb_scale;
+  const uint32_t* mask_bits;
+  float mask_slope;
 };
 
 namespace {
@@ -633,10 +637,11 @@
 constexpr int kDgY = 6 * 10 * 2 * 33 * 32;
 }
 
-template <int NT, int TD, int TH, int TW>
+template <int NT, int TD, int TH, int TW, bool PNB = false>
 __global__ __launch_bounds__(512) void upconv_subpixel_dgrad_kernel(SubpixDgradArgs a) {
   extern __shared__ __attribute__((aligned(16))) char smem[];
   static_assert(TD * TH * TW == 256, "256 low-resolution voxels per tile");
+  static_assert(!PNB || NT == 2, "pixel-norm backward epilogue: the block holds all 64 channels of a voxel");
   constexpr int NG = 64 * NT / 16;
   constexpr int TPG = 16 / NT;
   constexpr int FD = 2 * TD + 2, FH = 2 * TH + 2, PW = TW + 1;
@@ -725,6 +730,9 @@
   if (ntl == 0) return;
   const int nchunk = a.nchunk;
   f32x16 acc[NT];
+  u32x4 yraw[PNB ? NT : 1][PNB ? 2 : 1];
+  float pscale = 0.f;
+  uint32_t mb[2] = {0u, 0u};
 
   enter_tile(t_first);
   plan_tile();
@@ -760,6 +768,24 @@
         load_w(wr[g & 3], c4, g4 % NG);
       }
       load_y_part(nchunk_i, more, GG);
+      if constexpr (PNB && g == 1) {
+        const bool last = chunk + 1 == nchunk;
+        const int64_t sv = (int64_t)a.d * a.h * a.w;
+        const uint32_t ovs = (uint32_t)(((od0 + vd) * a.h + oh0 + vh) * a.w + ow0 + vw);
+        const auto rsrc = [&](const void* base, int64_t sample_bytes) {
+          return __builtin_amdgcn_make_buffer_rsrc(const_cast<char*>(reinterpret_cast<const char*>(base)) + on0 * sample_bytes, 0,
+                                                   (int)sample_bytes, 0x00020000);
+        };
+        const __amdgpu_buffer_rsrc_t rb = rsrc(a.pnb_y, sv * 128), rq = rsrc(a.pnb_scale, sv * 4), rm = rsrc(a.mask_bits, sv * 8);
+#pragma unroll
+        for (int nt = 0; nt < NT; ++nt) {
+#pragma unroll
+          for (int j = 0; j < 2; ++j)
+            yraw[nt][j] = __builtin_amdgcn_raw_buffer_load_b128(rb, last ? (ovs * 64u + (uint32_t)(nt * 32 + 16 * j + 8 * hh)) * 2u : DEAD, 0, 0);
+          mb[nt] = __builtin_amdgcn_raw_buffer_load_b32(rm, last ? (ovs * 2u + nt) * 4u : DEAD, 0, 0);
+        }
+        pscale = __uint_as_float(__builtin_amdgcn_raw_buffer_load_b32(rq, last ? ovs * 4u : DEAD, 0, 0));
+      }
       const char* ws = wbuf + (g & 1) * kDgW;
       constexpr int FD_ = 3;
       u32x4 xf[FD_], wf[FD_][NT];
@@ -786,6 +812,40 @@
     });
     if (chunk + 1 == nchunk) {
       const int64_t ov = (((int64_t)on0 * a.d + od0 + vd) * a.h + oh0 + vh) * a.w + ow0 + vw;
+      if constexpr (PNB) {
+        float yv[NT][16];
+        float dot = 0.f;
+#pragma unroll
+        for (int nt = 0; nt < NT; ++nt) {
+#pragma unroll
+          for (int i = 0; i < 16; i += 2) {
+            const uint32_t pk = sg_pack_bf16(acc[nt][i], acc[nt][i + 1]);
+            acc[nt][i] = __uint_as_float(pk << 16);
+            acc[nt][i + 1] = __uint_as_float(pk & 0xFFFF0000u);
+          }
+#pragma unroll
+          for (int j = 0; j < 2; ++j) {
+            const auto t0 = __builtin_amdgcn_permlane32_swap(yraw[nt][j][0], yraw[nt][j][2], false, false);
+            const auto t1 = __builtin_amdgcn_permlane32_swap(yraw[nt][j][1], yraw[nt][j][3], false, false);
+            const uint32_t pk[4] = {t0[0], t1[0], t0[1], t1[1]};
+#pragma unroll
+            for (int k = 0; k < 4; ++k) {
+              yv[nt][8 * j + 2 * k] = __uint_as_float(pk[k] << 16);
+              yv[nt][8 * j + 2 * k + 1] = __uint_as_float(pk[k] & 0xFFFF0000u);
+            }
+          }
+#pragma unroll
+          for (int i = 0; i < 16; ++i) dot = fmaf(acc[nt][i], yv[nt][i], dot);
+        }
+        const auto sw2 = __builtin_amdgcn_permlane32_swap(__float_as_uint(dot), __float_as_uint(dot), false, false);
+        const float mean = (__uint_as_float(sw2[0]) + __uint_as_float(sw2[1])) * (1.f / 64.f);
+#pragma unroll
+        for (int nt = 0; nt < NT; ++nt) {
+#pragma unroll
+          for (int i = 0; i < 16; ++i) acc[nt][i] = pscale * fmaf(-yv[nt][i], mean, acc[nt][i]);
+          sg_apply_sign_word(acc[nt], mb[nt], hh, a.mask_slope);
+        }
+      }
 #pragma unroll
       for (int nt = 0; nt < NT; ++nt) sg_store_tile_row_bf16(a.gx + ov * a.ci + (cpart * NT + nt) * 32, acc[nt], hh, true);
     }
@@ -863,10 +923,27 @@
 }
 
 extern "C" int sg_upconv3d_subpixel_dgrad(const void* gy, const void* wp, void* gx, const sg_conv_shape* s, sg_dtype dt, sg_stream_t st) {
+  return sg_upconv3d_subpixel_dgrad_ep(gy, wp, gx, s, nullptr, dt, st);
+}
+
+extern "C" int sg_upconv3d_subpixel_dgrad_ep(const void* gy, const void* wp, void* gx, const sg_conv_shape* s, const sg_conv_epilogue* ep,
+                                             sg_dtype dt, sg_stream_t st) {
   if (!s || !gy || !wp || !gx) return SG_EINVAL;
+  if (ep && ep->struct_size != (uint32_t)sizeof(sg_conv_epilogue)) return SG_EINVAL;
   if (!sg_aligned16(gy) || !sg_aligned16(wp) || !sg_aligned16(gx)) return SG_EALIGN;
   if (!sg_upconv3d_subpixel_dgrad_supported(s, dt)) return SG_EUNSUPPORTED;
+  const bool pnb = ep && ep->pn_bwd_y;
+  if (ep && ((ep->pn_bwd_y != nullptr) != (ep->pn_bwd_scale != nullptr) || (pnb && !ep->mask_bits))) return SG_EINVAL;
+  if (ep && (!pnb || ep->bias || ep->act || ep->pixel_norm || ep->sign_out || ep->pool || ep->x_plane_channels || ep->out_scale ||
+             ep->in_mask_bits || ep->rgb_out || ep->pw_x))
+    return SG_EUNSUPPORTED;
+  if (pnb && (!sg_aligned16(ep->pn_bwd_y) || !sg_aligned16(ep->mask_bits))) return SG_EALIGN;
+  if (pnb && (s->cin != 64 || (int64_t)s->d * s->h * s->w * 128 >= (1ll << 31))) return SG_EUNSUPPORTED;
   SubpixDgradArgs a;
+  a.pnb_y = pnb ? reinterpret_cast<const bf16_t*>(ep->pn_bwd_y) : nullptr;
+  a.pnb_scale = pnb ? ep->pn_bwd_scale : nullptr;
+  a.mask_bits = pnb ? reinterpret_cast<const uint32_t*>(ep->mask_bits) : nullptr;
+  a.mask_slope = pnb ? ep->mask_slope : 0.f;
   int TD, TH, TW;
   subpix_tile(s, &TD, &TH, &TW);
   a.gy = reinterpret_cast<const bf16_t*>(gy); a.wp = reinterpret_cast<const char*>(wp); a.gx = reinterpret_cast<bf16_t*>(gx);
@@ -882,15 +959,18 @@
   const unsigned gx_ = (unsigned)per_part;
   const size_t lds = 2 * (size_t)kDgW + (size_t)kDgY;
   const int nt = s->cin / 32;
-  SG_KNAME("upconv_subpixel_dgrad");
-#define SG_DG(NT_, TD_, TH_, TW_)                                                    \
+  if (pnb) SG_KNAME("upconv_subpixel_dgrad<pnb>");
+  else SG_KNAME("upconv_subpixel_dgrad");
+#define SG_DG(NT_, TD_, TH_, TW_, PNB_)                                              \
   do {                                                                               \
-    auto kern = upconv_subpixel_dgrad_kernel<NT_, TD_, TH_, TW_>;                    \
+    auto kern = upconv_subpixel_dgrad_kernel<NT_, TD_, TH_, TW_, PNB_>;              \
     SG_ALLOW_160K_LDS(kern);                                                         \
     hipLaunchKernelGGL(kern, dim3(gx_, (unsigned)(nt / 2)), dim3(512), lds, sg_st(st), a); \
   } while (0)
-  if (TW == 32) SG_DG(2, 2, 4, 32);
-  else if (TW == 16) SG_DG(2, 2, 8, 16);
+  if (TW == 32 && pnb) SG_DG(2, 2, 4, 32, true);
+  else if (TW == 16 && pnb) SG_DG(2, 2, 8, 16, true);
+  else if (TW == 32) SG_DG(2, 2, 4, 32, false);
+  else if (TW == 16) SG_DG(2, 2, 8, 16, false);
   else { prof.done(SG_EUNSUPPORTED); return SG_EUNSUPPORTED; }
 #undef SG_DG
   hipError_t e = hipGetLastError();
diff --git a/saragan_amd/functional.py b/saragan_amd/functional.py
--- a/saragan_amd/functional.py
+++ b/saragan_amd/functional.py
@@ -69,6 +69,7 @@
 _NO_SIGN_WORDS = _switch('NO_SIGN_WORDS')
 _NO_GRAD_DEST = _switch('NO_GRAD_DEST')
 _NO_PN_EPILOGUE = _switch('NO_PN_EPILOGUE')
+_NO_PN64_EPILOGUE = _switch('NO_PN64_EPILOGUE')
 _NO_PW_EPILOGUE = _switch('NO_PW_EPILOGUE')
 _NO_BACK_PREMASK = _switch('NO_BACK_PREMASK')
 _NO_RGB_FWD_EPILOGUE = _switch('NO_RGB_FWD_EPILOGUE')
@@ -525,10 +526,17 @@
     return ctx_info is not None and ctx_info.all_premask()
 
 
-def pn_bwd_epilogue_available(prod_shape, kernel, fmaps, dtype):
+def pn_bwd_epilogue_available(prod_shape, kernel, fmaps, dtype, ups=False):
     if _NO_PN_EPILOGUE or dtype != torch.bfloat16 or len(prod_shape) != 5 or tuple(kernel) != (3, 3, 3):
         return False
     n, c, d, h, w = prod_shape
+    if ups:
+        if _NO_PN64_EPILOGUE or _NO_SUBPIXEL or c != 64:
+            return False
+        low = _shape(n, d, h, w, c, fmaps, (3, 3, 3), False)
+        return bool(_lib.load().sg_upconv3d_subpixel_dgrad_supported(C.byref(low), _lib.SG_BF16))
+    if c == 64:
+        return not _NO_PN64_EPILOGUE and fmaps == 64 and w % 32 == 0 and h % 2 == 0 and n * d * h * w >= 512 * 256
     return c == 32 and fmaps == 32 and w % 32 == 0 and d >= 2 and h >= 8
 
 
@@ -603,6 +611,8 @@
 
 def _conv_dgrad(g, w, coef, flip, ups=False, in_info=None, x_back=None):
     if ups:
+        if _masked_in(in_info):
+            return _upconv_dgrad_into(in_info, g, w, coef, flip)
         return _upconv_dgrad(g, w, coef, flip)
     if x_back is not None and x_back.all_premask():
         return _Conv.apply(g, w, coef, flip, False, None, x_back.bits, x_back.slope)
@@ -1075,7 +1085,7 @@
 _POOL_REST = {1: (1, 2, 1), 2: (2, 1, 1)}
 
 
-def _upconv_dgrad_subpixel(g, w, coef):
+def _upconv_dgrad_subpixel(g, w, coef, info=None):
     lib = _lib.load()
     g = ndhwc(g)
     n, co, d2, h2, w2 = _dims(g)
@@ -1099,11 +1109,34 @@
     else:
         wp = hit[0]
     gx = _empty_like_shape(g, ci, (d2 // 2, h2 // 2, w2 // 2))
-    rc = lib.sg_upconv3d_subpixel_dgrad(_ptr(g), _ptr(wp), _ptr(gx), C.byref(low), dt, st)
+    if info is not None:
+        pn_y, pn_scale = ndhwc(info.pn[0]), info.pn[1]
+        if tuple(pn_y.shape) != tuple(gx.shape) or pn_y.dtype != gx.dtype or pn_scale.numel() != n * (d2 // 2) * (h2 // 2) * (w2 // 2):
+            raise ValueError('pn_bwd: y / scale do not match the low-resolution gradient')
+        _check_signs(info.bits, pn_scale.numel(), ci)
+        ep = ConvEpilogue(None, 0, 0.0, 0, 0.0, None, _ptr(info.bits), float(info.slope), None)
+        ep.pn_bwd_y, ep.pn_bwd_scale = pn_y.data_ptr(), pn_scale.data_ptr()
+        rc = lib.sg_upconv3d_subpixel_dgrad_ep(_ptr(g), _ptr(wp), _ptr(gx), C.byref(low), C.byref(ep), dt, st)
+    else:
+        rc = lib.sg_upconv3d_subpixel_dgrad(_ptr(g), _ptr(wp), _ptr(gx), C.byref(low), dt, st)
     if rc == _lib.SG_EUNSUPPORTED:
         return None
     check(rc, 'sg_upconv3d_subpixel_dgrad')
     return gx
+
+
+def _upconv_dgrad_into(info, g, w, coef, flip):
+    if torch.is_grad_enabled():
+        raise NotImplementedError('second-order gradient through a fused-upsample conv')
+    if (info.pn is not None and flip and not _NO_SUBPIXEL and w.dim() == 5 and tuple(w.shape[:3]) == (3, 3, 3) and
+            g.dtype == torch.bfloat16):
+        gx = _upconv_dgrad_subpixel(g, w, coef, info)
+        if gx is not None:
+            return gx
+    gx = _upconv_dgrad(g, w, coef, flip)
+    if info.pn is None:
+        return _BiasActBwd.apply(gx, info.bits, info.slope, False)[0]
+    return _PnActBwd.apply(gx, info.pn[0], info.pn[1], info.bits, info.slope, False)[0]
 
 
 def _upconv_dgrad(g, w, coef, flip):
diff --git a/saragan_amd/networks/ops.py b/saragan_amd/networks/ops.py
--- a/saragan_amd/networks/ops.py
+++ b/saragan_amd/networks/ops.py
@@ -11,11 +11,14 @@
     def __init__(self, x):
         self._src = x
         self._v = None
+        self._info = None
 
     @property
     def x(self):
         if not isinstance(self._src, torch.Tensor):
             self._src = _val(self._src)
+        elif self._info is not None:
+            self._info.consume(False)
         return self._src
 
     @property
@@ -27,6 +30,12 @@
         if self._v is None:
             self._v = F.upscale2x(self.x, 1.0)
         return self._v
+
+    def consume(self, pn_ok):
+        if isinstance(self._src, torch.Tensor) or not pn_ok:
+            return self.x, None
+        self._src, self._info = _consume(self._src, premask=True, pn_ok=True)
+        return self._src, self._info
 
 
 class _LazyConv:
@@ -274,7 +283,10 @@
         w = get_weight([*kernel, cin, fmaps], activation, param=param, lrmul=lrmul)
         return _LazyRgbTail(x, w.var, w.coef)
     if ups:
-        xin, in_info = x.x, None
+        src = x._src
+        pn_ok = (isinstance(src, _LazyConv) and src.act and src.pn and
+                 F.pn_bwd_epilogue_available(tuple(src.shape), kernel, fmaps, compute_dtype(), ups=True))
+        xin, in_info = x.consume(pn_ok)
     else:
         pn_ok = isinstance(x, _LazyConv) and x.pn and F.pn_bwd_epilogue_available(tuple(x.shape), kernel, fmaps, compute_dtype())
         xin, in_info = _consume(x, premask=True, pn_ok=pn_ok)
```
